# ProgramerSalar/stable-diffusion-from-scratch

Hardware: AMD Instinct MI355X
Metric: images/sec (512×512, 50-step DDIM) at 1/2/4/8 MI355X; UNet step ms (higher is better)
Workload: dtype f16; 1 GPU; sd1-txt2img-512-ddim50; global_batch=16, batch_per_gpu=16, ddim_steps=50, parallelism=dp1

## Files before the change

include/sdk_amd.h:

```cpp
#ifndef SDK_AMD_H
#define SDK_AMD_H

#include <stdint.h>

#ifdef __cplusplus
extern "C" {
#endif

typedef void* sdk_stream_t;

enum sdk_status {
  SDK_OK = 0,
  SDK_EINVAL = -1,
  SDK_EHIP = -2,
  SDK_EWORKSPACE = -3
};

typedef struct {
  const void* src0;
  const void* src1;
  int32_t c_split;
  int32_t cin;
  int32_t ld0, ld1;
  int32_t h, w;
  int32_t ksize;
  int32_t stride, pad;
  int32_t upsample;
  const float* gn_scale;
  const float* gn_shift;
  int32_t silu;
  int32_t pad_end;
} sdk_conv_src;

enum sdk_out_mode {
  SDK_OUT_NHWC_F16 = 0,
  SDK_OUT_NCHW_F32 = 1,
  SDK_OUT_GEGLU_F16 = 2,
  SDK_OUT_ROWS_F32 = 3
};

typedef struct {
  int32_t batch, ho, wo, cout;
  int32_t nseg;
  sdk_conv_src seg[2];
  const void* weight;
  int32_t k_total;
  const float* bias;
  const float* row_bias;
  int32_t row_bias_ld;
  const void* residual;
  int32_t res_ld;
  void* out;
  int32_t out_ld;
  int32_t out_mode;
  int32_t split_k;
  float* workspace;
  int64_t workspace_bytes;
  int32_t variant_hint;
  int32_t act;
  float* gn_partial;
  int64_t weight_batch_stride;
  int32_t split_inlaunch;
  uint32_t* tile_counters;
  int32_t tile_group_m;
  int32_t upsample_phase;
} sdk_conv_args;

#define SDK_TILE_COUNTERS 16384

enum sdk_conv_act {
  SDK_ACT_NONE = 0,
  SDK_ACT_QUICK_GELU = 1,
  SDK_ACT_GELU = 2
};

typedef struct {
  int32_t split_k;
  int32_t grid_tiles;
  int64_t workspace_bytes;
  int32_t variant;
  double flops;
  int32_t gn_chunks;
} sdk_conv_plan_info;

int sdk_conv2d_plan(const sdk_conv_args* a, sdk_conv_plan_info* info);
int sdk_conv2d(const sdk_conv_args* a, sdk_stream_t stream);

typedef struct {
  const void* src0; const void* src1;
  int32_t c_split, ld0, ld1;
  int32_t batch, hw, channels, groups;
  float eps;
  const float* gamma; const float* beta;
  float* scale; float* shift;
  float* workspace; int64_t workspace_bytes;
} sdk_group_norm_args;

int64_t sdk_group_norm_workspace(int32_t batch, int32_t hw, int32_t channels);
int sdk_group_norm_affine(const sdk_group_norm_args* a, sdk_stream_t stream);

int sdk_group_norm_apply(const sdk_group_norm_args* a, int32_t silu, void* y, int32_t ld_y, sdk_stream_t stream);

int sdk_group_norm_apply_padded(const sdk_group_norm_args* a, int32_t silu, void* y, int32_t ld_y, int32_t h,
                                int32_t w, int32_t pad, sdk_stream_t stream);

int sdk_group_norm(const sdk_group_norm_args* a, int32_t silu, void* y, int32_t ld_y, int32_t h, int32_t w,
                   int32_t pad, const float* part0, int32_t nch0, const float* part1, int32_t nch1,
                   sdk_stream_t stream);

int sdk_group_norm_finalize(const sdk_group_norm_args* a, const float* part0, int32_t nch0, const float* part1,
                            int32_t nch1, sdk_stream_t stream);

int sdk_group_norm_apply_ex(const sdk_group_norm_args* a, int32_t silu, const float* post_bias, int32_t pb_ld,
                            const void* residual, int32_t res_ld, void* y, int32_t ld_y, sdk_stream_t stream);

enum { SDK_GN_STATS_GIVEN = 0,
       SDK_GN_STATS_SLICE,
       SDK_GN_STATS_CHUNKED,
       SDK_GN_STATS_PARTS };
enum { SDK_GN_APPLY_NONE = 0,
       SDK_GN_APPLY_IN_STATS,
       SDK_GN_APPLY_FLAT, SDK_GN_APPLY_ROW, SDK_GN_APPLY_STRIDE };
typedef struct { int32_t stats, apply, launches; int64_t workspace_bytes; } sdk_group_norm_plan_info;
int sdk_group_norm_plan(const sdk_group_norm_args* a, int32_t want_stats, int32_t want_apply, int32_t h, int32_t w,
                        int32_t pad, int32_t nch0, int32_t nch1, int32_t allow_single_launch,
                        sdk_group_norm_plan_info* info);

double sdk_probe_mfma_flops(int32_t m16, int32_t blocks, int32_t iters);
int sdk_probe_mfma(int32_t m16, int32_t blocks, int32_t iters, const void* seed, float* sink, sdk_stream_t stream);
int sdk_probe_copy(const void* src, void* dst, int64_t bytes, sdk_stream_t stream);
int sdk_probe_copy_ex(const void* src, void* dst, int64_t bytes, int32_t mode, sdk_stream_t stream);

int sdk_layer_norm(const void* x, void* y, int32_t rows, int32_t cols, int32_t ld_x, int32_t ld_y,
                   const float* gamma, const float* beta, float eps, sdk_stream_t stream);

typedef struct {
  const void* q; const void* k; const void* v; void* o;
  int32_t q_ld, k_ld, v_ld, o_ld;
  int32_t batch, heads, nq, nk, head_dim;
  float scale;
  int32_t causal;
} sdk_attention_args;

int sdk_attention(const sdk_attention_args* a, sdk_stream_t stream);

enum { SDK_ATTN_AUTO = 0, SDK_ATTN_NW4, SDK_ATTN_NW8, SDK_ATTN_NW8_STAG, SDK_ATTN_QB2, SDK_ATTN_WIDE };
#define SDK_ATTN_WIDE_ROWS 64
#define SDK_ATTN_WIDE_KT 32
typedef struct { int32_t form, dqk, dv, waves, qblocks, stagger, seed_col, causal, grid; } sdk_attention_form_info;
int sdk_attention_form(const sdk_attention_args* a, int32_t form, sdk_attention_form_info* ran ,
                       sdk_stream_t stream);

typedef struct {
  const void* q; const void* k; const void* v; void* o;
  int32_t q_ld, k_ld, v_ld, o_ld;
  int32_t batch, heads, n, dim_head;
  void* workspace; int64_t workspace_bytes;
} sdk_linear_attention_args;
int32_t sdk_linear_attention_chunks(int32_t n);
int64_t sdk_linear_attention_workspace_bytes(const sdk_linear_attention_args* a);
int sdk_linear_attention(const sdk_linear_attention_args* a, sdk_stream_t stream);

typedef struct {
  const void* t; const void* kv; const void* wq; const void* wo; const float* bias; const void* res;
  void* out;
  int32_t t_ld, kv_ld, w_ld, res_ld, out_ld;
  int32_t batch, n_img, nk, channels, head_dim;
  float scale;
} sdk_xattn_args;

int sdk_cross_attention_block_supported(int32_t channels, int32_t head_dim, int32_t nk, int32_t n_img);
int sdk_xattn_pack_weight(const void* w, int32_t w_ld, void* packed, int32_t channels, sdk_stream_t stream);
int sdk_cross_attention_block(const sdk_xattn_args* a, sdk_stream_t stream);

typedef struct {
  const float* in_gamma; const float* in_beta; float in_eps;
  const float* out_gamma; const float* out_beta; float out_eps;
  void* out_ln; int32_t out_ln_ld;
} sdk_xattn_ln_args;

int sdk_cross_attention_block_ln(const sdk_xattn_args* a, const sdk_xattn_ln_args* ln, sdk_stream_t stream);

int sdk_segment_softmax(const float* s, int32_t ld_s, void* p, int32_t ld_p, int32_t rows, int32_t nseg,
                        int32_t seglen, float scale, sdk_stream_t stream);

typedef struct {
  const void* t; const void* res; void* out; const void* packed; const float* b2;
  int32_t t_ld, res_ld, out_ld;
  int32_t rows, channels, features;
} sdk_ff_args;

int sdk_ff_supported(int32_t channels, int32_t features);
int64_t sdk_ff_packed_bytes(int32_t channels, int32_t features);
int sdk_ff_pack(const void* w1, const float* b1, const void* w2, void* packed, int32_t channels, int32_t features,
                sdk_stream_t stream);
int sdk_feed_forward(const sdk_ff_args* a, sdk_stream_t stream);

typedef struct {
  const void* x; const void* w; const float* bias; const void* res; void* out;
  int32_t x_ld, res_ld, out_ld;
  int32_t rows, in_features, out_features;
} sdk_token_linear_args;

int sdk_token_linear_supported(int32_t in_features, int32_t out_features);
int sdk_token_linear(const sdk_token_linear_args* a, sdk_stream_t stream);

int sdk_token_linear_ln(const sdk_token_linear_args* a, const float* gamma, const float* beta, float eps,
                        void* out_ln, int32_t out_ln_ld, sdk_stream_t stream);

typedef struct {
  const void* x; const float* gn_scale; const float* gn_shift; const void* w; const float* bias;
  const float* gamma; const float* beta; void* tok; void* qkv;
  int32_t x_ld, tok_ld, qkv_ld, rows, hw;
  int32_t in_features, features, qkv_features;
  float eps;
} sdk_proj_norm_qkv_args;

int sdk_proj_norm_qkv_supported(int32_t in_features, int32_t features, int32_t qkv_features);
int sdk_proj_norm_qkv(const sdk_proj_norm_qkv_args* a, sdk_stream_t stream);

typedef struct {
  const float* x; const float* e; const float* e_uncond; const float* noise;
  float* x_prev; float* pred_x0;
  int64_t n;
  float sqrt_one_minus_at, sqrt_at, dir_coef, sqrt_a_prev, sigma, temperature;
  float guidance;
  int32_t v_param;
  float v_sqrt_a, v_sqrt_1ma;
} sdk_ddim_args;

int sdk_ddim_step(const sdk_ddim_args* a, sdk_stream_t stream);

int sdk_ddim_xprev(const sdk_ddim_args* a, sdk_stream_t stream);

typedef struct {
  const float* x; const float* model_out; const float* noise; const float* x_recon_in;
  float* x_prev; float* x_recon;
  int64_t n;
  int32_t stage, x0_param, clip;
  float c_recip, c_recipm1, coef1, coef2, sigma, nonzero, temperature;
} sdk_posterior_args;

int sdk_posterior_step(const sdk_posterior_args* a, sdk_stream_t stream);

typedef struct {
  const float* x0; const float* noise; const float* mask; const float* img;
  float* out;
  int64_t n, per_sample;
  int32_t hw, mask_mode;
  float sqrt_acp, sqrt_1m_acp;
} sdk_masked_q_args;

int sdk_masked_q_sample(const sdk_masked_q_args* a, sdk_stream_t stream);

int sdk_cfg_combine(const float* e_uncond, const float* e_cond, float* out, int64_t n, float guidance,
                    sdk_stream_t stream);

typedef struct {
  sdk_ddim_args step;
  int32_t pred_x0_in;
  float drop_scale;
  const uint8_t* keep;
  sdk_masked_q_args blend;
} sdk_ddim_ex_args;

int sdk_ddim_step_ex(const sdk_ddim_ex_args* a, sdk_stream_t stream);

typedef struct {
  sdk_posterior_args step;
  const uint8_t* keep;
  float drop_scale;
} sdk_posterior_ex_args;

int sdk_posterior_step_ex(const sdk_posterior_ex_args* a, sdk_stream_t stream);

enum { SDK_MULTISTEP_PLMS = 0, SDK_MULTISTEP_PLMS_WARMUP = 1, SDK_MULTISTEP_DPM = 2 };

typedef struct {
  sdk_ddim_args step;
  const float* hist[3];
  const float* e_next;
  float* hist_out;
  int32_t form, nhist;
  float c_x, c_0, c_1;
  int32_t reserved;
  sdk_masked_q_args blend;
} sdk_multistep_args;

int sdk_multistep_step(const sdk_multistep_args* a, sdk_stream_t stream);

typedef struct {
  const float* src[4];
  int32_t channels[4];
  int32_t nsrc;
  void* y;
  int32_t batch, hw, c_pad;
} sdk_concat_args;

int sdk_concat_nchw_to_nhwc(const sdk_concat_args* a, sdk_stream_t stream);

typedef struct {
  const float* src[4];
  int32_t channels[4];
  int32_t nsrc;
  void* y;
  int32_t batch, h, w, c_pad;
  int32_t kh, kw, sy, sx;
  int32_t p0, np;
} sdk_patch_pack_args;

int sdk_patch_pack(const sdk_patch_pack_args* a, sdk_stream_t stream);

int sdk_vq_code_norms(const float* codebook, float* norms, int32_t n, int32_t d, sdk_stream_t stream);

int32_t sdk_vq_nearest_splits(int64_t m, int32_t n, int32_t d);

int sdk_vq_nearest(const float* z, const float* codebook, const float* norms, int64_t* idx, float* z_q,
                   int32_t batch, int32_t d, int32_t hw, int32_t n, void* keys, int64_t keys_bytes,
                   int32_t force_splits, sdk_stream_t stream);

int sdk_vq_lookup(const int64_t* idx, const float* codebook, float* out, int64_t m, int32_t n, int32_t d,
                  int32_t hw, int32_t nchw, sdk_stream_t stream);

int sdk_vq_remap(const int64_t* inds, const int64_t* used, const int64_t* rnd, int64_t* out, int64_t count,
                 int32_t n_used, int32_t mode, int64_t unknown, int32_t extra, sdk_stream_t stream);

int sdk_ddpm_step(const float* x, const float* eps, const float* noise, float* out, int64_t n,
                  float inv_sqrt_alpha, float coef, float sigma, sdk_stream_t stream);

int sdk_timestep_embedding(const int64_t* t, const float* freqs, void* out, int32_t batch, int32_t dim,
                           sdk_stream_t stream);

int sdk_nchw_to_nhwc(const float* x, void* y, int32_t batch, int32_t channels, int32_t hw, int32_t c_pad,
                     float scale, sdk_stream_t stream);

int sdk_diag_gaussian_sample(const float* moments, const float* noise, float* z, int32_t batch, int32_t channels,
                             int32_t hw, float scale, sdk_stream_t stream);

int sdk_stochastic_encode(const float* x0, const float* noise, float* out, int64_t n, float sqrt_a,
                          float sqrt_1ma, sdk_stream_t stream);

int sdk_token_embedding(const int64_t* ids, const float* tok, const float* pos, void* out, int32_t batch,
                        int32_t seq, int32_t dim, sdk_stream_t stream);

int sdk_extract_patches(const float* z, float* out, int32_t batch, int32_t channels, int32_t h, int32_t w,
                        int32_t kh, int32_t kw, int32_t sy, int32_t sx, sdk_stream_t stream);
int sdk_fold_patches(const float* patches, const float* pix_w, const float* l_w, float* out, int32_t batch,
                     int32_t channels, int32_t h, int32_t w, int32_t ph, int32_t pw, int32_t sy, int32_t sx,
                     int32_t ly, int32_t lx, sdk_stream_t stream);

int sdk_upsample_bilinear2x(const void* x, void* y, int32_t batch, int32_t h, int32_t w, int32_t channels,
                            sdk_stream_t stream);
int sdk_gelu(const void* x, void* y, int64_t n, sdk_stream_t stream);

int sdk_upsample_nearest2x_padded(const void* x, int32_t ld_x, void* y, int32_t batch, int32_t h, int32_t w,
                                  int32_t channels, int32_t pad, sdk_stream_t stream);

int sdk_zero_border(const void* x, int32_t ld_x, void* y, int32_t batch, int32_t h, int32_t w, int32_t channels,
                    int32_t pad, sdk_stream_t stream);

int sdk_group_norm_film(const sdk_group_norm_args* a, const float* film, int32_t film_ld, int32_t film_off,
                        int32_t silu, void* y, int32_t ld_y, int32_t h, int32_t w, int32_t pad, const float* part0,
                        int32_t nch0, const float* part1, int32_t nch1, sdk_stream_t stream);

enum { SDK_RESAMPLE_AVGPOOL2 = 0, SDK_RESAMPLE_NEAREST2 = 1 };
int sdk_group_norm_resample(const sdk_group_norm_args* a, int32_t mode, int32_t silu, int32_t h, int32_t w,
                            int32_t pad, void* y_act, void* y_raw, sdk_stream_t stream);

int sdk_embedding_add(const void* emb, const float* table, const int64_t* ids, void* out, int32_t batch, int32_t dim,
                      int32_t n, sdk_stream_t stream);

int sdk_embedding_rows(const int64_t* ids, const float* table, void* out, int32_t n, int32_t dim,
                       sdk_stream_t stream);

enum { SDK_RESIZE_NEAREST = 0, SDK_RESIZE_BILINEAR = 1, SDK_RESIZE_BICUBIC = 2, SDK_RESIZE_AREA = 3 };
typedef struct {
  const float* x;
  float* y;
  int32_t planes, h, w, out_h, out_w, mode;
  double scale_h, scale_w;
} sdk_resize2d_args;

int sdk_resize2d(const sdk_resize2d_args* a, sdk_stream_t stream);

const char* sdk_last_error(void);
int sdk_version(void);
const char* sdk_kernel_name(int32_t variant);

#ifdef __cplusplus
}
#endif
#endif
```

stable-diffusion-from-scratch_amd/_lib.py:

```python
from __future__ import annotations

import ctypes as C
import os

_HERE = os.path.dirname(os.path.abspath(__file__))
LIB_PATH = os.environ.get("SD_AMD_LIB") or os.path.join(_HERE, "libsdk_amd.so")

vp = C.c_void_p
i32 = C.c_int32
i64 = C.c_int64
f32 = C.c_float
fp = C.POINTER(C.c_float)


class ConvSrc(C.Structure):
    _fields_ = [("src0", vp), ("src1", vp), ("c_split", i32), ("cin", i32), ("ld0", i32), ("ld1", i32),
                ("h", i32), ("w", i32), ("ksize", i32), ("stride", i32), ("pad", i32), ("upsample", i32),
                ("gn_scale", vp), ("gn_shift", vp), ("silu", i32), ("pad_end", i32)]


class ConvArgs(C.Structure):
    _fields_ = [("batch", i32), ("ho", i32), ("wo", i32), ("cout", i32), ("nseg", i32), ("seg", ConvSrc * 2),
                ("weight", vp), ("k_total", i32), ("bias", vp), ("row_bias", vp), ("row_bias_ld", i32),
                ("residual", vp), ("res_ld", i32), ("out", vp), ("out_ld", i32), ("out_mode", i32),
                ("split_k", i32), ("workspace", vp), ("workspace_bytes", i64), ("variant_hint", i32),
                ("act", i32), ("gn_partial", vp), ("weight_batch_stride", i64), ("split_inlaunch", i32),
                ("tile_counters", vp), ("tile_group_m", i32), ("upsample_phase", i32)]


class ConvPlanInfo(C.Structure):
    _fields_ = [("split_k", i32), ("grid_tiles", i32), ("workspace_bytes", i64), ("variant", i32),
                ("flops", C.c_double), ("gn_chunks", i32)]


class GroupNormArgs(C.Structure):
    _fields_ = [("src0", vp), ("src1", vp), ("c_split", i32), ("ld0", i32), ("ld1", i32), ("batch", i32),
                ("hw", i32), ("channels", i32), ("groups", i32), ("eps", f32), ("gamma", vp), ("beta", vp),
                ("scale", vp), ("shift", vp), ("workspace", vp), ("workspace_bytes", i64)]


class GroupNormPlanInfo(C.Structure):
    _fields_ = [("stats", i32), ("apply", i32), ("launches", i32), ("workspace_bytes", i64)]


class AttentionArgs(C.Structure):
    _fields_ = [("q", vp), ("k", vp), ("v", vp), ("o", vp), ("q_ld", i32), ("k_ld", i32), ("v_ld", i32),
                ("o_ld", i32), ("batch", i32), ("heads", i32), ("nq", i32), ("nk", i32), ("head_dim", i32),
                ("scale", f32), ("causal", i32)]


class AttentionFormInfo(C.Structure):
    _fields_ = [("form", i32), ("dqk", i32), ("dv", i32), ("waves", i32), ("qblocks", i32), ("stagger", i32),
                ("seed_col", i32), ("causal", i32), ("grid", i32)]


class LinearAttentionArgs(C.Structure):
    _fields_ = [("q", vp), ("k", vp), ("v", vp), ("o", vp), ("q_ld", i32), ("k_ld", i32), ("v_ld", i32),
                ("o_ld", i32), ("batch", i32), ("heads", i32), ("n", i32), ("dim_head", i32), ("workspace", vp),
                ("workspace_bytes", i64)]


class XAttnArgs(C.Structure):
    _fields_ = [("t", vp), ("kv", vp), ("wq", vp), ("wo", vp), ("bias", vp), ("res", vp), ("out", vp),
                ("t_ld", i32), ("kv_ld", i32), ("w_ld", i32), ("res_ld", i32), ("out_ld", i32), ("batch", i32),
                ("n_img", i32), ("nk", i32), ("channels", i32), ("head_dim", i32), ("scale", f32)]


class XAttnLnArgs(C.Structure):
    _fields_ = [("in_gamma", vp), ("in_beta", vp), ("in_eps", f32), ("out_gamma", vp), ("out_beta", vp),
                ("out_eps", f32), ("out_ln", vp), ("out_ln_ld", i32)]


class FfArgs(C.Structure):
    _fields_ = [("t", vp), ("res", vp), ("out", vp), ("packed", vp), ("b2", vp), ("t_ld", i32), ("res_ld", i32),
                ("out_ld", i32), ("rows", i32), ("channels", i32), ("features", i32)]


class TokenLinearArgs(C.Structure):
    _fields_ = [("x", vp), ("w", vp), ("bias", vp), ("res", vp), ("out", vp), ("x_ld", i32), ("res_ld", i32),
                ("out_ld", i32), ("rows", i32), ("in_features", i32), ("out_features", i32)]


class ProjNormQkvArgs(C.Structure):
    _fields_ = [("x", vp), ("gn_scale", vp), ("gn_shift", vp), ("w", vp), ("bias", vp), ("gamma", vp), ("beta", vp),
                ("tok", vp), ("qkv", vp), ("x_ld", i32), ("tok_ld", i32), ("qkv_ld", i32), ("rows", i32), ("hw", i32),
                ("in_features", i32), ("features", i32), ("qkv_features", i32), ("eps", f32)]


class DdimArgs(C.Structure):
    _fields_ = [("x", vp), ("e", vp), ("e_uncond", vp), ("noise", vp), ("x_prev", vp), ("pred_x0", vp),
                ("n", i64), ("sqrt_one_minus_at", f32), ("sqrt_at", f32), ("dir_coef", f32), ("sqrt_a_prev", f32),
                ("sigma", f32), ("temperature", f32), ("guidance", f32), ("v_param", i32), ("v_sqrt_a", f32),
                ("v_sqrt_1ma", f32)]


class PosteriorArgs(C.Structure):
    _fields_ = [("x", vp), ("model_out", vp), ("noise", vp), ("x_recon_in", vp), ("x_prev", vp), ("x_recon", vp),
                ("n", i64), ("stage", i32), ("x0_param", i32), ("clip", i32), ("c_recip", f32), ("c_recipm1", f32),
                ("coef1", f32), ("coef2", f32), ("sigma", f32), ("nonzero", f32), ("temperature", f32)]


class MaskedQArgs(C.Structure):
    _fields_ = [("x0", vp), ("noise", vp), ("mask", vp), ("img", vp), ("out", vp), ("n", i64), ("per_sample", i64),
                ("hw", i32), ("mask_mode", i32), ("sqrt_acp", f32), ("sqrt_1m_acp", f32)]


class DdimExArgs(C.Structure):
    _fields_ = [("step", DdimArgs), ("pred_x0_in", i32), ("drop_scale", f32), ("keep", vp), ("blend", MaskedQArgs)]


class MultistepArgs(C.Structure):
    _fields_ = [("step", DdimArgs), ("hist", vp * 3), ("e_next", vp), ("hist_out", vp), ("form", i32), ("nhist", i32),
                ("c_x", f32), ("c_0", f32), ("c_1", f32), ("reserved", i32), ("blend", MaskedQArgs)]


class PosteriorExArgs(C.Structure):
    _fields_ = [("step", PosteriorArgs), ("keep", vp), ("drop_scale", f32)]


class ConcatArgs(C.Structure):
    _fields_ = [("src", vp * 4), ("channels", i32 * 4), ("nsrc", i32), ("y", vp), ("batch", i32), ("hw", i32),
                ("c_pad", i32)]


class PatchPackArgs(C.Structure):
    _fields_ = [("src", vp * 4), ("channels", i32 * 4), ("nsrc", i32), ("y", vp), ("batch", i32), ("h", i32),
                ("w", i32), ("c_pad", i32), ("kh", i32), ("kw", i32), ("sy", i32), ("sx", i32), ("p0", i32),
                ("np", i32)]


class Resize2dArgs(C.Structure):
    _fields_ = [("x", vp), ("y", vp), ("planes", i32), ("h", i32), ("w", i32), ("out_h", i32), ("out_w", i32),
                ("mode", i32), ("scale_h", C.c_double), ("scale_w", C.c_double)]


OUT_NHWC_F16, OUT_NCHW_F32, OUT_GEGLU_F16, OUT_ROWS_F32 = 0, 1, 2, 3
RESIZE_NEAREST, RESIZE_BILINEAR, RESIZE_BICUBIC, RESIZE_AREA = range(4)
ACT_NONE, ACT_QUICK_GELU, ACT_GELU = 0, 1, 2
ATTN_AUTO, ATTN_NW4, ATTN_NW8, ATTN_NW8_STAG, ATTN_QB2, ATTN_WIDE = range(6)
MULTISTEP_PLMS, MULTISTEP_PLMS_WARMUP, MULTISTEP_DPM = range(3)
ATTN_WIDE_ROWS, ATTN_WIDE_KT = 64, 32
RESAMPLE_AVGPOOL2, RESAMPLE_NEAREST2 = 0, 1
GN_STATS = ("given", "slice", "chunked", "parts")
GN_APPLY = ("none", "in_stats", "flat", "row", "stride")

EXPORTS = ["sdk_conv2d_plan", "sdk_conv2d", "sdk_group_norm_workspace", "sdk_group_norm_affine", "sdk_group_norm_apply", "sdk_group_norm_apply_padded", "sdk_group_norm_apply_ex", "sdk_group_norm", "sdk_group_norm_finalize", "sdk_group_norm_plan", "sdk_layer_norm",
           "sdk_attention", "sdk_attention_form", "sdk_linear_attention", "sdk_linear_attention_workspace_bytes", "sdk_linear_attention_chunks", "sdk_cross_attention_block_supported", "sdk_xattn_pack_weight", "sdk_cross_attention_block", "sdk_cross_attention_block_ln", "sdk_segment_softmax", "sdk_ff_supported", "sdk_ff_packed_bytes", "sdk_ff_pack", "sdk_feed_forward", "sdk_token_linear_supported", "sdk_token_linear", "sdk_token_linear_ln", "sdk_proj_norm_qkv_supported", "sdk_proj_norm_qkv", "sdk_ddim_step", "sdk_ddim_xprev", "sdk_ddim_step_ex", "sdk_multistep_step", "sdk_cfg_combine", "sdk_posterior_step", "sdk_posterior_step_ex", "sdk_masked_q_sample", "sdk_concat_nchw_to_nhwc", "sdk_patch_pack", "sdk_ddpm_step", "sdk_timestep_embedding", "sdk_nchw_to_nhwc",
           "sdk_diag_gaussian_sample", "sdk_stochastic_encode", "sdk_token_embedding", "sdk_extract_patches",
           "sdk_fold_patches", "sdk_vq_code_norms", "sdk_vq_nearest_splits", "sdk_vq_nearest", "sdk_vq_lookup", "sdk_vq_remap",
           "sdk_upsample_bilinear2x", "sdk_upsample_nearest2x_padded", "sdk_zero_border", "sdk_gelu",
           "sdk_group_norm_film", "sdk_group_norm_resample", "sdk_embedding_add", "sdk_embedding_rows", "sdk_resize2d", "sdk_last_error", "sdk_version", "sdk_kernel_name",
           "sdk_probe_mfma_flops", "sdk_probe_mfma", "sdk_probe_copy", "sdk_probe_copy_ex"]

_lib = None


def lib():
    global _lib
    if _lib is not None:
        return _lib
    if not os.path.exists(LIB_PATH):
        raise RuntimeError(f"sd_amd: HIP library not built ({LIB_PATH} missing); run __graft_entry__.build()")
    import torch
    L = C.CDLL(LIB_PATH)
    L.sdk_conv2d_plan.argtypes = [C.POINTER(ConvArgs), C.POINTER(ConvPlanInfo)]
    L.sdk_conv2d.argtypes = [C.POINTER(ConvArgs), vp]
    L.sdk_group_norm_workspace.argtypes = [i32, i32, i32]
    L.sdk_group_norm_workspace.restype = i64
    L.sdk_group_norm_affine.argtypes = [C.POINTER(GroupNormArgs), vp]
    L.sdk_group_norm_apply.argtypes = [C.POINTER(GroupNormArgs), i32, vp, i32, vp]
    L.sdk_group_norm_apply_padded.argtypes = [C.POINTER(GroupNormArgs), i32, vp, i32, i32, i32, i32, vp]
    L.sdk_group_norm_apply_ex.argtypes = [C.POINTER(GroupNormArgs), i32, vp, i32, vp, i32, vp, i32, vp]
    L.sdk_group_norm.argtypes = [C.POINTER(GroupNormArgs), i32, vp, i32, i32, i32, i32, vp, i32, vp, i32, vp]
    L.sdk_group_norm_finalize.argtypes = [C.POINTER(GroupNormArgs), vp, i32, vp, i32, vp]
    L.sdk_group_norm_film.argtypes = [C.POINTER(GroupNormArgs), vp, i32, i32, i32, vp, i32, i32, i32, i32, vp, i32, vp,
                                      i32, vp]
    L.sdk_group_norm_plan.argtypes = [C.POINTER(GroupNormArgs), i32, i32, i32, i32, i32, i32, i32, i32,
                                      C.POINTER(GroupNormPlanInfo)]
    L.sdk_group_norm_resample.argtypes = [C.POINTER(GroupNormArgs), i32, i32, i32, i32, i32, vp, vp, vp]
    L.sdk_embedding_add.argtypes = [vp, vp, vp, vp, i32, i32, i32, vp]
    L.sdk_embedding_rows.argtypes = [vp, vp, vp, i32, i32, vp]
    L.sdk_resize2d.argtypes = [C.POINTER(Resize2dArgs), vp]
    L.sdk_upsample_bilinear2x.argtypes = [vp, vp, i32, i32, i32, i32, vp]
    L.sdk_upsample_nearest2x_padded.argtypes = [vp, i32, vp, i32, i32, i32, i32, i32, vp]
    L.sdk_zero_border.argtypes = [vp, i32, vp, i32, i32, i32, i32, i32, vp]
    L.sdk_gelu.argtypes = [vp, vp, i64, vp]
    L.sdk_layer_norm.argtypes = [vp, vp, i32, i32, i32, i32, vp, vp, f32, vp]
    L.sdk_attention.argtypes = [C.POINTER(AttentionArgs), vp]
    L.sdk_attention_form.argtypes = [C.POINTER(AttentionArgs), i32, C.POINTER(AttentionFormInfo), vp]
    L.sdk_linear_attention.argtypes = [C.POINTER(LinearAttentionArgs), vp]
    L.sdk_linear_attention_workspace_bytes.argtypes = [C.POINTER(LinearAttentionArgs)]
    L.sdk_linear_attention_workspace_bytes.restype = i64
    L.sdk_linear_attention_chunks.argtypes = [i32]
    L.sdk_linear_attention_chunks.restype = i32
    L.sdk_cross_attention_block_supported.argtypes = [i32, i32, i32, i32]
    L.sdk_xattn_pack_weight.argtypes = [vp, i32, vp, i32, vp]
    L.sdk_cross_attention_block.argtypes = [C.POINTER(XAttnArgs), vp]
    L.sdk_cross_attention_block_ln.argtypes = [C.POINTER(XAttnArgs), C.POINTER(XAttnLnArgs), vp]
    L.sdk_segment_softmax.argtypes = [vp, i32, vp, i32, i32, i32, i32, f32, vp]
    L.sdk_ff_supported.argtypes = [i32, i32]
    L.sdk_ff_packed_bytes.argtypes = [i32, i32]
    L.sdk_ff_packed_bytes.restype = i64
    L.sdk_ff_pack.argtypes = [vp, vp, vp, vp, i32, i32, vp]
    L.sdk_feed_forward.argtypes = [C.POINTER(FfArgs), vp]
    L.sdk_token_linear_supported.argtypes = [i32, i32]
    L.sdk_token_linear.argtypes = [C.POINTER(TokenLinearArgs), vp]
    L.sdk_token_linear_ln.argtypes = [C.POINTER(TokenLinearArgs), vp, vp, f32, vp, i32, vp]
    L.sdk_proj_norm_qkv_supported.argtypes = [i32, i32, i32]
    L.sdk_proj_norm_qkv.argtypes = [C.POINTER(ProjNormQkvArgs), vp]
    L.sdk_ddim_step.argtypes = [C.POINTER(DdimArgs), vp]
    L.sdk_ddim_xprev.argtypes = [C.POINTER(DdimArgs), vp]
    L.sdk_posterior_step.argtypes = [C.POINTER(PosteriorArgs), vp]
    L.sdk_ddim_step_ex.argtypes = [C.POINTER(DdimExArgs), vp]
    L.sdk_multistep_step.argtypes = [C.POINTER(MultistepArgs), vp]
    L.sdk_cfg_combine.argtypes = [vp, vp, vp, i64, f32, vp]
    L.sdk_posterior_step_ex.argtypes = [C.POINTER(PosteriorExArgs), vp]
    L.sdk_masked_q_sample.argtypes = [C.POINTER(MaskedQArgs), vp]
    L.sdk_concat_nchw_to_nhwc.argtypes = [C.POINTER(ConcatArgs), vp]
    L.sdk_patch_pack.argtypes = [C.POINTER(PatchPackArgs), vp]
    L.sdk_vq_code_norms.argtypes = [vp, vp, i32, i32, vp]
    L.sdk_vq_nearest_splits.argtypes = [i64, i32, i32]
    L.sdk_vq_nearest_splits.restype = i32
    L.sdk_vq_nearest.argtypes = [vp, vp, vp, vp, vp, i32, i32, i32, i32, vp, i64, i32, vp]
    L.sdk_vq_lookup.argtypes = [vp, vp, vp, i64, i32, i32, i32, i32, vp]
    L.sdk_vq_remap.argtypes = [vp, vp, vp, vp, i64, i32, i32, i64, i32, vp]
    L.sdk_ddpm_step.argtypes = [vp, vp, vp, vp, i64, f32, f32, f32, vp]
    L.sdk_timestep_embedding.argtypes = [vp, vp, vp, i32, i32, vp]
    L.sdk_nchw_to_nhwc.argtypes = [vp, vp, i32, i32, i32, i32, f32, vp]
    L.sdk_diag_gaussian_sample.argtypes = [vp, vp, vp, i32, i32, i32, f32, vp]
    L.sdk_stochastic_encode.argtypes = [vp, vp, vp, i64, f32, f32, vp]
    L.sdk_token_embedding.argtypes = [vp, vp, vp, vp, i32, i32, i32, vp]
    L.sdk_extract_patches.argtypes = [vp, vp, i32, i32, i32, i32, i32, i32, i32, i32, vp]
    L.sdk_fold_patches.argtypes = [vp, vp, vp, vp, i32, i32, i32, i32, i32, i32, i32, i32, i32, i32, vp]
    L.sdk_probe_mfma_flops.argtypes = [i32, i32, i32]
    L.sdk_probe_mfma_flops.restype = C.c_double
    L.sdk_probe_mfma.argtypes = [i32, i32, i32, vp, vp, vp]
    L.sdk_probe_copy.argtypes = [vp, vp, i64, vp]
    L.sdk_probe_copy_ex.argtypes = [vp, vp, i64, i32, vp]
    L.sdk_last_error.restype = C.c_char_p
    L.sdk_kernel_name.restype = C.c_char_p
    L.sdk_kernel_name.argtypes = [i32]
    for name in EXPORTS:
        if not hasattr(L, name):
            raise RuntimeError(f"sd_amd: {LIB_PATH} does not export {name}")
    _lib = L
    return L


def check(rc: int, what: str):
    if rc != 0:
        msg = lib().sdk_last_error().decode(errors="replace")
        raise RuntimeError(f"sd_amd.{what} failed ({rc}): {msg}")
```

stable-diffusion-from-scratch_amd/build.py:

```python
from __future__ import annotations

import concurrent.futures as cf
import os
import re
import subprocess

HERE = os.path.dirname(os.path.abspath(__file__))
CSRC = os.path.join(HERE, "csrc")
BUILD = os.path.join(HERE, "build")
LIB = os.path.join(HERE, "libsdk_amd.so")
SOURCES = ["norm.hip", "attention.hip", "attention_wide.hip", "linattn.hip", "sampler.hip", "xattn.hip", "ff.hip", "token.hip", "proj_qkv.hip", "vq.hip", "cond.hip", "probe.hip"]
CONV_TILE_PARTS = 5


def _units():
    yield "conv_plan.hip", "conv_plan", []
    yield "conv_small.hip", "conv_small", []
    yield "conv_rowpanel.hip", "conv_rowpanel", []
    for k in range(1, CONV_TILE_PARTS + 1):
        yield "conv_tile.hip", f"conv_tile_p{k}", [f"-DSDK_CONV_PART={k}"]
    for src in SOURCES:
        yield src, src.replace(".hip", ""), []


def _deps(src: str, csrc: str):
    headers = [os.path.join(csrc, "common.h"), os.path.join(HERE, "..", "include", "sdk_amd.h")]
    if src.startswith("conv") or src == "proj_qkv.hip":
        headers += sorted(os.path.join(csrc, f) for f in os.listdir(csrc) if f.startswith("conv") and f.endswith(".h"))
    return [os.path.join(csrc, src)] + headers
HIPCC = os.environ.get("HIPCC", "/opt/rocm/bin/hipcc")
FLAGS = ["--offload-arch=gfx950", "-O3", "-fPIC", "-std=c++17", "-Wno-unused-result"]
EXTRA = {"attention.hip": ["-mno-amdgpu-ieee", "-fno-honor-nans"],
         "attention_wide.hip": ["-mno-amdgpu-ieee", "-fno-honor-nans"]}
REMARK = "-Rpass-analysis=kernel-resource-usage"
NO_SCRATCH = re.compile(r"token_linear320_kernel|attn_wide_kernel|conv_rowpanel_kernel|proj_norm_qkv_kernel")
WARN_SCRATCH = re.compile(r"conv_glds_kernel|conv_ph_kernel|ff_geglu_kernel|xattn_block_kernel|attn_fwd_kernel|vq_nearest_")
_RES = re.compile(r"remark: (?:Function Name: (\S+)|\s+(VGPRs|AGPRs|ScratchSize \[bytes/lane\]|Occupancy \[waves/SIMD\]): (\d+))")


def resource_usage(stderr: str):
    out = []
    for m in _RES.finditer(stderr):
        if m.group(1):
            out.append((m.group(1), {}))
        elif out:
            out[-1][1][m.group(2).split(" ")[0]] = int(m.group(3))
    return out


def _needs(obj: str, deps) -> bool:
    if not os.path.exists(obj):
        return True
    t = os.path.getmtime(obj)
    return any(os.path.getmtime(d) > t for d in deps)


def build(force: bool = False, verbose: bool = False, diag: bool = False, tag: str = "", defines=(),
          extra=None, csrc: str = CSRC) -> str:
    suffix = "_diag" if diag else (f"_{tag}" if tag else "")
    bdir = BUILD + suffix
    lib = LIB.replace(".so", f"{suffix}.so")
    extra_flags = dict(EXTRA)
    for k, v in (extra or {}).items():
        extra_flags[k] = extra_flags.get(k, []) + list(v)
    os.makedirs(bdir, exist_ok=True)
    jobs = []
    objs = []
    for src, stem, udefs in _units():
        s = os.path.join(csrc, src)
        o = os.path.join(bdir, stem + ".o")
        objs.append(o)
        flags_file = o + ".flags"
        dflags = (["-DSDK_CONV_DIAGNOSTICS"] if diag else []) + list(defines) + udefs
        fl = " ".join(FLAGS + extra_flags.get(src, []) + dflags)
        stale_flags = not os.path.exists(flags_file) or open(flags_file).read() != fl
        if force or stale_flags or _needs(o, _deps(src, csrc)) or not os.path.exists(o + ".res"):
            for stale in (o, flags_file):
                if os.path.exists(stale):
                    os.remove(stale)
            jobs.append(([HIPCC, *FLAGS, *dflags, *extra_flags.get(src, []), REMARK, "-c", s, "-o", o],
                         (flags_file, fl)))

    def run(cmd, sidecar=None):
        r = subprocess.run(cmd, capture_output=True, text=True)
        if r.returncode != 0:
            raise RuntimeError(f"hipcc failed: {' '.join(cmd)}\n{r.stdout}\n{r.stderr}")
        if REMARK in cmd:
            usage = resource_usage(r.stderr)
            obj = cmd[cmd.index("-o") + 1]
            with open(obj + ".res", "w") as f:
                for name, u in usage:
                    f.write(f"{name} vgpr={u.get('VGPRs')} agpr={u.get('AGPRs')} scratch={u.get('ScratchSize')} "
                            f"occ={u.get('Occupancy')}\n")
            if os.path.basename(obj).startswith("token") and not any(
                    NO_SCRATCH.search(n) and "ScratchSize" in u for n, u in usage):
                os.remove(obj)
                raise RuntimeError("no kernel-resource-usage remark for token_linear320_kernel: cannot verify "
                                   "that it uses no scratch")
            bad = [n for n, u in usage if NO_SCRATCH.search(n) and u.get("ScratchSize", 0) > 0]
            for n, u in usage:
                if WARN_SCRATCH.search(n) and u.get("ScratchSize", 0) > 0:
                    print(f"warning: {n} uses {u['ScratchSize']} B/lane of scratch", flush=True)
            if bad:
                os.remove(obj)
                raise RuntimeError("counted-vmcnt kernels use scratch (spills break the hand-counted waits): " +
                                   ", ".join(bad))
        if sidecar:
            with open(sidecar[0], "w") as f:
                f.write(sidecar[1])
        if verbose:
            print(" ".join(cmd))
        return r

    workers = int(os.environ.get("SD_AMD_BUILD_JOBS", "8"))
    with cf.ThreadPoolExecutor(max_workers=min(workers, max(1, len(jobs)))) as ex:
        list(ex.map(lambda j: run(*j), jobs))
    if force or jobs or _needs(lib, objs):
        run([HIPCC, "--offload-arch=gfx950", "-shared", "-fPIC", *objs, "-o", lib])
        with open(os.path.join(bdir, "resource_usage.txt"), "w") as f:
            for o in objs:
                if os.path.exists(o + ".res"):
                    f.write(open(o + ".res").read())
    return lib


if __name__ == "__main__":
    import sys
    print(build(verbose=True, diag="--diag" in sys.argv))
```

stable-diffusion-from-scratch_amd/csrc/ff.hip:

```cpp
#include <cstdlib>
#include <type_traits>

#include "common.h"

namespace sdk {
namespace {

constexpr int FFC = 320;
constexpr int FF_KS = FFC / 16;
constexpr int FF_OB = FFC / 32;
constexpr int FF_OBH = FF_OB / 2;
constexpr int FF_W1 = 32 * FFC * 2;
constexpr int FF_W2 = 2 * FFC * 16;
constexpr int FF_B1 = 32 * 4;
constexpr int FF_BLK = FF_W1 + FF_W2 + FF_B1;
constexpr int FF_BSL = FF_W1 + FF_W2 + 1024;
constexpr int FF_BPC = (FF_W1 + FF_W2) / 1024 + 1;
constexpr int FF_SLOT = 2 * FF_BSL;
constexpr int FF_PIECES = 2 * FF_BPC;
constexpr int FF_NW = 8, FF_NT = FF_NW * 64, FF_ROWS = 128;
constexpr int FF_GPW = (FF_PIECES + FF_NW - 1) / FF_NW;
constexpr int FF_NS = 2;
constexpr int FF_XB = FF_NS * FF_SLOT;
constexpr int FF_LDS = FF_XB + FF_NW * 1024 + 1024;
constexpr int FF_ORS = FFC + 8;
constexpr unsigned FF_OOB = 0x80000000u;
static_assert(FF_ROWS * FF_ORS * 2 <= FF_NS * FF_SLOT, "epilogue staging fits the ring");
static_assert(FF_LDS <= 160 * 1024, "LDS");

struct FfParams {
  const half_t* t;
  const half_t* res;
  half_t* out;
  const char* w;
  const float* b2;
  int t_ld, res_ld, out_ld;
  int M, nfb;
};

__device__ __forceinline__ __amdgpu_buffer_rsrc_t ff_rsrc(const void* base, long long bytes) {
  const int n = (int)(bytes < 0x7fffffffLL ? bytes : 0x7fffffffLL);
  return __builtin_amdgcn_make_buffer_rsrc(const_cast<void*>(base), 0, n, 0x00020000);
}

__device__ __forceinline__ void ff_dma(__amdgpu_buffer_rsrc_t r, char* dst, unsigned voff) {
  __builtin_amdgcn_raw_ptr_buffer_load_lds(r, (__attribute__((address_space(3))) void*)dst, 16, voff, 0, 0, 0);
}

template <int DBG>
__global__ void __launch_bounds__(FF_NT, 1) ff_geglu_kernel(FfParams p) {
  extern __shared__ __attribute__((aligned(16))) char ffl[];
  const int tid = threadIdx.x, lane = tid & 63;
  const int wave = __builtin_amdgcn_readfirstlane(tid >> 6);
  const int pr = wave & 3, half = wave >> 2;
  const int fr = lane & 31, hh = lane >> 5;
  const int m0 = blockIdx.x * FF_ROWS;
  const __amdgpu_buffer_rsrc_t rw = ff_rsrc(p.w, (long long)p.nfb * FF_BLK);

  const unsigned lane16 = (unsigned)lane * 16u;
  const unsigned lane16_b1 = lane < 8 ? lane16 : FF_OOB;
  unsigned soff[FF_GPW];
  int doff[FF_GPW];
  unsigned b1mask = 0;
#pragma unroll
  for (int j = 0; j < FF_GPW; ++j) {
    const int piece = j * FF_NW + wave;
    const int blk = piece / FF_BPC, q = piece - blk * FF_BPC;
    const bool dummy = piece >= FF_PIECES, b1p = !dummy && q == FF_BPC - 1;
    soff[j] = dummy ? FF_OOB : (unsigned)(blk * FF_BLK + (b1p ? FF_W1 + FF_W2 : q * 1024));
    doff[j] = dummy ? FF_LDS - 1024 : blk * FF_BSL + (b1p ? FF_W1 + FF_W2 : q * 1024);
    b1mask |= (b1p ? 1u : 0u) << j;
  }
  auto issue = [&](int it, int slot) __attribute__((always_inline)) {
    if constexpr ((DBG & 1) != 0) return;
    const unsigned base = 2 * it < p.nfb ? (unsigned)(2 * it) * FF_BLK : FF_OOB;
#pragma unroll
    for (int j = 0; j < FF_GPW; ++j) {
      const bool dummy = doff[j] == FF_LDS - 1024;
      char* d = ffl + (dummy ? 0 : slot * FF_SLOT) + doff[j];
      ff_dma(rw, d, base + soff[j] + (((b1mask >> j) & 1u) ? lane16_b1 : lane16));
    }
  };

  h8 tq[FF_KS];
  {
    const int tok = min(m0 + pr * 32 + fr, p.M - 1);
    const half_t* tp = p.t + (size_t)tok * p.t_ld + 8 * hh;
#pragma unroll
    for (int ks = 0; ks < FF_KS; ++ks) tq[ks] = *reinterpret_cast<const h8*>(tp + 16 * ks);
  }
  issue(0, 0);

  const int sw = (fr >> 1) & 7;
  f16v o[FF_OBH];
#pragma unroll
  for (int ob = 0; ob < FF_OBH; ++ob) o[ob] = f16v{};
  const int niter = p.nfb / 2;
  h8* xb_own = reinterpret_cast<h8*>(ffl + FF_XB + wave * 1024) + lane;
  const h8* xb_par = reinterpret_cast<const h8*>(ffl + FF_XB + (wave ^ 4) * 1024) + lane;
  for (int it = 0; it < niter; ++it) {
    const int slot = it & 1;
    asm volatile("s_waitcnt vmcnt(0)" ::: "memory");
    __builtin_amdgcn_s_barrier();
    issue(it + 1, slot ^ 1);
    const char* st = ffl + slot * FF_SLOT + half * FF_BSL;
    const float* b1 = reinterpret_cast<const float*>(st + FF_W1 + FF_W2);
    f16v s;
    {
      const f4 q0 = *reinterpret_cast<const f4*>(b1 + 4 * hh), q1 = *reinterpret_cast<const f4*>(b1 + 8 + 4 * hh);
      const f4 q2 = *reinterpret_cast<const f4*>(b1 + 16 + 4 * hh), q3 = *reinterpret_cast<const f4*>(b1 + 24 + 4 * hh);
#pragma unroll
      for (int q = 0; q < 4; ++q) {
        s[q] = q0[q];
        s[4 + q] = q1[q];
        s[8 + q] = q2[q];
        s[12 + q] = q3[q];
      }
    }
    auto w1frag = [&](int ks) __attribute__((always_inline)) {
      const int c = 2 * (ks & 3) + hh;
      return *reinterpret_cast<const h8*>(st + (ks >> 2) * 4096 + fr * 128 + ((c ^ sw) << 4));
    };
    constexpr int LA = 4;
    h8 wa[FF_KS];
#pragma unroll
    for (int j = 0; j < LA; ++j) wa[j] = w1frag(j);
#pragma unroll
    for (int ks = 0; ks < FF_KS; ++ks) {
      if (ks + LA < FF_KS) wa[ks + LA] = w1frag(ks + LA);
      if constexpr ((DBG & 2) == 0) s = __builtin_amdgcn_mfma_f32_32x32x16_f16(wa[ks], tq[ks], s, 0, 0, 0);
      else s[ks & 15] += (float)wa[ks][0];
    }
    __builtin_amdgcn_sched_group_barrier(0x100, LA + 4, 0);
#pragma unroll
    for (int i = 0; i < FF_KS; ++i) {
      __builtin_amdgcn_sched_group_barrier(0x008, 1, 0);
      __builtin_amdgcn_sched_group_barrier(0x100, 1, 0);
    }
    h8 h;
#pragma unroll
    for (int j = 0; j < 8; ++j) {
      if constexpr ((DBG & 4) != 0) h[j] = (half_t)s[j];
      else h[j] = (half_t)(s[j] * gelu_erf(s[j + 8]));
    }
    *xb_own = h;
    __syncthreads();
    const h8 hp = *xb_par;
    const h8 he = half ? hp : h, ho = half ? h : hp;
    const char* w2e = ffl + slot * FF_SLOT + FF_W1 + (hh * FFC + half * 160 + fr) * 16;
    const char* w2o = w2e + FF_BSL;
#pragma unroll
    for (int ob = 0; ob < FF_OBH; ++ob) {
      const h8 ae = *reinterpret_cast<const h8*>(w2e + ob * 32 * 16);
      const h8 ao = *reinterpret_cast<const h8*>(w2o + ob * 32 * 16);
      if constexpr ((DBG & 2) == 0) {
        o[ob] = __builtin_amdgcn_mfma_f32_32x32x16_f16(ae, he, o[ob], 0, 0, 0);
        o[ob] = __builtin_amdgcn_mfma_f32_32x32x16_f16(ao, ho, o[ob], 0, 0, 0);
      } else {
        o[ob][ob] += (float)ae[0] + (float)ao[0] + (float)he[ob & 7] + (float)ho[ob & 7];
      }
    }
  }

  asm volatile("s_waitcnt vmcnt(0)" ::: "memory");
  __syncthreads();
  half_t* os = reinterpret_cast<half_t*>(ffl);
  const int trow = pr * 32 + fr;
#pragma unroll
  for (int ob = 0; ob < FF_OBH; ++ob)
#pragma unroll
    for (int g = 0; g < 4; ++g) {
      const int ch = half * 160 + ob * 32 + 8 * g + 4 * hh;
      const f4 bb = p.b2 ? *reinterpret_cast<const f4*>(p.b2 + ch) : f4{0.f, 0.f, 0.f, 0.f};
      h4 v;
#pragma unroll
      for (int q = 0; q < 4; ++q) v[q] = (half_t)(o[ob][4 * g + q] + bb[q]);
      *reinterpret_cast<h4*>(os + trow * FF_ORS + ch) = v;
    }
  __syncthreads();
  constexpr int CPR = FFC / 8;
  for (int e = tid; e < FF_ROWS * CPR; e += FF_NT) {
    const int r = e / CPR, c8 = e - r * CPR;
    const int m = m0 + r;
    if (m >= p.M) break;
    h8 v = *reinterpret_cast<const h8*>(os + r * FF_ORS + c8 * 8);
    if (p.res) {
      const h8 rr = *reinterpret_cast<const h8*>(p.res + (size_t)m * p.res_ld + c8 * 8);
#pragma unroll
      for (int q = 0; q < 8; ++q) v[q] = (half_t)((float)v[q] + (float)rr[q]);
    }
    *reinterpret_cast<h8*>(p.out + (size_t)m * p.out_ld + c8 * 8) = v;
  }
}

__global__ void __launch_bounds__(256) ff_pack_kernel(const half_t* __restrict__ w1, const float* __restrict__ b1,
                                                      const half_t* __restrict__ w2, char* __restrict__ out, int F,
                                                      int nfb) {
  constexpr int CPB = FF_BLK / 16;
  const long long q = (long long)blockIdx.x * 256 + threadIdx.x;
  if (q >= (long long)nfb * CPB) return;
  const int fb = (int)(q / CPB), e = (int)(q - (long long)fb * CPB);
  char* dst = out + (size_t)fb * FF_BLK + (size_t)e * 16;
  auto w1row = [&](int r) { return r < 16 ? 16 * fb + r : F + 16 * fb + (r - 16); };
  if (e < FF_W1 / 16) {
    const int u = e / 256, rem = e - u * 256, r = rem / 8, cpos = rem - r * 8;
    const int c = cpos ^ ((r >> 1) & 7);
    *reinterpret_cast<h8*>(dst) = *reinterpret_cast<const h8*>(w1 + (size_t)w1row(r) * FFC + 64 * u + 8 * c);
  } else if (e < (FF_W1 + FF_W2) / 16) {
    const int x = e - FF_W1 / 16, hv = x / FFC, o = x - hv * FFC;
    h8 v;
#pragma unroll
    for (int j = 0; j < 8; ++j) v[j] = w2[(size_t)o * F + 16 * fb + 8 * (j >> 2) + 4 * hv + (j & 3)];
    *reinterpret_cast<h8*>(dst) = v;
  } else {
    const int r0 = (e - (FF_W1 + FF_W2) / 16) * 4;
    f4 v;
#pragma unroll
    for (int i = 0; i < 4; ++i) v[i] = b1 ? b1[w1row(r0 + i)] : 0.f;
    *reinterpret_cast<f4*>(dst) = v;
  }
}

template <int DBG>
int ff_launch(const FfParams& p, unsigned blocks, hipStream_t s) {
  static std::atomic<unsigned long long> lds_done{0};
  const int rc = ensure_dyn_lds((const void*)ff_geglu_kernel<DBG>, FF_LDS, lds_done, "feed_forward");
  if (rc != SDK_OK) return rc;
  hipLaunchKernelGGL(ff_geglu_kernel<DBG>, dim3(blocks), dim3(FF_NT), FF_LDS, s, p);
  return check_launch("feed_forward");
}

int ff_launch_dbg(const FfParams& p, unsigned blocks, int dbg, hipStream_t s) {
#if defined(SDK_CONV_DIAGNOSTICS)
  switch (dbg) {
    case 1: return ff_launch<1>(p, blocks, s);
    case 2: return ff_launch<2>(p, blocks, s);
    case 3: return ff_launch<3>(p, blocks, s);
    case 4: return ff_launch<4>(p, blocks, s);
    case 5: return ff_launch<5>(p, blocks, s);
    default: break;
  }
#endif
  (void)dbg;
  return ff_launch<0>(p, blocks, s);
}

bool ff_shape_ok(int channels, int features) { return channels == FFC && features > 0 && features % 32 == 0; }

}
}

using namespace sdk;

extern "C" int sdk_ff_supported(int32_t channels, int32_t features) { return ff_shape_ok(channels, features) ? 1 : 0; }

extern "C" int64_t sdk_ff_packed_bytes(int32_t channels, int32_t features) {
  return ff_shape_ok(channels, features) ? (int64_t)(features / 16) * FF_BLK : -1;
}

extern "C" int sdk_ff_pack(const void* w1, const float* b1, const void* w2, void* packed, int32_t channels,
                           int32_t features, sdk_stream_t stream) {
  if (!w1 || !w2 || !packed) return fail(SDK_EINVAL, "ff_pack: null pointer");
  if (!ff_shape_ok(channels, features)) return fail(SDK_EINVAL, "ff_pack: channels must be 320, features a multiple of 32");
  if (((uintptr_t)w1 | (uintptr_t)packed) & 15) return fail(SDK_EINVAL, "ff_pack: w1 / packed must be 16-B aligned");
  const int nfb = features / 16;
  const long long chunks = (long long)nfb * (FF_BLK / 16);
  hipLaunchKernelGGL(ff_pack_kernel, dim3((unsigned)((chunks + 255) / 256)), dim3(256), 0, (hipStream_t)stream,
                     (const half_t*)w1, b1, (const half_t*)w2, (char*)packed, (int)features, nfb);
  return check_launch("ff_pack");
}

extern "C" int sdk_feed_forward(const sdk_ff_args* a, sdk_stream_t stream) {
  if (!a || !a->t || !a->out || !a->packed) return fail(SDK_EINVAL, "feed_forward: null pointer");
  if (!ff_shape_ok(a->channels, a->features))
    return fail(SDK_EINVAL, "feed_forward: channels must be 320, features a multiple of 32");
  if (a->rows <= 0) return fail(SDK_EINVAL, "feed_forward: empty");
  if (a->t_ld % 8 || a->out_ld % 8 || (a->res && a->res_ld % 8) || a->t_ld < a->channels || a->out_ld < a->channels ||
      (a->res && a->res_ld < a->channels))
    return fail(SDK_EINVAL, "feed_forward: row strides must be multiples of 8 and >= channels");
  if (((uintptr_t)a->t | (uintptr_t)a->out | (uintptr_t)a->res | (uintptr_t)a->packed | (uintptr_t)a->b2) & 15)
    return fail(SDK_EINVAL, "feed_forward: pointers must be 16-B aligned");
  if ((long long)(a->features / 16) * FF_BLK >= 0x7fffffffLL) return fail(SDK_EINVAL, "feed_forward: too many features");
  FfParams p{(const half_t*)a->t, (const half_t*)a->res, (half_t*)a->out, (const char*)a->packed, a->b2,
             a->t_ld, a->res_ld, a->out_ld, a->rows, a->features / 16};
  const unsigned blocks = (unsigned)((a->rows + FF_ROWS - 1) / FF_ROWS);
#if defined(SDK_CONV_DIAGNOSTICS)
  static const int dbg = getenv("SDK_FF_DBG") ? atoi(getenv("SDK_FF_DBG")) & 7 : 0;
#else
  constexpr int dbg = 0;
#endif
  return ff_launch_dbg(p, blocks, dbg, (hipStream_t)stream);
}
```

stable-diffusion-from-scratch_amd/openai_model/attention.py:

```python
from __future__ import annotations

import os
import math

import torch
from torch import nn

from .. import ops
from ..packing import f32, gn_norm, gn_scale_shift, prep_norm
from .utils import conv_nd, normalization, zero_module


def Normalize(in_channels):
    return torch.nn.GroupNorm(num_groups=32, num_channels=in_channels, eps=1e-6, affine=True)


_FUSED_ENV = os.environ.get("SD_AMD_FUSED_XATTN")
FUSED_CROSS_ATTENTION = _FUSED_ENV != "0"
FUSED_XATTN_MIN_ROWS = 0 if _FUSED_ENV == "1" else 65536
FUSED_XATTN_640_MAX_ROWS = 16384
FUSED_XATTN_NORMS = os.environ.get("SD_AMD_XATTN_NORMS") != "0"


def _use_fused_xattn(channels, head_dim, nk, n_img, batch):
    if not FUSED_CROSS_ATTENTION or n_img % 64:
        return False
    rows = batch * n_img
    if _FUSED_ENV != "1":
        if channels == 320:
            if rows < FUSED_XATTN_MIN_ROWS:
                return False
        elif channels != 640 or rows > FUSED_XATTN_640_MAX_ROWS:
            return False
    return ops.cross_attention_block_supported(channels, head_dim, nk, n_img)


XATTN_REASSOC = os.environ.get("SD_AMD_XATTN_REASSOC") != "0"

FUSED_FF = os.environ.get("SD_AMD_FUSED_FF") != "0"
TOKEN_LINEAR = os.environ.get("SD_AMD_TOKEN_LINEAR", "1") != "0"
_CHAIN_ENV = os.environ.get("SD_AMD_PROJ_QKV_CHAIN", "1")
PROJ_QKV_CHAIN = _CHAIN_ENV != "0"
PROJ_QKV_CHAIN_GN = _CHAIN_ENV != "xn"


class ReassocContext:
    __slots__ = ("kv", "w1", "w2", "heads", "nk", "batch", "_build")

    def __init__(self, kv, heads, nk, batch, build):
        self.kv, self.heads, self.nk, self.batch, self._build = kv, heads, nk, batch, build
        self.w1 = self.w2 = None

    def weights(self):
        if self.w1 is None:
            if torch.cuda.is_available() and torch.cuda.is_current_stream_capturing():
                raise RuntimeError("ReassocContext: per-prompt weights are built eagerly — run one eager "
                                   "step with this context before capturing a graph")
            self.w1, self.w2 = self._build()
            self._build = None
        return self.w1, self.w2


def reassoc_weights(k, v, wq, wo):
    B, L, H, d = k.shape
    w1 = torch.einsum("bjhe,hec->bhjc", k, wq.view(H, d, -1)).reshape(B, H * L, -1)
    w2 = torch.einsum("che,bjhe->bchj", wo.view(wo.shape[0], H, d), v).reshape(B, wo.shape[0], H * L)
    return w1, w2


def _reassoc_applies(inner, heads, nk):
    kr = (heads * nk + ops.BK - 1) // ops.BK * ops.BK
    return XATTN_REASSOC and 2 * kr <= inner


class CrossAttention(nn.Module):

    def __init__(self, query_dim, context_dim=None, heads=8, dim_head=64, dropout=0.):
        super().__init__()
        inner_dim = dim_head * heads
        self.self_attn = context_dim is None
        context_dim = query_dim if context_dim is None else context_dim
        self.scale = dim_head ** -0.5
        self.heads = heads
        self.dim_head = dim_head
        self.to_q = nn.Linear(query_dim, inner_dim, bias=False)
        self.to_k = nn.Linear(context_dim, inner_dim, bias=False)
        self.to_v = nn.Linear(context_dim, inner_dim, bias=False)
        self.to_out = nn.Sequential(nn.Linear(inner_dim, query_dim), nn.Dropout(dropout))

    def _prepare(self, dev):
        qd = self.to_q.in_features
        cd = self.to_k.in_features
        if self.self_attn:
            w = torch.cat([self.to_q.weight, self.to_k.weight, self.to_v.weight], 0)
            self._pc_qkv = ops.PackedConv([(w, qd)], None, device=dev)
        self._pc_q = ops.PackedConv([(self.to_q.weight, qd)], None, device=dev)
        self._pc_kv = ops.PackedConv([(torch.cat([self.to_k.weight, self.to_v.weight], 0), cd)], None, device=dev)
        self._pc_o = ops.PackedConv([(self.to_out[0].weight, self.heads * self.dim_head)], self.to_out[0].bias,
                                    device=dev)
        inner = self.heads * self.dim_head
        self._ptl_o = (ops.PackedTokenLinear(self.to_out[0].weight, self.to_out[0].bias, dev)
                       if self.self_attn and ops.token_linear_supported(inner, self.to_out[0].out_features) else None)
        if not self.self_attn:
            self._bo32 = f32(self.to_out[0].bias, dev)
            self._pc_reassoc = None

    def context_kv(self, ctx2d, L=None):
        kv = ops.linear(self._pc_kv, ctx2d)
        inner = self.heads * self.dim_head
        if L is None or self.self_attn or not _reassoc_applies(inner, self.heads, L):
            return kv
        B, H, d = ctx2d.shape[0] // L, self.heads, self.dim_head
        C = self.to_q.in_features
        Co = self.to_out[0].out_features

        def build():
            dev = kv.device
            if self._pc_reassoc is None:
                wq, wo = self.to_q.weight.detach(), self.to_out[0].weight.detach()
                self._pc_reassoc = (
                    [ops.PackedConv([(wq[h * d:(h + 1) * d].t().contiguous(), d)], None, device=dev) for h in range(H)],
                    [ops.PackedConv([(wo[:, h * d:(h + 1) * d].contiguous(), d)], None, device=dev) for h in range(H)])
            pq, po = self._pc_reassoc
            kr = (H * L + ops.BK - 1) // ops.BK * ops.BK
            w1 = torch.zeros(B, (kr + ops.BN - 1) // ops.BN * ops.BN, C, dtype=torch.float16, device=dev)
            w2 = torch.zeros(B, (Co + ops.BN - 1) // ops.BN * ops.BN, kr, dtype=torch.float16, device=dev)
            w1h = w1[:, :H * L].view(B, H, L, C)
            for h in range(H):
                w1h[:, h] = ops.linear(pq[h], kv[:, h * d:(h + 1) * d]).view(B, L, C)
                w2[:, :Co, h * L:(h + 1) * L] = ops.linear(po[h], kv[:, inner + h * d:inner + (h + 1) * d]).view(
                    B, L, Co).transpose(1, 2)
            return ops.PerImageWeights(w1, H * L), ops.PerImageWeights(w2, Co, self._bo32)
        return ReassocContext(kv, H, L, B, build)

    def _run(self, t, residual, B, N, kv=None, Lc=None, qkv=None):
        inner = self.heads * self.dim_head
        if kv is None:
            if self.self_attn:
                if qkv is None:
                    qkv = ops.linear(self._pc_qkv, t)
                q, k, v, nk = qkv[:, :inner], qkv[:, inner:2 * inner], qkv[:, 2 * inner:], N
            else:
                q = ops.linear(self._pc_q, t)
                kvx = ops.linear(self._pc_kv, t)
                k, v, nk = kvx[:, :inner], kvx[:, inner:], N
        else:
            ops.PROFILER.region = "cross_attention"
            if isinstance(kv, ReassocContext):
                if t.stride(-1) == 1 and N % 128 == 0 and kv.batch == B:
                    w1, w2 = kv.weights()
                    s = ops.linear(w1, t, out_mode=ops.OUT_ROWS_F32, n_img=N)
                    p = ops.segment_softmax(s, kv.heads, kv.nk, self.scale, ld_p=w2.k_total)
                    out = ops.linear(w2, p, residual=residual, n_img=N)
                    ops.PROFILER.region = None
                    return out
                kv = kv.kv
            if t.stride(-1) == 1 and _use_fused_xattn(inner, self.dim_head, Lc, N, B):
                out = ops.cross_attention_block(t, kv, self._pc_q, self._pc_o, batch=B, n_img=N, nk=Lc,
                                                heads=self.heads, head_dim=self.dim_head, scale=self.scale,
                                                residual=residual)
                ops.PROFILER.region = None
                return out
            q = ops.linear(self._pc_q, t)
            k, v, nk = kv[:, :inner], kv[:, inner:], Lc
        o = ops.attention(q, k, v, batch=B, heads=self.heads, nq=N, nk=nk, head_dim=self.dim_head, scale=self.scale)
        if TOKEN_LINEAR and self._ptl_o is not None and o.stride(-1) == 1 and \
                (residual is None or residual.is_contiguous()):
            out = ops.token_linear(self._ptl_o, o, residual=residual)
        else:
            out = ops.linear(self._pc_o, o, residual=residual)
        ops.PROFILER.region = None
        return out


class GELU(nn.Module):

    def __init__(self, dim_in, dim_out):
        super().__init__()
        self.proj = nn.Linear(dim_in, dim_out * 2)


class FeedForward(nn.Module):

    def __init__(self, dim, dim_out=None, mult=4, glu=False, dropout=0.):
        super().__init__()
        inner_dim = int(dim * mult)
        dim_out = dim if dim_out is None else dim_out
        if not glu:
            raise NotImplementedError("sd_amd: only the gated (GEGLU) feed-forward is on the SD path")
        self.net = nn.Sequential(GELU(dim, inner_dim), nn.Dropout(dropout), nn.Linear(inner_dim, dim_out))

    def _prepare(self, dev):
        p = self.net[0].proj
        self._pc1 = ops.PackedConv([(p.weight, p.in_features)], p.bias, geglu=True, device=dev)
        self._pc2 = ops.PackedConv([(self.net[2].weight, self.net[2].in_features)], self.net[2].bias, device=dev)
        self._pff = None
        if FUSED_FF and ops.ff_supported(p.in_features, p.out_features // 2):
            self._pff = ops.PackedFF(p.weight, p.bias, self.net[2].weight, self.net[2].bias, dev)

    def _run(self, t, residual):
        if self._pff is not None and t.stride(-1) == 1:
            return ops.feed_forward(self._pff, t, residual=residual)
        g = ops.linear(self._pc1, t, out_mode=ops.OUT_GEGLU_F16)
        return ops.linear(self._pc2, g, residual=residual)


class BasicTransformerBlock(nn.Module):

    def __init__(self, dim, n_heads, d_head, dropout=0., context_dim=None, gated_ff=True, checkpoint=True):
        super().__init__()
        self.attn1 = CrossAttention(query_dim=dim, heads=n_heads, dim_head=d_head, dropout=dropout)
        self.ff = FeedForward(dim=dim, dropout=dropout, glu=gated_ff)
        self.attn2 = CrossAttention(query_dim=dim, context_dim=context_dim, heads=n_heads, dim_head=d_head,
                                    dropout=dropout)
        self.norm1 = nn.LayerNorm(dim)
        self.norm2 = nn.LayerNorm(dim)
        self.norm3 = nn.LayerNorm(dim)
        self.checkpoint = checkpoint

    def _prepare(self, dev):
        for m in (self.attn1, self.attn2, self.ff):
            m._prepare(dev)
        for n in (self.norm1, self.norm2, self.norm3):
            prep_norm(n, dev)

    def _run(self, tok, B, N, kv=None, Lc=None, t=None, qkv=None):
        if t is None and qkv is None:
            t = ops.layer_norm(tok, self.norm1._g, self.norm1._b, self.norm1.eps)
        tok = self.attn1._run(t, tok, B, N, qkv=qkv)
        a2 = self.attn2
        if (kv is not None and FUSED_XATTN_NORMS and tok.stride(-1) == 1
                and _use_fused_xattn(a2.heads * a2.dim_head, a2.dim_head, Lc, N, B)):
            ops.PROFILER.region = "cross_attention"
            tok, t = ops.cross_attention_block(
                tok, kv, a2._pc_q, a2._pc_o, batch=B, n_img=N, nk=Lc, heads=a2.heads, head_dim=a2.dim_head,
                scale=a2.scale, residual=tok, norm_in=(self.norm2._g, self.norm2._b, self.norm2.eps),
                norm_out=(self.norm3._g, self.norm3._b, self.norm3.eps))
            ops.PROFILER.region = None
            return self.ff._run(t, tok)
        t = ops.layer_norm(tok, self.norm2._g, self.norm2._b, self.norm2.eps)
        tok = self.attn2._run(t, tok, B, N, kv, Lc)
        t = ops.layer_norm(tok, self.norm3._g, self.norm3._b, self.norm3.eps)
        return self.ff._run(t, tok)


class SpatialTransformer(nn.Module):

    def __init__(self, in_channels, n_heads, d_head, depth=1, dropout=0., context_dim=None, use_linear=False):
        super().__init__()
        self.in_channels = in_channels
        inner_dim = n_heads * d_head
        self.inner_dim = inner_dim
        self.use_linear = use_linear
        self.norm = Normalize(in_channels)
        if use_linear:
            self.proj_in = nn.Linear(in_channels, inner_dim)
        else:
            self.proj_in = nn.Conv2d(in_channels, inner_dim, kernel_size=1, stride=1, padding=0)
        self.transformer_blocks = nn.ModuleList(
            [BasicTransformerBlock(inner_dim, n_heads, d_head, dropout=dropout, context_dim=context_dim)
             for _ in range(depth)])
        if use_linear:
            self.proj_out = zero_module(nn.Linear(in_channels, inner_dim))
        else:
            self.proj_out = zero_module(nn.Conv2d(inner_dim, in_channels, kernel_size=1, stride=1, padding=0))

    def _prepare(self, dev):
        prep_norm(self.norm, dev)
        self._pc_in = ops.PackedConv([(self.proj_in.weight, self.in_channels)], self.proj_in.bias, device=dev)
        self._ptl_in = (ops.PackedTokenLinear(self.proj_in.weight, self.proj_in.bias, dev)
                        if ops.token_linear_supported(self.in_channels, self.inner_dim) else None)
        self._pc_out = ops.PackedConv([(self.proj_out.weight, self.inner_dim)], self.proj_out.bias, device=dev)
        for blk in self.transformer_blocks:
            blk._prepare(dev)
        self._ppq = None
        if len(self.transformer_blocks) and self._ptl_in is not None:
            a1 = self.transformer_blocks[0].attn1
            if ops.proj_norm_qkv_supported(self.in_channels, self.inner_dim, 3 * a1.heads * a1.dim_head):
                wqkv = torch.cat([a1.to_q.weight, a1.to_k.weight, a1.to_v.weight], 0)
                self._ppq = ops.PackedProjQkv(self.proj_in.weight, self.proj_in.bias, wqkv, dev)

    def context_kv(self, ctx2d, L=None):
        return [blk.attn2.context_kv(ctx2d, L) for blk in self.transformer_blocks]

    def _run(self, x, kvs=None, Lc=None):
        B, H, W, Cc = x.shape
        if (PROJ_QKV_CHAIN and TOKEN_LINEAR and self._ppq is not None and x.is_contiguous()
                and ops.proj_qkv_chain_fills(B * H * W, ops.cu_count(x.device))):
            n1 = self.transformer_blocks[0].norm1
            if PROJ_QKV_CHAIN_GN:
                tok, qkv = ops.proj_norm_qkv(self._ppq, x.view(B * H * W, Cc), (n1._g, n1._b, n1.eps),
                                             gn=gn_scale_shift(self.norm, x), hw=H * W)
            else:
                xn = gn_norm(self.norm, x, silu=False)
                tok, qkv = ops.proj_norm_qkv(self._ppq, xn.view(B * H * W, Cc), (n1._g, n1._b, n1.eps))
            for i, blk in enumerate(self.transformer_blocks):
                tok = blk._run(tok, B, H * W, None if kvs is None else kvs[i], Lc, qkv=qkv if i == 0 else None)
            return ops.conv2d(self._pc_out, tok.view(B, H, W, self.inner_dim), residual=x, gn_stats=True)
        xn = gn_norm(self.norm, x, silu=False)
        t1 = None
        if TOKEN_LINEAR and self._ptl_in is not None and xn.is_contiguous():
            n1 = self.transformer_blocks[0].norm1 if len(self.transformer_blocks) else None
            if n1 is not None:
                tok, t1 = ops.token_linear(self._ptl_in, xn.view(B * H * W, Cc), norm=(n1._g, n1._b, n1.eps))
            else:
                tok = ops.token_linear(self._ptl_in, xn.view(B * H * W, Cc))
        else:
            tok = ops.conv2d(self._pc_in, xn).view(B * H * W, self.inner_dim)
        for i, blk in enumerate(self.transformer_blocks):
            tok = blk._run(tok, B, H * W, None if kvs is None else kvs[i], Lc, t=t1 if i == 0 else None)
        return ops.conv2d(self._pc_out, tok.view(B, H, W, self.inner_dim), residual=x, gn_stats=True)


class QKVAttentionLegacy(nn.Module):

    def __init__(self, n_heads):
        super().__init__()
        self.n_heads = n_heads

    def scale(self, ch):
        return 1.0 / math.sqrt(math.sqrt(ch))


class FlashAttention(nn.Module):

    def __init__(self, n_heads):
        super().__init__()
        self.n_heads = n_heads

    def scale(self, ch):
        return 1.0 / math.sqrt(ch)


class AttentionBlock(nn.Module):

    def __init__(self, channels, num_heads=1, num_head_channels=-1, use_checkpoint=False,
                 use_new_attention_order=False):
        super().__init__()
        self.channels = channels
        if num_head_channels == -1:
            self.num_heads = num_heads
        else:
            assert channels % num_head_channels == 0
            self.num_heads = channels // num_head_channels
        self.use_checkpoint = use_checkpoint
        self.norm = normalization(channels)
        self.qkv = conv_nd(1, channels, channels * 3, 1)
        self.attention = FlashAttention(self.num_heads) if use_new_attention_order else \
            QKVAttentionLegacy(self.num_heads)
        self.proj_out = zero_module(conv_nd(1, channels, channels, 1))

    def _prepare(self, dev):
        self.norm._prepare(dev)
        self._pc_qkv = ops.PackedConv([(self.qkv.weight, self.channels)], self.qkv.bias, device=dev)
        self._pc_proj = ops.PackedConv([(self.proj_out.weight, self.channels)], self.proj_out.bias, device=dev)

    def _run(self, x):
        B, H, W, Cc = x.shape
        xn = self.norm.norm(x, silu=False)
        qkv = ops.conv2d(self._pc_qkv, xn).view(B * H * W, 3 * Cc)
        ch = Cc // self.num_heads
        o = ops.attention(qkv[:, :Cc], qkv[:, Cc:2 * Cc], qkv[:, 2 * Cc:], batch=B, heads=self.num_heads,
                          nq=H * W, nk=H * W, head_dim=ch, scale=self.attention.scale(ch))
        return ops.conv2d(self._pc_proj, o.view(B, H, W, Cc), residual=x, gn_stats=True)
```

stable-diffusion-from-scratch_amd/ops.py:

```python
from __future__ import annotations

import ctypes as C
import math

import numpy as np
import torch

from . import _lib
from ._lib import (ACT_NONE, ACT_QUICK_GELU, ACT_GELU, AttentionArgs, XAttnArgs, XAttnLnArgs, FfArgs, TokenLinearArgs, ProjNormQkvArgs, ConvArgs, ConvPlanInfo, GroupNormArgs,
                   OUT_GEGLU_F16, OUT_NCHW_F32, OUT_NHWC_F16, OUT_ROWS_F32, check, lib)

BK = 64
BN = 128


def _stream():
    return C.c_void_p(torch.cuda.current_stream().cuda_stream)


def _ptr(t):
    return C.c_void_p(t.data_ptr()) if t is not None else None


def _need_cuda(t: torch.Tensor, what: str, dtype=torch.float16):
    if not isinstance(t, torch.Tensor) or not t.is_cuda:
        raise TypeError(f"sd_amd.{what}: expected a CUDA tensor (HIP path only, no CPU fallback)")
    if dtype is not None and t.dtype != dtype:
        raise TypeError(f"sd_amd.{what}: expected {dtype}, got {t.dtype}")


def need_gpu_sampler(option: str, device):
    if torch.device(device).type != "cuda":
        raise NotImplementedError(f"sd_amd: {option} is implemented on the GPU only (HIP kernels, no CPU "
                                  f"fallback); got device '{device}'")



class _Workspace:

    def __init__(self):
        self.buf = {}
        self.retired = []
        self.lane = 0

    def release_retired(self):
        self.retired.clear()

    def use_lane(self, lane: int):
        import contextlib

        @contextlib.contextmanager
        def cm():
            prev, self.lane = self.lane, lane
            try:
                yield
            finally:
                self.lane = prev
        return cm()

    def counters(self, device) -> torch.Tensor:
        key = (torch.device(device).index, self.lane, "cnt")
        c = self.buf.get(key)
        if c is None:
            if torch.cuda.is_current_stream_capturing():
                raise RuntimeError("sd_amd: tile counters must exist before graph capture (run one warm-up step)")
            c = torch.zeros(TILE_COUNTERS, dtype=torch.int32, device=device)
            self.buf[key] = c
        return c

    def get(self, nbytes: int, device) -> torch.Tensor:
        key = (torch.device(device).index, self.lane)
        b = self.buf.get(key)
        if b is None or b.numel() < nbytes:
            if torch.cuda.is_current_stream_capturing():
                raise RuntimeError("sd_amd: workspace must be sized before graph capture (run one warm-up step)")
            if b is not None:
                self.retired.append(b)
                nbytes = max(nbytes, 2 * b.numel())
            b = torch.empty(max(nbytes, 1 << 20), dtype=torch.uint8, device=device)
            self.buf[key] = b
        return b


WORKSPACE = _Workspace()
TILE_COUNTERS = 16384



def _as_pair(x):
    if isinstance(x, tuple):
        a, b = x
        return a, b
    return x, None


def src_shape(x):
    a, b = _as_pair(x)
    B, H, W, C0 = a.shape
    return B, H, W, C0 + (b.shape[-1] if b is not None else 0)


def _fill_src(s: "_lib.ConvSrc", x, ksize, stride, pad, upsample, gn, silu):
    a, b = _as_pair(x)
    _need_cuda(a, "conv2d")
    B, H, W, C0 = a.shape
    if a.stride(3) != 1 or (H > 1 and a.stride(1) != W * a.stride(2)) or (B > 1 and a.stride(0) != H * a.stride(1)):
        raise ValueError("sd_amd.conv2d: source must be NHWC with contiguous channels and a uniform pixel stride")
    s.src0 = a.data_ptr()
    s.ld0 = a.stride(2) if a.dim() == 4 else a.stride(1)
    if b is not None:
        _need_cuda(b, "conv2d")
        s.src1 = b.data_ptr()
        s.ld1 = b.stride(2)
        s.c_split = C0
        s.cin = C0 + b.shape[-1]
    else:
        s.src1 = None
        s.ld1 = 0
        s.c_split = C0
        s.cin = C0
    s.h, s.w = H, W
    s.ksize, s.stride, s.pad, s.upsample = ksize, stride, pad, 1 if upsample else 0
    if gn is not None:
        s.gn_scale, s.gn_shift = gn[0].data_ptr(), gn[1].data_ptr()
    else:
        s.gn_scale = s.gn_shift = None
    s.silu = 1 if silu else 0
    return B, H, W



class PackedConv:

    def __init__(self, segments, bias=None, geglu=False, device="cuda"):
        cols, self.seg_geom = [], []
        n_out = None
        for w, cin_src in segments:
            w = w.detach().float()
            if w.dim() == 2:
                w = w[:, :, None, None]
            if w.dim() == 3:
                w = w[:, :, :, None]
            N, Cin, kh, kw = w.shape
            assert kh == kw, "square kernels only"
            if n_out is None:
                n_out = N
            assert N == n_out
            cin_pad = (cin_src + BK - 1) // BK * BK
            wp = torch.zeros(N, kh, kw, cin_pad, dtype=torch.float32, device=w.device)
            wp[:, :, :, :Cin] = w.permute(0, 2, 3, 1)
            wp = wp.reshape(N, kh * kw, cin_pad // BK, BK).permute(0, 2, 1, 3)
            cols.append(wp.reshape(N, -1))
            self.seg_geom.append((kh, cin_src))
        Wt = torch.cat(cols, dim=1)
        b = bias.detach().float().clone() if bias is not None else None
        if geglu:
            inner = n_out // 2
            assert inner % 32 == 0
            idx = []
            for q in range(inner // 32):
                idx += list(range(32 * q, 32 * q + 32)) + list(range(inner + 32 * q, inner + 32 * q + 32))
            idx = torch.tensor(idx, device=Wt.device)
            Wt = Wt[idx]
            if b is not None:
                b = b[idx.to(b.device)]
        self.N = n_out
        self.geglu = geglu
        npad = (n_out + BN - 1) // BN * BN
        Wfull = torch.zeros(npad, Wt.shape[1], dtype=torch.float32, device=Wt.device)
        Wfull[:n_out] = Wt
        self.weight = Wfull.to(device=device, dtype=torch.float16).contiguous()
        self.k_total = self.weight.shape[1]
        self.bias = b.to(device=device, dtype=torch.float32).contiguous() if b is not None else None


class PerImageWeights:

    def __init__(self, weight, n, bias=None):
        assert weight.dim() == 3 and weight.dtype == torch.float16 and weight.is_contiguous()
        assert weight.shape[1] % BN == 0 and weight.shape[2] % BK == 0 and n <= weight.shape[1]
        self.weight = weight
        self.N = n
        self.k_total = weight.shape[2]
        self.bias = bias
        self.geglu = False
        self.seg_geom = [(1, weight.shape[2])]
        self.w_batch_stride = weight.shape[1] * weight.shape[2]


def fold_upsample_weight(w):
    assert w.dim() == 4 and w.shape[2:] == (3, 3)
    rows = ((w[:, :, 0], w[:, :, 1] + w[:, :, 2]), (w[:, :, 0] + w[:, :, 1], w[:, :, 2]))
    out = w.new_empty(4, w.shape[0], w.shape[1], 2, 2)
    for a in range(2):
        for dy in range(2):
            r = rows[a][dy]
            cols = ((r[:, :, 0], r[:, :, 1] + r[:, :, 2]), (r[:, :, 0] + r[:, :, 1], r[:, :, 2]))
            for b in range(2):
                for dx in range(2):
                    out[2 * a + b, :, :, dy, dx] = cols[b][dx]
    return out


class PhaseConv:

    def __init__(self, weight, cin_src, bias=None, device="cuda"):
        ph = fold_upsample_weight(weight.detach().float())
        packs = [PackedConv([(ph[q], cin_src)], bias if q == 0 else None, device=device) for q in range(4)]
        self.weight = torch.stack([pk.weight for pk in packs]).contiguous()
        self.N, self.k_total, self.bias = packs[0].N, packs[0].k_total, packs[0].bias
        self.geglu = False
        self.seg_geom = [(2, cin_src)]
        self.w_batch_stride = self.weight.shape[1] * self.weight.shape[2]


def _conv_source_files():
    import os
    src = os.environ.get("SD_AMD_CONV_SOURCE") or os.path.join(os.path.dirname(os.path.abspath(__file__)), "csrc")
    if not os.path.isdir(src):
        src = os.path.dirname(src)
    return [os.path.join(src, f) for f in sorted(os.listdir(src)) if f.startswith("conv")]


def _conv_source_hash():
    import hashlib
    import os
    h = hashlib.sha1()
    for path in _conv_source_files():
        h.update(os.path.basename(path).encode() + b"\0")
        with open(path, "rb") as f:
            h.update(f.read())
    return h.hexdigest()[:16]


class _Autotune:
    VARIANTS = (2, 7, 6, 4, 3, 8, 9, 16, 17, 18, 19, 20, 21, 22, 23, 24, 25, 26, 31, 32, 33, 34, 35, 38, 40, 49)
    SPLITS = (0, 1, 2, 3, 4, 6, 8, 12, 16, -2)
    GROUPS = (1, 8, 16)

    def __init__(self):
        import os
        self.enabled = False
        self.table = {}
        self.timed = 0
        ev = os.environ.get("SD_AMD_TUNE_VARIANTS")
        if ev:
            self.VARIANTS = tuple(int(v) for v in ev.split(","))
        self.reps = int(os.environ.get("SD_AMD_TUNE_REPS", "3"))

    def enable(self, on=True):
        self.enabled = on

    def save(self, path):
        import json
        with open(path, "w") as f:
            json.dump({"device": torch.cuda.get_device_name(0) if torch.cuda.is_available() else None,
                       "conv_source": _conv_source_hash(),
                       "entries": [[list(k), list(v)] for k, v in sorted(self.table.items(), key=str)]}, f, indent=0)

    def load(self, path):
        import json
        with open(path) as f:
            d = json.load(f)
        if d.get("conv_source") != _conv_source_hash():
            return 0
        n = 0
        for k, v in d["entries"]:
            self.table[tuple(k)] = tuple(v)
            n += 1
        return n

    def key(self, a, pc, gn=False):
        s0, s1 = a.seg[0], a.seg[1]
        return (a.batch, a.ho, a.wo, a.cout, a.nseg, pc.k_total, a.out_mode, s0.cin, s0.h, s0.w, s0.ksize,
                s0.stride, s0.upsample, s0.c_split, int(bool(s0.gn_scale) or bool(s0.silu)),
                s1.cin if a.nseg > 1 else 0, int(gn), int(bool(a.weight_batch_stride)))

    def choose(self, a, pc, dev, gn=False):
        key = self.key(a, pc, gn)
        hit = self.table.get(key)
        if hit is not None or not self.enabled or torch.cuda.is_current_stream_capturing():
            return hit
        cands = self.VARIANTS
        if a.nseg > 1 and (a.seg[1].gn_scale or a.seg[1].silu):
            self.table[key] = (0, 0)
            return self.table[key]
        if a.seg[0].gn_scale or a.seg[0].silu:
            cands = (0, 35)
        best, best_t = (0, 0), float("inf")
        info = ConvPlanInfo()
        stream = _stream()
        emit_any = False
        if gn:
            for v in cands:
                for sp in self.SPLITS:
                    a.variant_hint = v + 1
                    set_split(a, sp, dev)
                    if lib().sdk_conv2d_plan(C.byref(a), C.byref(info)) == 0 and info.gn_chunks > 0:
                        emit_any = True
        for v in cands:
            for sp in self.SPLITS:
                a.variant_hint = v + 1
                set_split(a, sp, dev)
                if lib().sdk_conv2d_plan(C.byref(a), C.byref(info)) != 0:
                    continue
                if info.variant != v:
                    continue
                if sp == 0 and info.split_k in self.SPLITS[1:]:
                    continue
                part = None
                if emit_any:
                    if info.gn_chunks == 0:
                        continue
                    part = torch.empty(a.batch, info.gn_chunks, a.cout, 2, dtype=torch.float32, device=dev)
                    a.gn_partial = part.data_ptr()
                else:
                    a.gn_partial = None
                if info.workspace_bytes > 0:
                    ws = WORKSPACE.get(info.workspace_bytes, dev)
                    a.workspace, a.workspace_bytes = ws.data_ptr(), ws.numel()
                for gm in (self.GROUPS if info.split_k == 1 else (0,)):
                    a.tile_group_m = gm
                    check(lib().sdk_conv2d(C.byref(a), stream), "conv2d(autotune)")
                    e0, e1 = torch.cuda.Event(enable_timing=True), torch.cuda.Event(enable_timing=True)
                    e0.record()
                    for _ in range(self.reps):
                        lib().sdk_conv2d(C.byref(a), stream)
                    e1.record()
                    e1.synchronize()
                    t = e0.elapsed_time(e1)
                    if t < best_t:
                        best_t, best = t, (v + 1, -2 if sp == -2 else info.split_k, gm)
        a.variant_hint, a.gn_partial, a.tile_group_m = 0, None, 0
        set_split(a, 0, dev)
        self.table[key] = best
        self.timed += 1
        if self.timed % 10 == 0:
            import sys
            print(f"sd_amd autotune: {self.timed} conv problems timed", file=sys.stderr, flush=True)
        return best


AUTOTUNE = _Autotune()


def set_split(a, sp, dev):
    if sp == -2:
        a.split_k, a.split_inlaunch = 2, 1
        a.tile_counters = WORKSPACE.counters(dev).data_ptr()
    else:
        a.split_k, a.split_inlaunch, a.tile_counters = sp, 0, None


FORCE_VARIANT = None
TILE_GROUP_M = None


GN_ATTR = "_sd_gn_partial"
EMIT_GN_STATS = True


def _claim(out):
    if out is not None and hasattr(out, GN_ATTR):
        delattr(out, GN_ATTR)
    return out


BUF_LIMIT = int(__import__("os").environ.get("SD_AMD_CONV_CHUNK_LIMIT", "2147483647"))


def _src_bytes(x):
    a, b = _as_pair(x)
    B, H, W, _ = a.shape
    ld = max(a.stride(2), b.stride(2) if b is not None else 0)
    return B * H * W * ld * 2


def _bslice(t, b0, b1):
    if t is None:
        return None
    if isinstance(t, tuple):
        return tuple(_bslice(u, b0, b1) for u in t)
    return t[b0:b1]


def _conv2d_batch_chunks(pc, x, seg2, gn, row_bias, residual, out, B, kw):
    big = max(_src_bytes(x), _src_bytes(seg2[0]) if seg2 is not None else 0)
    n = -(-big // BUF_LIMIT)
    while big * 1.0 / n >= BUF_LIMIT or B % n:
        n += 1
        if n >= B:
            n = B
            break
    cb = B // n
    outs = []
    for b0 in range(0, B, cb):
        b1 = min(B, b0 + cb)
        s2 = None if seg2 is None else (_bslice(seg2[0], b0, b1), _bslice(seg2[1], b0, b1), seg2[2])
        rb = None if row_bias is None else (row_bias[0][b0:b1], row_bias[1])
        outs.append(conv2d(pc, _bslice(x, b0, b1), seg2=s2, gn=_bslice(gn, b0, b1), row_bias=rb,
                           residual=_bslice(residual, b0, b1), out=None if out is None else out[b0:b1], **kw))
    full = out if out is not None else torch.cat(outs, 0)
    parts = [getattr(o, GN_ATTR, None) for o in outs]
    if all(pp is not None for pp in parts) and len({pp[1] for pp in parts}) == 1:
        setattr(full, GN_ATTR, (torch.cat([pp[0] for pp in parts], 0), parts[0][1], full._version))
    return full


def _conv_out(pc, x, ksize, stride, pad, pad_end, upsample, phase, out_mode):
    B, H, W = _as_pair(x)[0].shape[:3]
    lh, lw = (2 * H, 2 * W) if upsample else (H, W)
    Ho = (lh + 2 * pad + pad_end - ksize) // stride + 1
    Wo = (lw + 2 * pad + pad_end - ksize) // stride + 1
    if phase:
        Ho, Wo = 2 * (H - 2), 2 * (W - 2)
    shape = {OUT_GEGLU_F16: (B, Ho, Wo, pc.N // 2), OUT_NCHW_F32: (B, pc.N, Ho, Wo)}.get(out_mode, (B, Ho, Wo, pc.N))
    dt = torch.float16 if out_mode in (OUT_NHWC_F16, OUT_GEGLU_F16) else torch.float32
    return Ho, Wo, shape, dt


def conv2d(pc: PackedConv, x, *, ksize=None, stride=1, pad=None, pad_end=0, upsample=False, gn=None, silu=False,
           seg2=None, bias=True, row_bias=None, residual=None, out_mode=OUT_NHWC_F16, out=None,
           variant=None, split_k=None, act=ACT_NONE, gn_stats=False, plan_out=None, phase=False):
    _claim(out)
    if phase:
        assert isinstance(pc, PhaseConv) and not isinstance(x, tuple) and not upsample and stride == 1
        ksize, pad, pad_end = 2, 0, 0
    B0 = _as_pair(x)[0].shape[0]
    dev = _as_pair(x)[0].device
    k0 = pc.seg_geom[0][0] if ksize is None else ksize
    Ho, Wo, shape, dt = _conv_out(pc, x, k0, stride, k0 // 2 if pad is None else pad, pad_end, upsample, phase, out_mode)
    if B0 > 1 and (_src_bytes(x) >= BUF_LIMIT or (seg2 is not None and _src_bytes(seg2[0]) >= BUF_LIMIT)):
        if out is None:
            out = torch.empty(shape, dtype=dt, device=dev)
        kw = dict(ksize=ksize, stride=stride, pad=pad, pad_end=pad_end, upsample=upsample, silu=silu, bias=bias,
                  out_mode=out_mode, variant=variant, split_k=split_k, act=act, gn_stats=gn_stats,
                  plan_out=plan_out, phase=phase)
        return _conv2d_batch_chunks(pc, x, seg2, gn, row_bias, residual, out, B0, kw)
    a = ConvArgs()
    if pad is None:
        pad = k0 // 2
    B, H, W = _fill_src(a.seg[0], x, k0, stride, pad, upsample, gn, silu)
    a.seg[0].pad_end = pad_end
    a.upsample_phase = 1 if phase else 0
    a.nseg = 1
    if seg2 is not None:
        x2, gn2, silu2 = seg2
        _fill_src(a.seg[1], x2, 1, 1, 0, False, gn2, silu2)
        a.nseg = 2
    a.batch, a.ho, a.wo, a.cout = B, Ho, Wo, pc.N
    a.act = act
    a.weight = pc.weight.data_ptr()
    a.k_total = pc.k_total
    a.weight_batch_stride = getattr(pc, "w_batch_stride", 0)
    a.bias = pc.bias.data_ptr() if (bias and pc.bias is not None) else None
    if row_bias is not None:
        rb, off = row_bias
        a.row_bias = rb.data_ptr() + 4 * off
        a.row_bias_ld = rb.stride(0)
    if out is None:
        out = torch.empty(shape, dtype=dt, device=dev)
    a.out = out.data_ptr()
    a.out_ld = out.shape[-1] if out_mode != OUT_NCHW_F32 else 0
    a.out_mode = out_mode
    if residual is not None:
        _need_cuda(residual, "conv2d residual")
        a.residual = residual.data_ptr()
        a.res_ld = residual.shape[-1]
    want_gn = gn_stats and EMIT_GN_STATS and out_mode == OUT_NHWC_F16
    tuned = AUTOTUNE.choose(a, pc, dev, want_gn) if (AUTOTUNE.enabled or AUTOTUNE.table) else None
    if tuned is not None:
        a.variant_hint = tuned[0]
        set_split(a, tuned[1], dev)
        a.tile_group_m = tuned[2] if len(tuned) > 2 else 0
    if variant is None:
        variant = FORCE_VARIANT
    if variant is not None:
        if variant + 1 != a.variant_hint:
            set_split(a, 0, dev)
            a.tile_group_m = 0
        a.variant_hint = variant + 1
    if split_k is not None:
        set_split(a, split_k, dev)
    if TILE_GROUP_M is not None:
        a.tile_group_m = TILE_GROUP_M
    info = ConvPlanInfo()
    check(lib().sdk_conv2d_plan(C.byref(a), C.byref(info)), "conv2d_plan")
    if plan_out is not None:
        plan_out.update(variant=info.variant, split_k=info.split_k, grid_tiles=info.grid_tiles,
                        gn_chunks=info.gn_chunks)
    if info.workspace_bytes > 0:
        ws = WORKSPACE.get(info.workspace_bytes, dev)
        a.workspace = ws.data_ptr()
        a.workspace_bytes = ws.numel()
    part = None
    if want_gn and info.gn_chunks > 0 and out.shape[-1] == pc.N:
        part = torch.empty(B, info.gn_chunks, pc.N, 2, dtype=torch.float32, device=dev)
        a.gn_partial = part.data_ptr()
    if PROFILER.active:
        nb = sum(t.numel() * 2 for t in _as_pair(x) if t is not None) + pc.N * pc.k_total * 2
        if seg2 is not None:
            nb += sum(t.numel() * 2 for t in _as_pair(seg2[0]) if t is not None)
        nb += out.numel() * out.element_size() + (residual.numel() * 2 if residual is not None else 0)
        PROFILER.begin("conv", info, shape=(B * Ho * Wo, pc.N, pc.k_total, info.variant, info.split_k), nbytes=nb)
    check(lib().sdk_conv2d(C.byref(a), _stream()), "conv2d")
    if PROFILER.active:
        PROFILER.end()
    if part is not None:
        setattr(out, GN_ATTR, (part, info.gn_chunks, out._version))
    return out


def linear(pc: PackedConv, x2d, *, silu=False, residual=None, out_mode=OUT_NHWC_F16, out=None, bias=True,
           act=ACT_NONE, n_img=None, plan_out=None, split_k=None):
    _claim(out)
    M = x2d.shape[0]
    nb, rows = (1, M) if n_img is None else (M // n_img, n_img)
    assert nb * rows == M
    if isinstance(pc, PerImageWeights):
        assert n_img is not None and nb == pc.weight.shape[0], "per-image weights: n_img must split M by image"
    x4 = x2d.view(nb, rows, 1, x2d.shape[-1]) if x2d.stride(-1) == 1 and x2d.is_contiguous() else None
    if x4 is None:
        x4 = x2d.as_strided((nb, rows, 1, x2d.shape[1]), (rows * x2d.stride(0), x2d.stride(0), x2d.stride(0), 1))
    res4 = residual.view(nb, rows, 1, residual.shape[-1]) if residual is not None else None
    y = conv2d(pc, x4, ksize=1, pad=0, silu=silu, residual=res4, out_mode=out_mode, bias=bias,
               out=None if out is None else out.view(nb, rows, 1, out.shape[-1]), act=act, plan_out=plan_out,
               split_k=split_k)
    return y.view(M, y.shape[-1])


def segment_softmax(s, nseg, seglen, scale, ld_p=None, out=None):
    _need_cuda(s, "segment_softmax", torch.float32)
    assert s.dtype == torch.float32 and s.stride(-1) == 1
    M = s.shape[0]
    ld_p = ld_p or (nseg * seglen + BK - 1) // BK * BK
    if out is None:
        out = torch.empty(M, ld_p, dtype=torch.float16, device=s.device)
    check(lib().sdk_segment_softmax(s.data_ptr(), s.stride(0), out.data_ptr(), out.stride(0), M, nseg, seglen,
                                    float(scale), _stream()), "segment_softmax")
    return out



def _gn_args(x, gamma=None, beta=None, eps=0.0, groups=32, gn=None):
    a0, a1 = _as_pair(x)
    _need_cuda(a0, "group_norm")
    B, H, W, Ch = src_shape(x)
    args = GroupNormArgs()
    args.src0 = a0.data_ptr()
    args.ld0 = a0.stride(2)
    if a1 is not None:
        args.src1 = a1.data_ptr()
        args.ld1 = a1.stride(2)
    args.c_split = a0.shape[-1]
    args.batch, args.hw, args.channels = B, H * W, Ch
    if gamma is not None:
        args.groups, args.eps = groups, eps
        args.gamma, args.beta = gamma.data_ptr(), beta.data_ptr()
        gn = (torch.empty(B, Ch, dtype=torch.float32, device=a0.device),
              torch.empty(B, Ch, dtype=torch.float32, device=a0.device))
        ws = WORKSPACE.get(lib().sdk_group_norm_workspace(B, H * W, Ch), a0.device)
        args.workspace, args.workspace_bytes = ws.data_ptr(), ws.numel()
    if gn is not None:
        args.scale, args.shift = gn[0].data_ptr(), gn[1].data_ptr()
    return args, (B, H, W, Ch), a0.device, gn


def _producer_parts(x):
    srcs = [t for t in _as_pair(x) if t is not None]
    parts = [getattr(t, GN_ATTR, None) for t in srcs]
    parts = [pp if pp is not None and pp[2] == t._version else None for pp, t in zip(parts, srcs)]
    if not all(pp is not None for pp in parts):
        return None, 0, None, 0
    p1, n1 = (parts[1][0], parts[1][1]) if len(parts) > 1 else (None, 0)
    return parts[0][0], parts[0][1], p1, n1


def group_norm_plan(x, *, groups=32, pad=0, stats=True, apply=True, parts=None, single_launch=True):
    args, (B, H, W, Ch), _, _ = _gn_args(x)
    args.groups = groups
    args.scale = args.shift = args.src0
    if parts is None:
        _, n0, _, n1 = _producer_parts(x)
    else:
        n0, n1 = (parts, parts) if isinstance(parts, int) else parts
    info = _lib.GroupNormPlanInfo()
    check(lib().sdk_group_norm_plan(C.byref(args), int(stats), int(apply), H, W, pad, int(n0), int(n1),
                                    int(single_launch), C.byref(info)), "group_norm_plan")
    return {"stats": _lib.GN_STATS[info.stats], "apply": _lib.GN_APPLY[info.apply], "launches": info.launches,
            "workspace_bytes": info.workspace_bytes}


PREPAD = 1


def gn_conv_pad():
    return (1, 0) if PREPAD else (0, 1)


def group_norm_apply(x, gn, silu=True, out=None, pad=0):
    args, (B, H, W, Ch), dev, _ = _gn_args(x, gn=gn)
    y = _claim(out) if out is not None else torch.empty(B, H + 2 * pad, W + 2 * pad, Ch, dtype=torch.float16,
                                                          device=dev)
    if PROFILER.active:
        PROFILER.begin("gn_apply", None)
    if pad:
        check(lib().sdk_group_norm_apply_padded(C.byref(args), 1 if silu else 0, _ptr(y), Ch, H, W, pad, _stream()),
              "group_norm_apply_padded")
    else:
        check(lib().sdk_group_norm_apply(C.byref(args), 1 if silu else 0, _ptr(y), Ch, _stream()),
              "group_norm_apply")
    if PROFILER.active:
        PROFILER.end()
    return y


def group_norm_apply_ex(x, gn, silu=True, post_bias=None, residual=None):
    args, (B, H, W, Ch), dev, _ = _gn_args(x, gn=gn)
    y = torch.empty(B, H, W, Ch, dtype=torch.float16, device=dev)
    pb_ld = 0
    if post_bias is not None:
        _need_cuda(post_bias, "group_norm_apply_ex post_bias", torch.float32)
        pb_ld = post_bias.stride(0)
    res_ld = 0
    if residual is not None:
        _need_cuda(residual, "group_norm_apply_ex residual")
        res_ld = residual.shape[-1]
    if PROFILER.active:
        PROFILER.begin("gn_apply", None)
    check(lib().sdk_group_norm_apply_ex(C.byref(args), 1 if silu else 0, _ptr(post_bias), pb_ld, _ptr(residual),
                                        res_ld, _ptr(y), Ch, _stream()), "group_norm_apply_ex")
    if PROFILER.active:
        PROFILER.end()
    return y


def upsample_bilinear2x(x):
    _need_cuda(x, "upsample_bilinear2x")
    x = x.contiguous()
    B, H, W, Cc = x.shape
    y = torch.empty(B, 2 * H, 2 * W, Cc, dtype=torch.float16, device=x.device)
    check(lib().sdk_upsample_bilinear2x(_ptr(x), _ptr(y), B, H, W, Cc, _stream()), "upsample_bilinear2x")
    return y


def zero_border(x, pad=1):
    _need_cuda(x, "zero_border")
    B, H, W, Cc = x.shape
    if x.stride(-1) != 1 or x.stride(1) != W * x.stride(2) or x.stride(0) != H * x.stride(1):
        x = x.contiguous()
    y = torch.empty(B, H + 2 * pad, W + 2 * pad, Cc, dtype=torch.float16, device=x.device)
    check(lib().sdk_zero_border(_ptr(x), x.stride(2), _ptr(y), B, H, W, Cc, pad, _stream()), "zero_border")
    return y


def upsample_nearest2x_padded(x, pad=1):
    _need_cuda(x, "upsample_nearest2x_padded")
    B, H, W, Cc = x.shape
    if x.stride(-1) != 1 or x.stride(1) != W * x.stride(2) or x.stride(0) != H * x.stride(1):
        x = x.contiguous()
    y = torch.empty(B, 2 * H + 2 * pad, 2 * W + 2 * pad, Cc, dtype=torch.float16, device=x.device)
    check(lib().sdk_upsample_nearest2x_padded(_ptr(x), x.stride(2), _ptr(y), B, H, W, Cc, pad, _stream()),
          "upsample_nearest2x_padded")
    return y


def gelu(x):
    _need_cuda(x, "gelu")
    x = x.contiguous()
    y = torch.empty_like(x)
    check(lib().sdk_gelu(_ptr(x), _ptr(y), x.numel(), _stream()), "gelu")
    return y


def group_norm_scale_shift(x, gamma, beta, eps, groups=32):
    args, _, _, gn = _gn_args(x, gamma, beta, eps, groups)
    p0, n0, p1, n1 = _producer_parts(x)
    if PROFILER.active:
        PROFILER.begin("group_norm", None)
    check(lib().sdk_group_norm_finalize(C.byref(args), _ptr(p0), n0, _ptr(p1), n1, _stream()), "group_norm_finalize")
    if PROFILER.active:
        PROFILER.end()
    return gn


def group_norm_affine(x, gamma, beta, eps, groups=32):
    args, _, _, gn = _gn_args(x, gamma, beta, eps, groups)
    if PROFILER.active:
        PROFILER.begin("group_norm", None)
    check(lib().sdk_group_norm_affine(C.byref(args), _stream()), "group_norm_affine")
    if PROFILER.active:
        PROFILER.end()
    return gn


def group_norm(x, gamma, beta, eps, groups=32, silu=True, pad=0, out=None):
    args, (B, H, W, Ch), dev, gn = _gn_args(x, gamma, beta, eps, groups)
    y = _claim(out) if out is not None else torch.empty(B, H + 2 * pad, W + 2 * pad, Ch, dtype=torch.float16,
                                                          device=dev)
    p0, n0, p1, n1 = _producer_parts(x)
    if PROFILER.active:
        PROFILER.begin("group_norm", None)
    check(lib().sdk_group_norm(C.byref(args), 1 if silu else 0, _ptr(y), y.shape[-1], H, W, pad, _ptr(p0), n0,
                               _ptr(p1), n1, _stream()), "group_norm")
    if PROFILER.active:
        PROFILER.end()
    return y


def group_norm_film(x, gamma, beta, eps, film, film_off, groups=32, silu=True, pad=0, out=None):
    args, (B, H, W, Ch), dev, gn = _gn_args(x, gamma, beta, eps, groups)
    _need_cuda(film, "group_norm_film film", torch.float32)
    if film.dim() != 2 or film.shape[0] != B or film.stride(1) != 1 or film_off < 0 or \
            film_off + 2 * Ch > film.shape[1]:
        raise ValueError(f"sd_amd.group_norm_film: film {tuple(film.shape)} has no [{B}, {film_off}:{film_off}+2*{Ch}]")
    y = _claim(out) if out is not None else torch.empty(B, H + 2 * pad, W + 2 * pad, Ch, dtype=torch.float16,
                                                          device=dev)
    p0, n0, p1, n1 = _producer_parts(x)
    if PROFILER.active:
        PROFILER.begin("group_norm_film", None)
    check(lib().sdk_group_norm_film(C.byref(args), _ptr(film), film.stride(0), film_off, 1 if silu else 0, _ptr(y),
                                    y.shape[-1], H, W, pad, _ptr(p0), n0, _ptr(p1), n1, _stream()),
          "group_norm_film")
    if PROFILER.active:
        PROFILER.end()
    return y


RESAMPLE_MODES = {"down": _lib.RESAMPLE_AVGPOOL2, "up": _lib.RESAMPLE_NEAREST2}


def group_norm_resample(x, gn, mode, silu=True, pad=0, act=True, raw=True):
    args, (B, H, W, Ch), dev, _ = _gn_args(x, gn=gn)
    if gn is None:
        act = False
    if not act and not raw:
        raise ValueError("sd_amd.group_norm_resample: no output asked for")
    Ho, Wo = (H // 2, W // 2) if mode == "down" else (2 * H, 2 * W)
    ya = torch.empty(B, Ho + 2 * pad, Wo + 2 * pad, Ch, dtype=torch.float16, device=dev) if act else None
    yr = torch.empty(B, Ho, Wo, Ch, dtype=torch.float16, device=dev) if raw else None
    if PROFILER.active:
        PROFILER.begin("group_norm_resample", None)
    check(lib().sdk_group_norm_resample(C.byref(args), RESAMPLE_MODES[mode], 1 if silu else 0, H, W, pad, _ptr(ya),
                                        _ptr(yr), _stream()), "group_norm_resample")
    if PROFILER.active:
        PROFILER.end()
    return ya, yr


def embedding_add(emb, table, ids):
    _need_cuda(emb, "embedding_add emb")
    _need_cuda(table, "embedding_add table", torch.float32)
    _need_cuda(ids, "embedding_add ids", torch.int64)
    B, D = emb.shape
    if table.dim() != 2 or table.shape[1] != D or ids.shape != (B,):
        raise ValueError(f"sd_amd.embedding_add: emb {tuple(emb.shape)}, table {tuple(table.shape)}, "
                         f"ids {tuple(ids.shape)}")
    emb, table, ids = emb.contiguous(), table.contiguous(), ids.contiguous()
    out = torch.empty(B, D, dtype=torch.float16, device=emb.device)
    if PROFILER.active:
        PROFILER.begin("embedding_add", None)
    check(lib().sdk_embedding_add(_ptr(emb), _ptr(table), _ptr(ids), _ptr(out), B, D, table.shape[0], _stream()),
          "embedding_add")
    if PROFILER.active:
        PROFILER.end()
    return out


def embedding_rows(ids, table):
    _need_cuda(ids, "embedding_rows ids", torch.int64)
    _need_cuda(table, "embedding_rows table", torch.float32)
    if ids.dim() != 1 or ids.numel() < 1 or table.dim() != 2 or table.shape[1] < 1:
        raise ValueError(f"sd_amd.embedding_rows: ids {tuple(ids.shape)} (want [n >= 1]), table {tuple(table.shape)} "
                         "(want [rows, dim >= 1])")
    if ids.device != table.device:
        raise ValueError("sd_amd.embedding_rows: ids and table on different devices")
    lo, hi = int(ids.min()), int(ids.max())
    if lo < 0 or hi >= table.shape[0]:
        raise ValueError(f"sd_amd.embedding_rows: id outside [0, {table.shape[0]}) (min {lo}, max {hi})")
    ids, table = ids.contiguous(), table.contiguous()
    n, dim = ids.shape[0], table.shape[1]
    out = torch.empty(n, dim, dtype=torch.float16, device=table.device)
    check(lib().sdk_embedding_rows(_ptr(ids), _ptr(table), _ptr(out), n, dim, _stream()), "embedding_rows")
    return out


RESIZE_MODES = {"nearest": _lib.RESIZE_NEAREST, "bilinear": _lib.RESIZE_BILINEAR, "bicubic": _lib.RESIZE_BICUBIC,
                "area": _lib.RESIZE_AREA}


def resize2d(x, scale_factor, mode="bilinear", out=None):
    _need_cuda(x, "resize2d", torch.float32)
    if x.dim() != 4:
        raise ValueError(f"sd_amd.resize2d: expected NCHW, got {tuple(x.shape)}")
    if mode not in RESIZE_MODES:
        raise ValueError(f"sd_amd.resize2d: mode {mode!r} not in {sorted(RESIZE_MODES)}")
    sh, sw = (scale_factor if isinstance(scale_factor, (tuple, list)) else (scale_factor, scale_factor))
    sh, sw = float(sh), float(sw)
    if not (sh > 0 and sw > 0 and math.isfinite(sh) and math.isfinite(sw)):
        raise ValueError(f"sd_amd.resize2d: scale_factor {scale_factor!r} must be positive and finite")
    B, Cc, H, W = x.shape
    Ho, Wo = math.floor(H * sh), math.floor(W * sw)
    if min(B, Cc, H, W, Ho, Wo) < 1:
        raise ValueError(f"sd_amd.resize2d: empty input or output ({tuple(x.shape)} -> {Ho} x {Wo})")
    if B * Cc >= 2 ** 31 or max(H, W, Ho, Wo) >= 2 ** 31:
        raise ValueError("sd_amd.resize2d: sizes exceed int32")
    x = x.contiguous()
    if out is None:
        out = torch.empty(B, Cc, Ho, Wo, dtype=torch.float32, device=x.device)
    else:
        _need_cuda(out, "resize2d out", torch.float32)
        if tuple(out.shape) != (B, Cc, Ho, Wo) or not out.is_contiguous() or out.device != x.device:
            raise ValueError(f"sd_amd.resize2d: out must be contiguous {(B, Cc, Ho, Wo)} on the input's device")
    a = _lib.Resize2dArgs()
    a.x, a.y = x.data_ptr(), out.data_ptr()
    a.planes, a.h, a.w, a.out_h, a.out_w = B * Cc, H, W, Ho, Wo
    a.mode, a.scale_h, a.scale_w = RESIZE_MODES[mode], sh, sw
    if PROFILER.active:
        PROFILER.begin("resize2d", None, nbytes=4 * (x.numel() + out.numel()))
    check(lib().sdk_resize2d(C.byref(a), _stream()), "resize2d")
    if PROFILER.active:
        PROFILER.end()
    return out


def layer_norm(x2d, gamma, beta, eps=1e-5, out=None):
    _need_cuda(x2d, "layer_norm")
    M, Cc = x2d.shape
    y = _claim(out) if out is not None else torch.empty(M, Cc, dtype=torch.float16, device=x2d.device)
    if PROFILER.active:
        PROFILER.begin("layer_norm", None)
    check(lib().sdk_layer_norm(_ptr(x2d), _ptr(y), M, Cc, x2d.stride(0), y.stride(0), _ptr(gamma), _ptr(beta),
                               C.c_float(eps), _stream()), "layer_norm")
    if PROFILER.active:
        PROFILER.end()
    return y



def probe_peaks(reps=3):
    dev = torch.device("cuda", torch.cuda.current_device())
    seed = torch.randn(32768, device=dev).half()
    nsm = torch.cuda.get_device_properties(dev).multi_processor_count
    sink = torch.empty(4 * nsm * 4, dtype=torch.float32, device=dev)
    out = {}
    for m16, iters, name in ((1, 40000, "mfma_16x16x32_f16_tflops"), (0, 20000, "mfma_32x32x16_f16_tflops")):
        top = 0.0
        for blocks in (2 * nsm, 4 * nsm):
            check(lib().sdk_probe_mfma(m16, blocks, 200, _ptr(seed), _ptr(sink), _stream()), "probe_mfma")
            best = float("inf")
            for _ in range(reps):
                e0, e1 = torch.cuda.Event(enable_timing=True), torch.cuda.Event(enable_timing=True)
                e0.record()
                check(lib().sdk_probe_mfma(m16, blocks, iters, _ptr(seed), _ptr(sink), _stream()), "probe_mfma")
                e1.record()
                e1.synchronize()
                best = min(best, e0.elapsed_time(e1))
            top = max(top, lib().sdk_probe_mfma_flops(m16, blocks, iters) / (best * 1e-3) / 1e12)
        out[name] = round(top, 1)
    nbytes = 1 << 30
    src = torch.empty(nbytes // 2, dtype=torch.float16, device=dev).normal_()
    dst = torch.empty_like(src)
    best_gbs, best_mode = 0.0, 0
    for mode in (0, 1, 2, 3, 1 | (8 << 2), 3 | (8 << 2), 1 | (32 << 2), 3 | (32 << 2), 256, 257, 258, 259):
        check(lib().sdk_probe_copy_ex(_ptr(src), _ptr(dst), nbytes, mode, _stream()), "probe_copy")
        best = float("inf")
        for _ in range(reps):
            e0, e1 = torch.cuda.Event(enable_timing=True), torch.cuda.Event(enable_timing=True)
            e0.record()
            check(lib().sdk_probe_copy_ex(_ptr(src), _ptr(dst), nbytes, mode, _stream()), "probe_copy")
            e1.record()
            e1.synchronize()
            best = min(best, e0.elapsed_time(e1))
        gbs = 2 * nbytes / (best * 1e-3) / 1e9
        if gbs > best_gbs:
            best_gbs, best_mode = gbs, mode
    out["hbm_copy_gbs"] = round(best_gbs, 1)
    out["hbm_copy_mode"] = {"loads_in_flight": 8 if best_mode & 1 else 4, "nontemporal": bool(best_mode & 2),
                            "form": "flat one pass" if best_mode & 256 else "grid-stride",
                            "workgroups_per_cu": None if best_mode & 256 else ((best_mode >> 2) & 63) or 16}
    del src, dst
    return out



ATTN_FORMS = {"auto": _lib.ATTN_AUTO, "nw4": _lib.ATTN_NW4, "nw8": _lib.ATTN_NW8, "nw8_stag": _lib.ATTN_NW8_STAG,
              "qb2": _lib.ATTN_QB2, "wide": _lib.ATTN_WIDE}
_ATTN_FORM_NAMES = {v: k for k, v in ATTN_FORMS.items()}
ATTN_WIDE_ROWS = _lib.ATTN_WIDE_ROWS
ATTN_WIDE_KT = _lib.ATTN_WIDE_KT


def attention(q, k, v, *, batch, heads, nq, nk, head_dim, scale, out=None, causal=False, form=None, form_out=None):
    for t, n in ((q, "q"), (k, "k"), (v, "v")):
        _need_cuda(t, "attention " + n)
    if out is None:
        out = torch.empty(batch * nq, heads * head_dim, dtype=torch.float16, device=q.device)
    _claim(out)
    a = AttentionArgs()
    a.q, a.k, a.v, a.o = q.data_ptr(), k.data_ptr(), v.data_ptr(), out.data_ptr()
    a.q_ld, a.k_ld, a.v_ld, a.o_ld = q.stride(0), k.stride(0), v.stride(0), out.stride(0)
    a.batch, a.heads, a.nq, a.nk, a.head_dim, a.scale = batch, heads, nq, nk, head_dim, scale
    a.causal = 1 if causal else 0
    if PROFILER.active:
        PROFILER.begin("attention", (batch, heads, nq, nk, head_dim))
    if form is None and form_out is None:
        check(lib().sdk_attention(C.byref(a), _stream()), "attention")
    else:
        info = _lib.AttentionFormInfo()
        check(lib().sdk_attention_form(C.byref(a), ATTN_FORMS[form or "auto"], C.byref(info), _stream()), "attention")
        if form_out is not None:
            form_out.update(form=_ATTN_FORM_NAMES[info.form], dqk=info.dqk, dv=info.dv, waves=info.waves,
                            qblocks=info.qblocks, stagger=info.stagger, seed_col=info.seed_col,
                            causal=info.causal, grid=info.grid)
    if PROFILER.active:
        PROFILER.end()
    return out


def linear_attention(q, k, v, *, batch, heads, n, dim_head, out=None):
    for t, nm in ((q, "q"), (k, "k"), (v, "v")):
        _need_cuda(t, "linear_attention " + nm)
    if out is None:
        out = torch.empty(batch * n, heads * dim_head, dtype=torch.float16, device=q.device)
    _claim(out)
    a = _lib.LinearAttentionArgs()
    a.q, a.k, a.v, a.o = q.data_ptr(), k.data_ptr(), v.data_ptr(), out.data_ptr()
    a.q_ld, a.k_ld, a.v_ld, a.o_ld = q.stride(0), k.stride(0), v.stride(0), out.stride(0)
    a.batch, a.heads, a.n, a.dim_head = batch, heads, n, dim_head
    nbytes = lib().sdk_linear_attention_workspace_bytes(C.byref(a))
    if nbytes < 0:
        check(-1, "linear_attention")
    ws = torch.empty(nbytes, dtype=torch.uint8, device=q.device)
    a.workspace, a.workspace_bytes = ws.data_ptr(), nbytes
    if PROFILER.active:
        PROFILER.begin("linear_attention", None)
    check(lib().sdk_linear_attention(C.byref(a), _stream()), "linear_attention")
    if PROFILER.active:
        PROFILER.end()
    return out


def cross_attention_block_supported(channels, head_dim, nk, n_img):
    return bool(lib().sdk_cross_attention_block_supported(channels, head_dim, nk, n_img))


XATTN_PACKED_W = True


def xattn_packed_weight(pc: PackedConv):
    pk = getattr(pc, "_xattn_pk", None)
    if pk is None:
        Cc = pc.N
        pk = torch.empty(Cc * Cc, dtype=torch.float16, device=pc.weight.device)
        check(lib().sdk_xattn_pack_weight(pc.weight.data_ptr(), pc.k_total, pk.data_ptr(), Cc, _stream()),
              "xattn_pack_weight")
        pc._xattn_pk = pk
    return pk


def cross_attention_block(t, kv, pc_q: PackedConv, pc_o: PackedConv, *, batch, n_img, nk, heads, head_dim, scale,
                          residual=None, out=None, norm_in=None, norm_out=None, out_ln=None):
    Cc = heads * head_dim
    for x, n in ((t, "t"), (kv, "kv")):
        _need_cuda(x, "cross_attention_block " + n)
    if pc_q.k_total != Cc or pc_o.k_total != Cc or pc_q.N != Cc or pc_o.N != Cc:
        raise ValueError("sd_amd.cross_attention_block: to_q / to_out must be channels x channels")
    if out is None:
        out = torch.empty(batch * n_img, Cc, dtype=torch.float16, device=t.device)
    _claim(out)
    _claim(out_ln)
    a = XAttnArgs()
    a.t, a.kv, a.wq, a.wo = t.data_ptr(), kv.data_ptr(), pc_q.weight.data_ptr(), pc_o.weight.data_ptr()
    packed = XATTN_PACKED_W and (not torch.cuda.is_current_stream_capturing() or
                                 (hasattr(pc_q, "_xattn_pk") and hasattr(pc_o, "_xattn_pk")))
    if packed:
        a.wq, a.wo = xattn_packed_weight(pc_q).data_ptr(), xattn_packed_weight(pc_o).data_ptr()
    a.bias = pc_o.bias.data_ptr() if pc_o.bias is not None else None
    a.res = residual.data_ptr() if residual is not None else None
    a.out = out.data_ptr()
    a.t_ld, a.kv_ld, a.w_ld = t.stride(0), kv.stride(0), 0 if packed else Cc
    a.res_ld = residual.stride(0) if residual is not None else 0
    a.out_ld = out.stride(0)
    a.batch, a.n_img, a.nk, a.channels, a.head_dim, a.scale = batch, n_img, nk, Cc, head_dim, scale
    if PROFILER.active:
        PROFILER.begin("cross_attention_block", None)
        PROFILER._cur = PROFILER._cur[:2] + (4.0 * batch * n_img * Cc * Cc + 4.0 * batch * n_img * nk * Cc,) + \
            PROFILER._cur[3:]
    if norm_in is None and norm_out is None:
        check(lib().sdk_cross_attention_block(C.byref(a), _stream()), "cross_attention_block")
    else:
        ln = XAttnLnArgs()
        if norm_in is not None:
            ln.in_gamma, ln.in_beta, ln.in_eps = norm_in[0].data_ptr(), norm_in[1].data_ptr(), norm_in[2]
        if norm_out is not None:
            if out_ln is None:
                out_ln = torch.empty_like(out)
            ln.out_gamma, ln.out_beta, ln.out_eps = norm_out[0].data_ptr(), norm_out[1].data_ptr(), norm_out[2]
            ln.out_ln, ln.out_ln_ld = out_ln.data_ptr(), out_ln.stride(0)
        check(lib().sdk_cross_attention_block_ln(C.byref(a), C.byref(ln), _stream()), "cross_attention_block")
    if PROFILER.active:
        PROFILER.end()
    return (out, out_ln) if norm_out is not None else out


def ff_supported(channels, features):
    return bool(lib().sdk_ff_supported(channels, features))


class PackedFF:

    def __init__(self, w1, b1, w2, b2, device):
        F2, Cc = w1.shape
        self.channels, self.features = Cc, F2 // 2
        if not ff_supported(Cc, self.features):
            raise ValueError(f"sd_amd.PackedFF: unsupported shape channels={Cc} features={self.features}")
        w1h = w1.detach().to(device=device, dtype=torch.float16).contiguous()
        w2h = w2.detach().to(device=device, dtype=torch.float16).contiguous()
        b1f = b1.detach().to(device=device, dtype=torch.float32).contiguous() if b1 is not None else None
        self.b2 = b2.detach().to(device=device, dtype=torch.float32).contiguous() if b2 is not None else None
        nbytes = lib().sdk_ff_packed_bytes(Cc, self.features)
        self.packed = torch.empty(nbytes, dtype=torch.uint8, device=device)
        check(lib().sdk_ff_pack(_ptr(w1h), _ptr(b1f), _ptr(w2h), _ptr(self.packed), Cc, self.features, _stream()),
              "ff_pack")


def feed_forward(pf: PackedFF, t, residual=None, out=None):
    _need_cuda(t, "feed_forward t")
    M, Cc = t.shape
    if Cc != pf.channels or t.stride(-1) != 1:
        raise ValueError("sd_amd.feed_forward: t must be [M, channels] with unit column stride")
    if out is None:
        out = torch.empty(M, Cc, dtype=torch.float16, device=t.device)
    _claim(out)
    a = FfArgs()
    a.t, a.out, a.packed = t.data_ptr(), out.data_ptr(), pf.packed.data_ptr()
    a.b2 = pf.b2.data_ptr() if pf.b2 is not None else None
    if residual is not None:
        _need_cuda(residual, "feed_forward residual")
        a.res, a.res_ld = residual.data_ptr(), residual.stride(0)
    a.t_ld, a.out_ld = t.stride(0), out.stride(0)
    a.rows, a.channels, a.features = M, Cc, pf.features
    if PROFILER.active:
        PROFILER.begin("feed_forward", None, shape=(M, Cc, pf.features))
        PROFILER._cur = PROFILER._cur[:2] + (2.0 * M * Cc * 3 * pf.features,) + PROFILER._cur[3:]
    check(lib().sdk_feed_forward(C.byref(a), _stream()), "feed_forward")
    if PROFILER.active:
        PROFILER.end()
    return out


def token_linear_supported(in_features, out_features):
    return bool(lib().sdk_token_linear_supported(in_features, out_features))


class PackedTokenLinear:

    def __init__(self, w, b, device):
        w = w.detach().reshape(w.shape[0], -1)
        if not token_linear_supported(w.shape[1], w.shape[0]):
            raise ValueError(f"sd_amd.PackedTokenLinear: unsupported shape {tuple(w.shape)}")
        self.features = w.shape[0]
        self.w = w.to(device=device, dtype=torch.float16).contiguous()
        self.b = b.detach().to(device=device, dtype=torch.float32).contiguous() if b is not None else None


def token_linear(pk: PackedTokenLinear, x, residual=None, out=None, norm=None):
    _need_cuda(x, "token_linear x")
    M, K = x.shape
    if K != pk.features or x.stride(-1) != 1:
        raise ValueError("sd_amd.token_linear: x must be [M, 320] with unit column stride")
    if out is None:
        out = torch.empty(M, pk.features, dtype=torch.float16, device=x.device)
    _claim(out)
    a = TokenLinearArgs()
    a.x, a.w, a.out = x.data_ptr(), pk.w.data_ptr(), out.data_ptr()
    a.bias = pk.b.data_ptr() if pk.b is not None else None
    if residual is not None:
        _need_cuda(residual, "token_linear residual")
        if residual.shape != (M, pk.features) or residual.stride(-1) != 1:
            raise ValueError("sd_amd.token_linear: residual must be [M, 320] with unit column stride")
        a.res, a.res_ld = residual.data_ptr(), residual.stride(0)
    a.x_ld, a.out_ld = x.stride(0), out.stride(0)
    a.rows, a.in_features, a.out_features = M, K, pk.features
    if PROFILER.active:
        PROFILER.begin("token_linear", None, shape=(M, pk.features, K))
        PROFILER._cur = PROFILER._cur[:2] + (2.0 * M * K * pk.features,) + PROFILER._cur[3:]
    if norm is None:
        check(lib().sdk_token_linear(C.byref(a), _stream()), "token_linear")
    else:
        g, bt, eps = norm
        _need_cuda(g, "token_linear_ln gamma", torch.float32)
        _need_cuda(bt, "token_linear_ln beta", torch.float32)
        if g.numel() != pk.features or bt.numel() != pk.features:
            raise ValueError("sd_amd.token_linear: norm gamma / beta must have 320 elements")
        out_ln = torch.empty(M, pk.features, dtype=torch.float16, device=x.device)
        check(lib().sdk_token_linear_ln(C.byref(a), g.data_ptr(), bt.data_ptr(), float(eps), out_ln.data_ptr(),
                                        out_ln.stride(0), _stream()), "token_linear_ln")
    if PROFILER.active:
        PROFILER.end()
    return out if norm is None else (out, out_ln)


PROJ_QKV_C, PROJ_QKV_N = 320, 960
PROJ_QKV_PANEL = 256


def proj_qkv_perm():
    p = torch.arange(PROJ_QKV_C)
    c, r = p // 160, p % 160
    nb, cg, q = r // 16, (r % 16) // 4, r % 4
    g = 10 * c + nb
    return 32 * (g // 2) + 8 * cg + 4 * (g % 2) + q


def proj_qkv_pack(w_in, b_in, w_qkv, b_qkv=None):
    w_in = w_in.detach().float().reshape(w_in.shape[0], -1)
    w_qkv = w_qkv.detach().float().reshape(w_qkv.shape[0], -1)
    if tuple(w_in.shape) != (PROJ_QKV_C, PROJ_QKV_C) or tuple(w_qkv.shape) != (PROJ_QKV_N, PROJ_QKV_C):
        raise ValueError(f"sd_amd.proj_qkv_pack: unsupported shapes {tuple(w_in.shape)} / {tuple(w_qkv.shape)}")
    perm = proj_qkv_perm().to(w_in.device)
    b_in = torch.zeros(PROJ_QKV_C, device=w_in.device) if b_in is None else b_in.detach().float()
    b_qkv = torch.zeros(PROJ_QKV_N, device=w_in.device) if b_qkv is None else b_qkv.detach().float().to(w_in.device)
    return torch.cat([w_in[perm], w_qkv.to(w_in.device)], 0), torch.cat([b_in[perm], b_qkv], 0)


def proj_qkv_unpack(w, b):
    perm = proj_qkv_perm().to(w.device)
    w_in, b_in = torch.empty_like(w[:PROJ_QKV_C]), torch.empty_like(b[:PROJ_QKV_C])
    w_in[perm], b_in[perm] = w[:PROJ_QKV_C], b[:PROJ_QKV_C]
    return w_in, b_in, w[PROJ_QKV_C:], b[PROJ_QKV_C:]


def proj_norm_qkv_supported(in_features, features, qkv_features):
    return bool(lib().sdk_proj_norm_qkv_supported(in_features, features, qkv_features))


_CU_COUNT = {}


def cu_count(dev):
    key = torch.device(dev)
    if key not in _CU_COUNT:
        _CU_COUNT[key] = torch.cuda.get_device_properties(key).multi_processor_count
    return _CU_COUNT[key]


def proj_qkv_chain_fills(rows, cus):
    panels = (rows + PROJ_QKV_PANEL - 1) // PROJ_QKV_PANEL
    last = panels % cus
    return panels <= cus or last == 0 or 2 * last >= cus


class PackedProjQkv:

    def __init__(self, w_in, b_in, w_qkv, device, b_qkv=None):
        w, b = proj_qkv_pack(w_in, b_in, w_qkv, b_qkv)
        self.w = w.to(device=device, dtype=torch.float16).contiguous()
        self.b = b.to(device=device, dtype=torch.float32).contiguous()


def proj_norm_qkv(pk: PackedProjQkv, x, norm, gn=None, hw=None, tok=None, qkv=None):
    _need_cuda(x, "proj_norm_qkv x")
    M, K = x.shape
    if K != PROJ_QKV_C or x.stride(-1) != 1:
        raise ValueError("sd_amd.proj_norm_qkv: x must be [M, 320] with unit column stride")
    g, bt, eps = norm
    _need_cuda(g, "proj_norm_qkv gamma", torch.float32)
    _need_cuda(bt, "proj_norm_qkv beta", torch.float32)
    if g.numel() != PROJ_QKV_C or bt.numel() != PROJ_QKV_C:
        raise ValueError("sd_amd.proj_norm_qkv: norm gamma / beta must have 320 elements")
    if tok is None:
        tok = torch.empty(M, PROJ_QKV_C, dtype=torch.float16, device=x.device)
    if qkv is None:
        qkv = torch.empty(M, PROJ_QKV_N, dtype=torch.float16, device=x.device)
    _claim(tok)
    _claim(qkv)
    a = ProjNormQkvArgs()
    a.x, a.w, a.bias, a.gamma, a.beta = x.data_ptr(), pk.w.data_ptr(), pk.b.data_ptr(), g.data_ptr(), bt.data_ptr()
    a.tok, a.qkv = tok.data_ptr(), qkv.data_ptr()
    a.x_ld, a.tok_ld, a.qkv_ld = x.stride(0), tok.stride(0), qkv.stride(0)
    a.rows, a.in_features, a.features, a.qkv_features = M, K, tok.shape[1], qkv.shape[1]
    a.eps = float(eps)
    if gn is not None:
        sc, sh = gn
        _need_cuda(sc, "proj_norm_qkv gn scale", torch.float32)
        _need_cuda(sh, "proj_norm_qkv gn shift", torch.float32)
        if hw and (not sc.is_contiguous() or not sh.is_contiguous() or sc.numel() != M // hw * PROJ_QKV_C
                   or sh.numel() != sc.numel()):
            raise ValueError("sd_amd.proj_norm_qkv: gn scale / shift must be contiguous fp32 [M / hw, 320]")
        a.gn_scale, a.gn_shift = sc.data_ptr(), sh.data_ptr()
    a.hw = int(hw or 0)
    if PROFILER.active:
        PROFILER.begin("proj_norm_qkv", None, shape=(M, PROJ_QKV_C + PROJ_QKV_N, K),
                       nbytes=2 * M * (K + PROJ_QKV_C + PROJ_QKV_N))
        PROFILER._cur = PROFILER._cur[:2] + (2.0 * M * K * (PROJ_QKV_C + PROJ_QKV_N),) + PROFILER._cur[3:]
    check(lib().sdk_proj_norm_qkv(C.byref(a), _stream()), "proj_norm_qkv")
    if PROFILER.active:
        PROFILER.end()
    return tok, qkv



def token_embedding(ids: torch.Tensor, tok: torch.Tensor, pos: torch.Tensor):
    _need_cuda(ids, "token_embedding", torch.int64)
    _need_cuda(tok, "token_embedding table", torch.float32)
    _need_cuda(pos, "token_embedding positions", torch.float32)
    B, T = ids.shape
    if T > pos.shape[0]:
        raise ValueError(f"sd_amd.token_embedding: {T} tokens > {pos.shape[0]} positions")
    out = torch.empty(B, T, tok.shape[1], dtype=torch.float16, device=ids.device)
    check(lib().sdk_token_embedding(_ptr(ids.contiguous()), _ptr(tok), _ptr(pos), _ptr(out), B, T, tok.shape[1],
                                    _stream()), "token_embedding")
    return out


def extract_patches(z: torch.Tensor, kh: int, kw: int, sy: int, sx: int):
    _need_cuda(z, "extract_patches", torch.float32)
    z = z.contiguous()
    B, Cc, H, W = z.shape
    Ly, Lx = (H - kh) // sy + 1, (W - kw) // sx + 1
    out = torch.empty(Ly * Lx, B, Cc, kh, kw, dtype=torch.float32, device=z.device)
    check(lib().sdk_extract_patches(_ptr(z), _ptr(out), B, Cc, H, W, kh, kw, sy, sx, _stream()), "extract_patches")
    return out


def fold_patches(patches: torch.Tensor, pix_w: torch.Tensor, l_w, H: int, W: int, sy: int, sx: int, Ly: int,
                 Lx: int):
    _need_cuda(patches, "fold_patches", torch.float32)
    _need_cuda(pix_w, "fold_patches weights", torch.float32)
    patches = patches.contiguous()
    L, B, Cc, ph, pw = patches.shape
    assert L == Ly * Lx
    out = torch.empty(B, Cc, H, W, dtype=torch.float32, device=patches.device)
    check(lib().sdk_fold_patches(_ptr(patches), _ptr(pix_w.contiguous()), _ptr(l_w), _ptr(out), B, Cc, H, W, ph, pw,
                                 sy, sx, Ly, Lx, _stream()), "fold_patches")
    return out


def timestep_embedding(t: torch.Tensor, freqs: torch.Tensor, dim: int):
    _need_cuda(t, "timestep_embedding", torch.int64)
    out = torch.empty(t.shape[0], dim, dtype=torch.float16, device=t.device)
    check(lib().sdk_timestep_embedding(_ptr(t), _ptr(freqs), _ptr(out), t.shape[0], dim, _stream()),
          "timestep_embedding")
    return out


def nchw_to_nhwc(x: torch.Tensor, c_pad: int, scale: float = 1.0):
    _need_cuda(x, "nchw_to_nhwc", torch.float32)
    x = x.contiguous()
    B, Cc, H, W = x.shape
    y = torch.empty(B, H, W, c_pad, dtype=torch.float16, device=x.device)
    check(lib().sdk_nchw_to_nhwc(_ptr(x), _ptr(y), B, Cc, H * W, c_pad, C.c_float(scale), _stream()),
          "nchw_to_nhwc")
    return y


def _drop_scale(what, keep, drop_p, ref, noise):
    p = float(drop_p)
    if not 0.0 <= p <= 1.0:
        raise ValueError(f"sd_amd.{what}: drop_p must be in [0, 1], got {drop_p}")
    if keep is None:
        if p > 0.0:
            raise ValueError(f"sd_amd.{what}: drop_p > 0 needs keep (one byte per element)")
        return None, 0.0
    if not torch.is_tensor(keep) or not keep.is_cuda or keep.device != ref.device or \
            keep.dtype not in (torch.uint8, torch.bool):
        raise ValueError(f"sd_amd.{what}: keep must be a CUDA uint8 / bool tensor on {ref.device}")
    if keep.shape != ref.shape:
        raise ValueError(f"sd_amd.{what}: keep {tuple(keep.shape)} vs {tuple(ref.shape)}")
    if noise is None:
        raise ValueError(f"sd_amd.{what}: keep needs noise")
    keep = keep.contiguous()
    if keep.dtype == torch.bool:
        keep = keep.view(torch.uint8)
    return keep, (0.0 if p == 1.0 else float(np.float32(1.0 / (1.0 - p))))


def _same_f32(what, ref, **tensors):
    out = {}
    for k, v in tensors.items():
        if v is None:
            out[k] = None
            continue
        if not torch.is_tensor(v) or not v.is_cuda or v.dtype != torch.float32 or v.device != ref.device:
            raise ValueError(f"sd_amd.{what}: {k} must be a CUDA fp32 tensor on {ref.device}")
        if v.shape != ref.shape:
            raise ValueError(f"sd_amd.{what}: {k} {tuple(v.shape)} vs {tuple(ref.shape)}")
        out[k] = v.contiguous()
    return out


def _mask_mode(what, mask, shape):
    if len(shape) != 4:
        raise ValueError(f"sd_amd.{what}: the mask blend needs NCHW tensors, got {tuple(shape)}")
    B, Cc, H, W = shape
    modes = {(B, 1, H, W): 0, (1, 1, H, W): 1, (B, Cc, H, W): 2}
    if tuple(mask.shape) not in modes:
        raise ValueError(f"sd_amd.{what}: mask {tuple(mask.shape)} does not broadcast over {tuple(shape)}")
    return modes[tuple(mask.shape)]


def _ddim_ex(what, ref, x, e, sc, pred_x0_in, noise, e_uncond, guidance, v_param, x_prev, pred_x0, temperature,
             keep, drop_p, blend_x0, blend_noise, blend_mask, blend_sqrt_acp, blend_sqrt_1m_acp, x_next):
    t = _same_f32(what, ref, noise=noise, e_uncond=e_uncond)
    noise, e_uncond = t["noise"], t["e_uncond"]
    keep, scale = _drop_scale(what, keep, drop_p, ref, noise)
    ex = _lib.DdimExArgs()
    a = ex.step
    a.x = x.data_ptr() if x is not None else None
    a.e, a.x_prev, a.pred_x0 = e.data_ptr(), x_prev.data_ptr(), pred_x0.data_ptr()
    a.e_uncond = e_uncond.data_ptr() if e_uncond is not None else None
    a.noise = noise.data_ptr() if noise is not None else None
    a.n = ref.numel()
    if not pred_x0_in:
        a.sqrt_one_minus_at = float(sc["sqrt_one_minus_at"])
        a.sqrt_at = float(sc["sqrt_at"])
    a.dir_coef = float(sc["dir_coef"])
    a.sqrt_a_prev = float(sc["sqrt_a_prev"])
    a.sigma = float(sc["sigma"])
    a.temperature = float(temperature)
    a.guidance = float(guidance)
    if v_param is not None:
        a.v_param = 1
        a.v_sqrt_a, a.v_sqrt_1ma = float(v_param[0]), float(v_param[1])
    ex.pred_x0_in = int(pred_x0_in)
    if keep is not None:
        ex.keep, ex.drop_scale = keep.data_ptr(), scale
    if blend_mask is None:
        if blend_x0 is not None or blend_noise is not None or x_next is not None:
            raise ValueError(f"sd_amd.{what}: blend_x0 / blend_noise / x_next need blend_mask")
        check(lib().sdk_ddim_step_ex(C.byref(ex), _stream()), what)
        return None
    if blend_x0 is None or blend_noise is None or blend_sqrt_acp is None or blend_sqrt_1m_acp is None:
        raise ValueError(f"sd_amd.{what}: the blend needs blend_x0, blend_noise, blend_sqrt_acp and blend_sqrt_1m_acp")
    t = _same_f32(what, ref, blend_x0=blend_x0, blend_noise=blend_noise)
    if not torch.is_tensor(blend_mask) or not blend_mask.is_cuda or blend_mask.dtype != torch.float32 or \
            blend_mask.device != ref.device:
        raise ValueError(f"sd_amd.{what}: blend_mask must be a CUDA fp32 tensor on {ref.device}")
    m = ex.blend
    m.mask_mode = _mask_mode(what, blend_mask, ref.shape)
    blend_mask = blend_mask.contiguous()
    if x_next is None:
        x_next = torch.empty_like(ref)
    elif x_next.shape != ref.shape or not x_next.is_contiguous() or x_next.dtype != torch.float32 or \
            x_next.device != ref.device:
        raise ValueError(f"sd_amd.{what}: x_next must be a contiguous CUDA fp32 tensor of x's shape")
    m.x0, m.noise, m.mask, m.out = t["blend_x0"].data_ptr(), t["blend_noise"].data_ptr(), blend_mask.data_ptr(), \
        x_next.data_ptr()
    m.n, m.per_sample, m.hw = ref.numel(), ref.numel() // ref.shape[0], ref.shape[2] * ref.shape[3]
    m.sqrt_acp, m.sqrt_1m_acp = float(blend_sqrt_acp), float(blend_sqrt_1m_acp)
    check(lib().sdk_ddim_step_ex(C.byref(ex), _stream()), what)
    return x_next


def ddim_step(x, e, sc: dict, noise=None, e_uncond=None, guidance=1.0, v_param=None, x_prev=None, pred_x0=None,
              temperature=1.0, *, keep=None, drop_p=0.0, blend_x0=None, blend_noise=None, blend_mask=None,
              blend_sqrt_acp=None, blend_sqrt_1m_acp=None, x_next=None):
    _need_cuda(x, "ddim_step", torch.float32)
    _need_cuda(e, "ddim_step", torch.float32)
    if e.shape != x.shape:
        raise ValueError(f"sd_amd.ddim_step: x {tuple(x.shape)} vs e {tuple(e.shape)}")
    x, e = x.contiguous(), e.contiguous()
    xp = x_prev if x_prev is not None else torch.empty_like(x)
    p0 = pred_x0 if pred_x0 is not None else torch.empty_like(x)
    xn = _ddim_ex("ddim_step", x, x, e, sc, False, noise, e_uncond, guidance, v_param, xp, p0, temperature, keep,
                  drop_p, blend_x0, blend_noise, blend_mask, blend_sqrt_acp, blend_sqrt_1m_acp, x_next)
    return (xp, p0) if xn is None else (xp, p0, xn)


def ddim_xprev(pred_x0, e, sc: dict, x=None, noise=None, e_uncond=None, guidance=1.0, v_param=None, x_prev=None,
               temperature=1.0, *, keep=None, drop_p=0.0, blend_x0=None, blend_noise=None, blend_mask=None,
               blend_sqrt_acp=None, blend_sqrt_1m_acp=None, x_next=None):
    _need_cuda(pred_x0, "ddim_xprev", torch.float32)
    _need_cuda(e, "ddim_xprev", torch.float32)
    if e.shape != pred_x0.shape:
        raise ValueError(f"sd_amd.ddim_xprev: pred_x0 {tuple(pred_x0.shape)} vs e {tuple(e.shape)}")
    pred_x0, e = pred_x0.contiguous(), e.contiguous()
    xp = x_prev if x_prev is not None else torch.empty_like(pred_x0)
    if v_param is not None:
        if x is None:
            raise ValueError("sd_amd.ddim_xprev: v_param needs x")
        _need_cuda(x, "ddim_xprev", torch.float32)
        x = x.contiguous()
    else:
        x = None
    xn = _ddim_ex("ddim_xprev", pred_x0, x, e, sc, True, noise, e_uncond, guidance, v_param, xp, pred_x0, temperature,
                  keep, drop_p, blend_x0, blend_noise, blend_mask, blend_sqrt_acp, blend_sqrt_1m_acp, x_next)
    return xp if xn is None else (xp, xn)


MULTISTEP_FORMS = {"plms": _lib.MULTISTEP_PLMS, "plms_warmup": _lib.MULTISTEP_PLMS_WARMUP, "dpm": _lib.MULTISTEP_DPM}


def multistep_step(x, e, sc: dict, form="plms", history=(), e_next=None, coefs=None, e_uncond=None, guidance=1.0,
                   v_param=None, x_prev=None, pred_x0=None, hist_out=None, *, blend_x0=None, blend_noise=None,
                   blend_mask=None, blend_sqrt_acp=None, blend_sqrt_1m_acp=None, x_next=None):
    what = "multistep_step"
    _need_cuda(x, what, torch.float32)
    _need_cuda(e, what, torch.float32)
    if e.shape != x.shape:
        raise ValueError(f"sd_amd.{what}: x {tuple(x.shape)} vs e {tuple(e.shape)}")
    if form not in MULTISTEP_FORMS:
        raise ValueError(f"sd_amd.{what}: form must be one of {sorted(MULTISTEP_FORMS)}, got {form!r}")
    history = list(history)
    most = {"plms": 3, "plms_warmup": 0, "dpm": 1}[form]
    if len(history) > most:
        raise ValueError(f"sd_amd.{what}: form '{form}' takes at most {most} history tensors, got {len(history)}")
    if (form == "plms_warmup") != (e_next is not None):
        raise ValueError(f"sd_amd.{what}: e_next goes with form 'plms_warmup' (and only with it)")
    if (form == "dpm") != (coefs is not None):
        raise ValueError(f"sd_amd.{what}: coefs = (c_x, c_0, c_1) goes with form 'dpm' (and only with it)")
    x, e = x.contiguous(), e.contiguous()
    t = _same_f32(what, x, e_uncond=e_uncond, e_next=e_next, **{f"history[{k}]": h for k, h in enumerate(history)})
    for k, h in enumerate(history):
        if h is None:
            raise ValueError(f"sd_amd.{what}: history[{k}] is None")
    outs = {"x_prev": x_prev, "pred_x0": pred_x0, "hist_out": hist_out, "x_next": x_next}
    for k, v in outs.items():
        if v is not None and (not torch.is_tensor(v) or v.shape != x.shape or not v.is_contiguous() or
                              v.dtype != torch.float32 or v.device != x.device):
            raise ValueError(f"sd_amd.{what}: {k} must be a contiguous CUDA fp32 tensor of x's shape")
    xp = x_prev if x_prev is not None else torch.empty_like(x)
    p0 = pred_x0 if pred_x0 is not None else torch.empty_like(x)
    m = _lib.MultistepArgs()
    a = m.step
    a.x, a.e, a.x_prev, a.pred_x0 = x.data_ptr(), e.data_ptr(), xp.data_ptr(), p0.data_ptr()
    a.e_uncond = t["e_uncond"].data_ptr() if t["e_uncond"] is not None else None
    a.n = x.numel()
    a.sqrt_one_minus_at, a.sqrt_at = float(sc["sqrt_one_minus_at"]), float(sc["sqrt_at"])
    if form != "dpm":
        if float(sc.get("sigma", 0.0)) != 0.0:
            raise ValueError(f"sd_amd.{what}: PLMS is deterministic: the scalars must be those of eta = 0")
        a.dir_coef, a.sqrt_a_prev = float(sc["dir_coef"]), float(sc["sqrt_a_prev"])
    else:
        m.c_x, m.c_0, m.c_1 = (float(c) for c in coefs)
    a.temperature, a.guidance = 1.0, float(guidance)
    if v_param is not None:
        a.v_param = 1
        a.v_sqrt_a, a.v_sqrt_1ma = float(v_param[0]), float(v_param[1])
    m.form, m.nhist = MULTISTEP_FORMS[form], len(history)
    for k in range(len(history)):
        m.hist[k] = t[f"history[{k}]"].data_ptr()
    if e_next is not None:
        m.e_next = t["e_next"].data_ptr()
    if hist_out is not None:
        m.hist_out = hist_out.data_ptr()
    if blend_mask is None:
        if blend_x0 is not None or blend_noise is not None or x_next is not None:
            raise ValueError(f"sd_amd.{what}: blend_x0 / blend_noise / x_next need blend_mask")
        check(lib().sdk_multistep_step(C.byref(m), _stream()), what)
        return xp, p0
    if blend_x0 is None or blend_noise is None or blend_sqrt_acp is None or blend_sqrt_1m_acp is None:
        raise ValueError(f"sd_amd.{what}: the blend needs blend_x0, blend_noise, blend_sqrt_acp and blend_sqrt_1m_acp")
    tb = _same_f32(what, x, blend_x0=blend_x0, blend_noise=blend_noise)
    if not torch.is_tensor(blend_mask) or not blend_mask.is_cuda or blend_mask.dtype != torch.float32 or \
            blend_mask.device != x.device:
        raise ValueError(f"sd_amd.{what}: blend_mask must be a CUDA fp32 tensor on {x.device}")
    b = m.blend
    b.mask_mode = _mask_mode(what, blend_mask, x.shape)
    blend_mask = blend_mask.contiguous()
    xn = x_next if x_next is not None else torch.empty_like(x)
    b.x0, b.noise, b.mask, b.out = tb["blend_x0"].data_ptr(), tb["blend_noise"].data_ptr(), blend_mask.data_ptr(), \
        xn.data_ptr()
    b.n, b.per_sample, b.hw = x.numel(), x.numel() // x.shape[0], x.shape[2] * x.shape[3]
    b.sqrt_acp, b.sqrt_1m_acp = float(blend_sqrt_acp), float(blend_sqrt_1m_acp)
    check(lib().sdk_multistep_step(C.byref(m), _stream()), what)
    return xp, p0, xn


def cfg_combine(e_uncond, e_cond, guidance, out=None):
    _need_cuda(e_cond, "cfg_combine", torch.float32)
    t = _same_f32("cfg_combine", e_cond, e_uncond=e_uncond)
    if t["e_uncond"] is None:
        raise ValueError("sd_amd.cfg_combine: e_uncond must be a CUDA fp32 tensor")
    e_cond = e_cond.contiguous()
    y = out if out is not None else torch.empty_like(e_cond)
    if y.shape != e_cond.shape or not y.is_contiguous() or y.dtype != torch.float32 or y.device != e_cond.device:
        raise ValueError("sd_amd.cfg_combine: out must be a contiguous CUDA fp32 tensor of e_cond's shape")
    check(lib().sdk_cfg_combine(t["e_uncond"].data_ptr(), e_cond.data_ptr(), y.data_ptr(), e_cond.numel(),
                                C.c_float(float(guidance)), _stream()), "cfg_combine")
    return y



def concat_nchw_to_nhwc(srcs, c_pad: int):
    srcs = list(srcs)
    if not 1 <= len(srcs) <= 4:
        raise ValueError(f"sd_amd.concat_nchw_to_nhwc: 1..4 sources, got {len(srcs)}")
    for s in srcs:
        _need_cuda(s, "concat_nchw_to_nhwc", torch.float32)
        if s.dim() != 4 or s.shape[0] != srcs[0].shape[0] or s.shape[2:] != srcs[0].shape[2:]:
            raise ValueError("sd_amd.concat_nchw_to_nhwc: sources must be NCHW with the same batch and spatial "
                             f"size, got {[tuple(t.shape) for t in srcs]}")
    srcs = [s.contiguous() for s in srcs]
    B, _, H, W = srcs[0].shape
    csum = sum(s.shape[1] for s in srcs)
    if c_pad < csum:
        raise ValueError(f"sd_amd.concat_nchw_to_nhwc: c_pad {c_pad} below the channel sum {csum}")
    y = torch.empty(B, H, W, c_pad, dtype=torch.float16, device=srcs[0].device)
    a = _lib.ConcatArgs()
    for i, s in enumerate(srcs):
        a.src[i], a.channels[i] = s.data_ptr(), s.shape[1]
    a.nsrc, a.y, a.batch, a.hw, a.c_pad = len(srcs), y.data_ptr(), B, H * W, c_pad
    check(lib().sdk_concat_nchw_to_nhwc(C.byref(a), _stream()), "concat_nchw_to_nhwc")
    return y


def patch_grid(h: int, w: int, ks, stride):
    h, w = int(h), int(w)
    ks, stride = (int(ks[0]), int(ks[1])), (int(stride[0]), int(stride[1]))
    if h <= 0 or w <= 0 or min(ks) <= 0 or min(stride) <= 0:
        raise ValueError(f"sd_amd.patch_grid: sizes must be positive, got {h}x{w}, ks {ks}, stride {stride}")
    ks = (min(ks[0], h), min(ks[1], w))
    stride = (min(stride[0], h), min(stride[1], w))
    return ks, stride, (h - ks[0]) // stride[0] + 1, (w - ks[1]) // stride[1] + 1


def patch_pack(srcs, c_pad: int, kh: int, kw: int, sy: int, sx: int, p0: int = 0, np: int = None):
    srcs = list(srcs)
    if not 1 <= len(srcs) <= 4:
        raise ValueError(f"sd_amd.patch_pack: 1..4 sources, got {len(srcs)}")
    for s in srcs:
        _need_cuda(s, "patch_pack", torch.float32)
        if s.dim() != 4 or s.shape[0] != srcs[0].shape[0] or s.shape[2:] != srcs[0].shape[2:]:
            raise ValueError("sd_amd.patch_pack: sources must be NCHW with the same batch and spatial size, got "
                             f"{[tuple(t.shape) for t in srcs]}")
    srcs = [s.contiguous() for s in srcs]
    B, _, H, W = srcs[0].shape
    csum = sum(s.shape[1] for s in srcs)
    if c_pad < csum:
        raise ValueError(f"sd_amd.patch_pack: c_pad {c_pad} below the channel sum {csum}")
    if not (0 < kh <= H and 0 < kw <= W and sy > 0 and sx > 0):
        raise ValueError(f"sd_amd.patch_pack: patches {kh}x{kw} every ({sy}, {sx}) do not fit {H}x{W}")
    total = ((H - kh) // sy + 1) * ((W - kw) // sx + 1) * B
    if np is None:
        np = total - p0
    if p0 < 0 or np < 1 or p0 + np > total:
        raise ValueError(f"sd_amd.patch_pack: window [{p0}, {p0 + np}) outside the {total} patches")
    y = torch.empty(np, kh, kw, c_pad, dtype=torch.float16, device=srcs[0].device)
    a = _lib.PatchPackArgs()
    for i, s in enumerate(srcs):
        a.src[i], a.channels[i] = s.data_ptr(), s.shape[1]
    a.nsrc, a.y, a.batch, a.h, a.w, a.c_pad = len(srcs), y.data_ptr(), B, H, W, c_pad
    a.kh, a.kw, a.sy, a.sx, a.p0, a.np = kh, kw, sy, sx, p0, np
    check(lib().sdk_patch_pack(C.byref(a), _stream()), "patch_pack")
    return y


def _t_runs(t, batch):
    ts = [int(t)] * batch if not isinstance(t, (list, tuple)) else [int(v) for v in t]
    if len(ts) != batch:
        raise ValueError(f"sd_amd: {len(ts)} timesteps for a batch of {batch}")
    runs, b0 = [], 0
    for b in range(1, batch + 1):
        if b == batch or ts[b] != ts[b0]:
            runs.append((b0, b, ts[b0]))
            b0 = b
    return runs


def posterior_step(x, model_out, t, tables: dict, noise=None, *, x0_param=False, clip=False, temperature=1.0,
                   stage=0, x_recon_in=None, x_prev=None, x_recon=None, want_x_recon=False, keep=None, drop_p=0.0):
    ref = x if x is not None else model_out
    B = ref.shape[0]
    ins = {"x": x, "model_out": model_out, "noise": noise, "x_recon_in": x_recon_in}
    for k, v in ins.items():
        if v is not None:
            _need_cuda(v, "posterior_step " + k, torch.float32)
            if v.shape != ref.shape:
                raise ValueError(f"sd_amd.posterior_step: {k} {tuple(v.shape)} vs {tuple(ref.shape)}")
            ins[k] = v.contiguous()
    if stage != 1 and x_prev is None:
        x_prev = torch.empty_like(ref, memory_format=torch.contiguous_format)
    if (stage == 1 or want_x_recon) and x_recon is None:
        x_recon = torch.empty_like(ref, memory_format=torch.contiguous_format)
    keep, scale = _drop_scale("posterior_step", keep, drop_p, ref, ins["noise"])
    if keep is not None and stage == 1:
        raise ValueError("sd_amd.posterior_step: keep needs a stage that writes x_prev")
    per = ref.numel() // B
    ex = _lib.PosteriorExArgs()
    ex.drop_scale = scale
    a = ex.step
    a.stage, a.x0_param, a.clip, a.temperature = int(stage), int(bool(x0_param)), int(bool(clip)), float(temperature)
    for b0, b1, ti in _t_runs(t, B):
        off = b0 * per * 4
        for k, v in ins.items():
            setattr(a, k, v.data_ptr() + off if v is not None else None)
        a.x_prev = x_prev.data_ptr() + off if x_prev is not None and stage != 1 else None
        a.x_recon = x_recon.data_ptr() + off if x_recon is not None else None
        ex.keep = keep.data_ptr() + b0 * per if keep is not None else None
        a.n = (b1 - b0) * per
        a.c_recip, a.c_recipm1 = float(tables["c_recip"][ti]), float(tables["c_recipm1"][ti])
        a.coef1, a.coef2, a.sigma = float(tables["coef1"][ti]), float(tables["coef2"][ti]), float(tables["sigma"][ti])
        a.nonzero = 0.0 if ti == 0 or noise is None else 1.0
        check(lib().sdk_posterior_step_ex(C.byref(ex), _stream()), "posterior_step")
    return x_prev, x_recon


def masked_q_sample(x0, noise, mask, img, t, sqrt_acp, sqrt_1m_acp, out=None):
    for k, v in (("x0", x0), ("noise", noise), ("mask", mask), ("img", img)):
        _need_cuda(v, "masked_q_sample " + k, torch.float32)
    if x0.dim() != 4 or noise.shape != x0.shape or img.shape != x0.shape:
        raise ValueError("sd_amd.masked_q_sample: x0, noise and img must be one NCHW shape")
    B, Cc, H, W = x0.shape
    mode = _mask_mode("masked_q_sample", mask, x0.shape)
    x0, noise, mask = x0.contiguous(), noise.contiguous(), mask.contiguous()
    if not img.is_contiguous():
        if out is img:
            raise ValueError("sd_amd.masked_q_sample: in-place update needs a contiguous img")
        img = img.contiguous()
    y = out if out is not None else torch.empty_like(img)
    if y.shape != img.shape or not y.is_contiguous() or y.dtype != torch.float32:
        raise ValueError("sd_amd.masked_q_sample: out must be a contiguous fp32 tensor of img's shape")
    per, hw = Cc * H * W, H * W
    a = _lib.MaskedQArgs()
    a.per_sample, a.hw, a.mask_mode = per, hw, mode
    for b0, b1, ti in _t_runs(t, B):
        off = b0 * per * 4
        a.x0, a.noise, a.img, a.out = x0.data_ptr() + off, noise.data_ptr() + off, img.data_ptr() + off, y.data_ptr() + off
        a.mask = mask.data_ptr() + (0 if mode == 1 else b0 * (hw if mode == 0 else per) * 4)
        a.n = (b1 - b0) * per
        a.sqrt_acp, a.sqrt_1m_acp = float(sqrt_acp[ti]), float(sqrt_1m_acp[ti])
        check(lib().sdk_masked_q_sample(C.byref(a), _stream()), "masked_q_sample")
    return y



def _vq_codebook(codebook, what):
    _need_cuda(codebook, what + " codebook", torch.float32)
    if codebook.dim() != 2 or not codebook.is_contiguous():
        raise ValueError(f"sd_amd.{what}: codebook must be a contiguous [n_e, e_dim] tensor")
    return codebook.shape


def vq_code_norms(codebook: torch.Tensor):
    N, D = _vq_codebook(codebook, "vq_code_norms")
    norms = torch.empty(N, dtype=torch.float32, device=codebook.device)
    check(lib().sdk_vq_code_norms(_ptr(codebook), _ptr(norms), N, D, _stream()), "vq_code_norms")
    return norms


def vq_nearest(z: torch.Tensor, codebook: torch.Tensor, norms: torch.Tensor = None, splits: int = 0):
    _need_cuda(z, "vq_nearest", torch.float32)
    N, D = _vq_codebook(codebook, "vq_nearest")
    if z.dim() != 4 or z.shape[1] != D:
        raise ValueError(f"sd_amd.vq_nearest: z {tuple(z.shape)} does not match e_dim {D} (expected [B, {D}, H, W])")
    if not 1 <= D <= 256:
        raise ValueError(f"sd_amd.vq_nearest: e_dim {D} outside [1, 256]")
    if z.numel() == 0:
        raise ValueError("sd_amd.vq_nearest: empty input")
    if norms is None:
        norms = vq_code_norms(codebook)
    _need_cuda(norms, "vq_nearest norms", torch.float32)
    if norms.shape != (N,):
        raise ValueError(f"sd_amd.vq_nearest: norms {tuple(norms.shape)} vs n_e {N}")
    z = z.contiguous()
    B, _, H, W = z.shape
    M = B * H * W
    zq = torch.empty_like(z)
    idx = torch.empty(M, dtype=torch.int64, device=z.device)
    keys = None
    if splits > 1 or (splits <= 0 and lib().sdk_vq_nearest_splits(M, N, D) > 1):
        keys = torch.empty(M, dtype=torch.int64, device=z.device)
    check(lib().sdk_vq_nearest(_ptr(z), _ptr(codebook), _ptr(norms.contiguous()), _ptr(idx), _ptr(zq), B, D, H * W, N,
                               _ptr(keys), M * 8 if keys is not None else 0, int(splits), _stream()), "vq_nearest")
    return zq, idx


def vq_lookup(idx: torch.Tensor, codebook: torch.Tensor, nchw_shape=None):
    _need_cuda(idx, "vq_lookup", torch.int64)
    N, D = _vq_codebook(codebook, "vq_lookup")
    idx = idx.contiguous().view(-1)
    M = idx.numel()
    if M == 0:
        raise ValueError("sd_amd.vq_lookup: no indices")
    if nchw_shape is not None:
        B, H, W = (int(v) for v in nchw_shape)
        if B * H * W != M:
            raise ValueError(f"sd_amd.vq_lookup: {M} indices do not fill {(B, H, W)}")
        out = torch.empty(B, D, H, W, dtype=torch.float32, device=idx.device)
        hw, nchw = H * W, 1
    else:
        out = torch.empty(M, D, dtype=torch.float32, device=idx.device)
        hw, nchw = 1, 0
    check(lib().sdk_vq_lookup(_ptr(idx), _ptr(codebook), _ptr(out), M, N, D, hw, nchw, _stream()), "vq_lookup")
    return out


def vq_remap(inds: torch.Tensor, used: torch.Tensor, *, to_used: bool, unknown: int = 0, random=None,
             extra: bool = False):
    _need_cuda(inds, "vq_remap", torch.int64)
    _need_cuda(used, "vq_remap used", torch.int64)
    if inds.numel() == 0 or used.dim() != 1 or used.numel() == 0:
        raise ValueError("sd_amd.vq_remap: empty indices or used table")
    src = inds.contiguous()
    if random is not None:
        _need_cuda(random, "vq_remap random", torch.int64)
        if random.numel() != src.numel():
            raise ValueError("sd_amd.vq_remap: random must have one entry per index")
        random = random.contiguous()
    out = torch.empty_like(src)
    check(lib().sdk_vq_remap(_ptr(src), _ptr(used.contiguous()), _ptr(random), _ptr(out), src.numel(), used.numel(),
                             0 if to_used else 1, int(unknown), 1 if extra else 0, _stream()), "vq_remap")
    return out


def diag_gaussian_sample(moments: torch.Tensor, noise=None, scale: float = 1.0, out=None):
    _need_cuda(moments, "diag_gaussian_sample", torch.float32)
    B, C2, H, W = moments.shape
    moments = moments.contiguous()
    if noise is not None:
        _need_cuda(noise, "diag_gaussian_sample noise", torch.float32)
        noise = noise.contiguous()
    z = out if out is not None else torch.empty(B, C2 // 2, H, W, dtype=torch.float32, device=moments.device)
    check(lib().sdk_diag_gaussian_sample(_ptr(moments), _ptr(noise), _ptr(z), B, C2 // 2, H * W, float(scale),
                                         _stream()), "diag_gaussian_sample")
    return z


def stochastic_encode(x0: torch.Tensor, noise: torch.Tensor, sqrt_a: float, sqrt_1ma: float, out=None):
    _need_cuda(x0, "stochastic_encode", torch.float32)
    _need_cuda(noise, "stochastic_encode noise", torch.float32)
    x0, noise = x0.contiguous(), noise.contiguous()
    y = out if out is not None else torch.empty_like(x0)
    check(lib().sdk_stochastic_encode(_ptr(x0), _ptr(noise), _ptr(y), x0.numel(), float(sqrt_a), float(sqrt_1ma),
                                      _stream()), "stochastic_encode")
    return y


def ddpm_step(x, eps, noise, inv_sqrt_alpha, coef, sigma, out=None):
    _need_cuda(x, "ddpm_step", torch.float32)
    y = out if out is not None else torch.empty_like(x)
    check(lib().sdk_ddpm_step(_ptr(x), _ptr(eps), _ptr(noise), _ptr(y), x.numel(), C.c_float(inv_sqrt_alpha),
                              C.c_float(coef), C.c_float(sigma), _stream()), "ddpm_step")
    return y



class _Profiler:

    def __init__(self):
        self.active = False
        self.records = []
        self.regions = []
        self.region = None
        self._cur = None

    def start(self):
        self.records = []
        self.regions = []
        self.active = True

    def stop(self):
        self.active = False

    def begin(self, kind, info, shape=None, nbytes=0):
        s = torch.cuda.current_stream()
        e0 = torch.cuda.Event(enable_timing=True)
        e0.record(s)
        flops = info.flops if isinstance(info, ConvPlanInfo) else None
        if kind == "attention" and info is not None:
            b, h, nq, nk, d = info
            flops = 4.0 * b * h * nq * nk * d
            shape = info
        variant = info.variant if isinstance(info, ConvPlanInfo) else None
        self._cur = (kind, variant, flops, e0, shape, nbytes)

    def end(self):
        s = torch.cuda.current_stream()
        e1 = torch.cuda.Event(enable_timing=True)
        e1.record(s)
        kind, variant, flops, e0, shape, nbytes = self._cur
        self.records.append((kind, variant, flops, e0, e1, shape, nbytes))
        self.regions.append(self.region)

    def region_summary(self, region):
        torch.cuda.synchronize()
        tot = {"launches": 0, "ms": 0.0, "flops": 0.0, "by_kind": {}}
        for rec, reg in zip(self.records, self.regions):
            if reg != region:
                continue
            kind, _, flops, e0, e1, _, _ = rec
            ms = e0.elapsed_time(e1)
            k = tot["by_kind"].setdefault(kind, {"launches": 0, "ms": 0.0, "flops": 0.0})
            for d in (tot, k):
                d["launches"] += 1
                d["ms"] += ms
                d["flops"] += flops or 0.0
        return tot

    def shape_table(self):
        torch.cuda.synchronize()
        out = {}
        for kind, variant, flops, e0, e1, shape, _ in self.records:
            d = out.setdefault((kind, shape), [0, 0.0, 0.0])
            d[0] += 1
            d[1] += e0.elapsed_time(e1)
            d[2] += flops or 0.0
        rows = [(k, v[0], v[1], (v[2] / (v[1] * 1e-3) / 1e12) if v[1] > 0 and v[2] else 0.0) for k, v in out.items()]
        return sorted(rows, key=lambda r: -r[2])

    def summary(self):
        torch.cuda.synchronize()
        out = {}
        for kind, variant, flops, e0, e1, shape, nbytes in self.records:
            key = kind if variant is None else f"{kind}:{variant}"
            d = out.setdefault(key, {"launches": 0, "ms": 0.0, "flops": 0.0, "bytes": 0.0})
            d["launches"] += 1
            d["bytes"] += nbytes
            d["ms"] += e0.elapsed_time(e1)
            d["flops"] += flops or 0.0
        return out


PROFILER = _Profiler()
```

Measured before the change: 18.55 images/sec.

## Fuse SpatialTransformer proj_out and residual into last feed-forward kernel with GN partial stats

Extends the GEGLU feed-forward kernel with a PROJ variant that, for the last transformer block, applies the 1x1 proj_out linear, its bias and the outer residual in the same kernel. Packed proj weights are streamed through a three-stage LDS ring and the output tile is reused from LDS. Per-128-row GroupNorm partial statistics are also emitted so the following group norm can skip its stats pass. This removes a separate conv launch and a round-trip of the token tensor through HBM, at the cost of a larger LDS footprint and a longer, more complex kernel.

After: 18.66 images/sec (median of 6 runs). About the same (+0.6%).

```diff
diff --git a/include/sdk_amd.h b/include/sdk_amd.h
--- a/include/sdk_amd.h
+++ b/include/sdk_amd.h
@@ -188,12 +188,17 @@
   const void* t; const void* res; void* out; const void* packed; const float* b2;
   int32_t t_ld, res_ld, out_ld;
   int32_t rows, channels, features;
+  const void* proj_packed; const float* proj_bias; const void* x;
+  int32_t x_ld, hw;
+  void* gn_partial;
 } sdk_ff_args;
 
 int sdk_ff_supported(int32_t channels, int32_t features);
 int64_t sdk_ff_packed_bytes(int32_t channels, int32_t features);
 int sdk_ff_pack(const void* w1, const float* b1, const void* w2, void* packed, int32_t channels, int32_t features,
                 sdk_stream_t stream);
+int64_t sdk_ff_proj_packed_bytes(int32_t channels);
+int sdk_ff_proj_pack(const void* w, int32_t w_ld, void* packed, int32_t channels, sdk_stream_t stream);
 int sdk_feed_forward(const sdk_ff_args* a, sdk_stream_t stream);
 
 typedef struct {
diff --git a/stable-diffusion-from-scratch_amd/_lib.py b/stable-diffusion-from-scratch_amd/_lib.py
--- a/stable-diffusion-from-scratch_amd/_lib.py
+++ b/stable-diffusion-from-scratch_amd/_lib.py
@@ -73,7 +73,8 @@
 
 class FfArgs(C.Structure):
     _fields_ = [("t", vp), ("res", vp), ("out", vp), ("packed", vp), ("b2", vp), ("t_ld", i32), ("res_ld", i32),
-                ("out_ld", i32), ("rows", i32), ("channels", i32), ("features", i32)]
+                ("out_ld", i32), ("rows", i32), ("channels", i32), ("features", i32),
+                ("proj_packed", vp), ("proj_bias", vp), ("x", vp), ("x_ld", i32), ("hw", i32), ("gn_partial", vp)]
 
 
 class TokenLinearArgs(C.Structure):
@@ -145,7 +146,7 @@
 GN_APPLY = ("none", "in_stats", "flat", "row", "stride")
 
 EXPORTS = ["sdk_conv2d_plan", "sdk_conv2d", "sdk_group_norm_workspace", "sdk_group_norm_affine", "sdk_group_norm_apply", "sdk_group_norm_apply_padded", "sdk_group_norm_apply_ex", "sdk_group_norm", "sdk_group_norm_finalize", "sdk_group_norm_plan", "sdk_layer_norm",
-           "sdk_attention", "sdk_attention_form", "sdk_linear_attention", "sdk_linear_attention_workspace_bytes", "sdk_linear_attention_chunks", "sdk_cross_attention_block_supported", "sdk_xattn_pack_weight", "sdk_cross_attention_block", "sdk_cross_attention_block_ln", "sdk_segment_softmax", "sdk_ff_supported", "sdk_ff_packed_bytes", "sdk_ff_pack", "sdk_feed_forward", "sdk_token_linear_supported", "sdk_token_linear", "sdk_token_linear_ln", "sdk_proj_norm_qkv_supported", "sdk_proj_norm_qkv", "sdk_ddim_step", "sdk_ddim_xprev", "sdk_ddim_step_ex", "sdk_multistep_step", "sdk_cfg_combine", "sdk_posterior_step", "sdk_posterior_step_ex", "sdk_masked_q_sample", "sdk_concat_nchw_to_nhwc", "sdk_patch_pack", "sdk_ddpm_step", "sdk_timestep_embedding", "sdk_nchw_to_nhwc",
+           "sdk_attention", "sdk_attention_form", "sdk_linear_attention", "sdk_linear_attention_workspace_bytes", "sdk_linear_attention_chunks", "sdk_cross_attention_block_supported", "sdk_xattn_pack_weight", "sdk_cross_attention_block", "sdk_cross_attention_block_ln", "sdk_segment_softmax", "sdk_ff_supported", "sdk_ff_packed_bytes", "sdk_ff_pack", "sdk_ff_proj_packed_bytes", "sdk_ff_proj_pack", "sdk_feed_forward", "sdk_token_linear_supported", "sdk_token_linear", "sdk_token_linear_ln", "sdk_proj_norm_qkv_supported", "sdk_proj_norm_qkv", "sdk_ddim_step", "sdk_ddim_xprev", "sdk_ddim_step_ex", "sdk_multistep_step", "sdk_cfg_combine", "sdk_posterior_step", "sdk_posterior_step_ex", "sdk_masked_q_sample", "sdk_concat_nchw_to_nhwc", "sdk_patch_pack", "sdk_ddpm_step", "sdk_timestep_embedding", "sdk_nchw_to_nhwc",
            "sdk_diag_gaussian_sample", "sdk_stochastic_encode", "sdk_token_embedding", "sdk_extract_patches",
            "sdk_fold_patches", "sdk_vq_code_norms", "sdk_vq_nearest_splits", "sdk_vq_nearest", "sdk_vq_lookup", "sdk_vq_remap",
            "sdk_upsample_bilinear2x", "sdk_upsample_nearest2x_padded", "sdk_zero_border", "sdk_gelu",
@@ -202,6 +203,9 @@
     L.sdk_ff_packed_bytes.argtypes = [i32, i32]
     L.sdk_ff_packed_bytes.restype = i64
     L.sdk_ff_pack.argtypes = [vp, vp, vp, vp, i32, i32, vp]
+    L.sdk_ff_proj_packed_bytes.argtypes = [i32]
+    L.sdk_ff_proj_packed_bytes.restype = i64
+    L.sdk_ff_proj_pack.argtypes = [vp, i32, vp, i32, vp]
     L.sdk_feed_forward.argtypes = [C.POINTER(FfArgs), vp]
     L.sdk_token_linear_supported.argtypes = [i32, i32]
     L.sdk_token_linear.argtypes = [C.POINTER(TokenLinearArgs), vp]
diff --git a/stable-diffusion-from-scratch_amd/build.py b/stable-diffusion-from-scratch_amd/build.py
--- a/stable-diffusion-from-scratch_amd/build.py
+++ b/stable-diffusion-from-scratch_amd/build.py
@@ -25,7 +25,7 @@
 
 def _deps(src: str, csrc: str):
     headers = [os.path.join(csrc, "common.h"), os.path.join(HERE, "..", "include", "sdk_amd.h")]
-    if src.startswith("conv") or src == "proj_qkv.hip":
+    if src.startswith("conv") or src in ("proj_qkv.hip", "ff.hip"):
         headers += sorted(os.path.join(csrc, f) for f in os.listdir(csrc) if f.startswith("conv") and f.endswith(".h"))
     return [os.path.join(csrc, src)] + headers
 HIPCC = os.environ.get("HIPCC", "/opt/rocm/bin/hipcc")
diff --git a/stable-diffusion-from-scratch_amd/csrc/ff.hip b/stable-diffusion-from-scratch_amd/csrc/ff.hip
--- a/stable-diffusion-from-scratch_amd/csrc/ff.hip
+++ b/stable-diffusion-from-scratch_amd/csrc/ff.hip
@@ -2,6 +2,7 @@
 #include <type_traits>
 
 #include "common.h"
+#include "conv_tile.h"
 
 namespace sdk {
 namespace {
@@ -27,6 +28,23 @@
 constexpr unsigned FF_OOB = 0x80000000u;
 static_assert(FF_ROWS * FF_ORS * 2 <= FF_NS * FF_SLOT, "epilogue staging fits the ring");
 static_assert(FF_LDS <= 160 * 1024, "LDS");
+constexpr int FFP_NB = FFC / 16;
+constexpr int FFP_NBH = FFP_NB / 2;
+constexpr int FFP_KS = FFC / 32;
+constexpr int FFP_SLAB = FFP_NB * 1024;
+constexpr int FFP_BYTES = FFP_KS * FFP_SLAB;
+constexpr int FFP_GPW = (FFP_NB + FF_NW - 1) / FF_NW;
+constexpr int FFP_RING = FF_ROWS * FF_ORS * 2;
+constexpr int FFP_RB = 32;
+constexpr int FFP_S0 = FF_LDS;
+constexpr int FFP_BIAS = FFP_S0 + FFP_SLAB;
+constexpr int FFP_LDS = FFP_BIAS + 2 * FFC * 4;
+static_assert(FFP_LDS <= 160 * 1024, "LDS");
+static_assert(FFP_RING % 1024 == 0 && FFP_RING + 2 * FFP_SLAB <= FF_XB, "two slab stages end below the exchange slots");
+__device__ __forceinline__ constexpr int ffp_stage(int ks) {
+  return ks % 3 == 0 ? FFP_S0 : FFP_RING + (ks % 3 - 1) * FFP_SLAB;
+}
+static_assert((FF_ROWS / FFP_RB) * FFC * 8 <= 2 * FFP_SLAB, "parked statistics fit the idle slab ring");
 
 struct FfParams {
   const half_t* t;
@@ -36,6 +54,11 @@
   const float* b2;
   int t_ld, res_ld, out_ld;
   int M, nfb;
+  const char* wp;
+  const float* bp;
+  const half_t* x;
+  float2* gnp;
+  int x_ld, hw;
 };
 
 __device__ __forceinline__ __amdgpu_buffer_rsrc_t ff_rsrc(const void* base, long long bytes) {
@@ -47,7 +70,17 @@
   __builtin_amdgcn_raw_ptr_buffer_load_lds(r, (__attribute__((address_space(3))) void*)dst, 16, voff, 0, 0, 0);
 }
 
-template <int DBG>
+__device__ __forceinline__ void ff_issue_proj(__amdgpu_buffer_rsrc_t rwp, char* ffl, int wave, unsigned lane16, int ks) {
+#pragma unroll
+  for (int j = 0; j < FFP_GPW; ++j) {
+    const int piece = j * FF_NW + wave;
+    const bool dummy = piece >= FFP_NB;
+    char* d = ffl + (dummy ? FF_LDS - 1024 : ffp_stage(ks) + piece * 1024);
+    ff_dma(rwp, d, (dummy ? FF_OOB : (unsigned)(ks * FFP_SLAB + piece * 1024)) + lane16);
+  }
+}
+
+template <int DBG, bool PROJ>
 __global__ void __launch_bounds__(FF_NT, 1) ff_geglu_kernel(FfParams p) {
   extern __shared__ __attribute__((aligned(16))) char ffl[];
   const int tid = threadIdx.x, lane = tid & 63;
@@ -88,6 +121,12 @@
     const half_t* tp = p.t + (size_t)tok * p.t_ld + 8 * hh;
 #pragma unroll
     for (int ks = 0; ks < FF_KS; ++ks) tq[ks] = *reinterpret_cast<const h8*>(tp + 16 * ks);
+  }
+  f4 bpv = {0.f, 0.f, 0.f, 0.f}, b2v = {0.f, 0.f, 0.f, 0.f};
+  if constexpr (PROJ) {
+    if (p.bp) bpv = *reinterpret_cast<const f4*>(p.bp + 4 * (tid % (FFC / 4)));
+    if (p.b2) b2v = *reinterpret_cast<const f4*>(p.b2 + 4 * (tid % (FFC / 4)));
+    ff_issue_proj(ff_rsrc(p.wp, FFP_BYTES), ffl, wave, lane16, 0);
   }
   issue(0, 0);
 
@@ -162,8 +201,32 @@
     }
   }
 
+  if constexpr (PROJ) {
+    if (tid < FFC / 4) {
+      reinterpret_cast<f4*>(ffl + FFP_BIAS)[tid] = bpv;
+      reinterpret_cast<f4*>(ffl + FFP_BIAS + FFC * 4)[tid] = b2v;
+    }
+  }
   asm volatile("s_waitcnt vmcnt(0)" ::: "memory");
   __syncthreads();
+  constexpr int CPR = FFC / 8;
+  constexpr int XPT = FF_ROWS * CPR / FF_NT;
+  static_assert(XPT * FF_NT == FF_ROWS * CPR, "whole row-pass rounds");
+  h8 rr[XPT], xr[XPT];
+  if constexpr (PROJ) {
+    const __amdgpu_buffer_rsrc_t rwp = ff_rsrc(p.wp, FFP_BYTES);
+    ff_issue_proj(rwp, ffl, wave, lane16, 1);
+    ff_issue_proj(rwp, ffl, wave, lane16, 2);
+#pragma unroll
+    for (int i = 0; i < XPT; ++i) rr[i] = h8{};
+    if (p.res) {
+#pragma unroll
+      for (int i = 0; i < XPT; ++i) {
+        const int e = tid + i * FF_NT, r = e / CPR, c8 = e - r * CPR;
+        rr[i] = *reinterpret_cast<const h8*>(p.res + (size_t)(m0 + r) * p.res_ld + c8 * 8);
+      }
+    }
+  }
   half_t* os = reinterpret_cast<half_t*>(ffl);
   const int trow = pr * 32 + fr;
 #pragma unroll
@@ -171,14 +234,16 @@
 #pragma unroll
     for (int g = 0; g < 4; ++g) {
       const int ch = half * 160 + ob * 32 + 8 * g + 4 * hh;
-      const f4 bb = p.b2 ? *reinterpret_cast<const f4*>(p.b2 + ch) : f4{0.f, 0.f, 0.f, 0.f};
+      f4 bb;
+      if constexpr (PROJ) bb = *reinterpret_cast<const f4*>(ffl + FFP_BIAS + (FFC + ch) * 4);
+      else bb = p.b2 ? *reinterpret_cast<const f4*>(p.b2 + ch) : f4{0.f, 0.f, 0.f, 0.f};
       h4 v;
 #pragma unroll
       for (int q = 0; q < 4; ++q) v[q] = (half_t)(o[ob][4 * g + q] + bb[q]);
       *reinterpret_cast<h4*>(os + trow * FF_ORS + ch) = v;
     }
   __syncthreads();
-  constexpr int CPR = FFC / 8;
+  if constexpr (!PROJ)
   for (int e = tid; e < FF_ROWS * CPR; e += FF_NT) {
     const int r = e / CPR, c8 = e - r * CPR;
     const int m = m0 + r;
@@ -190,6 +255,96 @@
       for (int q = 0; q < 8; ++q) v[q] = (half_t)((float)v[q] + (float)rr[q]);
     }
     *reinterpret_cast<h8*>(p.out + (size_t)m * p.out_ld + c8 * 8) = v;
+  }
+  if constexpr (PROJ) {
+#pragma unroll
+    for (int i = 0; i < XPT; ++i) {
+      const int e = tid + i * FF_NT, r = e / CPR, c8 = e - r * CPR;
+      h8 v = *reinterpret_cast<const h8*>(os + r * FF_ORS + c8 * 8);
+      if (p.res) {
+#pragma unroll
+        for (int q = 0; q < 8; ++q) v[q] = (half_t)((float)v[q] + (float)rr[i][q]);
+      }
+      *reinterpret_cast<h8*>(os + r * FF_ORS + c8 * 8) = v;
+    }
+    const __amdgpu_buffer_rsrc_t rwp = ff_rsrc(p.wp, FFP_BYTES);
+    const int px = lane & 15, kq = lane >> 4;
+    f4 z[2][FFP_NBH];
+#pragma unroll
+    for (int tg = 0; tg < 2; ++tg)
+#pragma unroll
+      for (int nb = 0; nb < FFP_NBH; ++nb) z[tg][nb] = f4{0.f, 0.f, 0.f, 0.f};
+    const half_t* yb = os + (pr * 32 + px) * FF_ORS + 8 * kq;
+#pragma unroll
+    for (int i = 0; i < XPT; ++i) {
+      const int e = tid + i * FF_NT, r = e / CPR, c8 = e - r * CPR;
+      xr[i] = *reinterpret_cast<const h8*>(p.x + (size_t)(m0 + r) * p.x_ld + c8 * 8);
+    }
+#pragma unroll
+    for (int ks = 0; ks < FFP_KS; ++ks) {
+      if (ks == 0) {
+        asm volatile("s_waitcnt vmcnt(0)" ::: "memory");
+        __syncthreads();
+      } else {
+        if (ks == FFP_KS - 1) asm volatile("s_waitcnt vmcnt(0) lgkmcnt(0)" ::: "memory");
+        else if (ks >= 3) asm volatile("s_waitcnt vmcnt(%0) lgkmcnt(0)" ::"n"(FFP_GPW) : "memory");
+        else asm volatile("s_waitcnt lgkmcnt(0)" ::: "memory");
+        __builtin_amdgcn_s_barrier();
+        asm volatile("" ::: "memory");
+      }
+      if (ks >= 1 && ks + 2 < FFP_KS) ff_issue_proj(rwp, ffl, wave, lane16, ks + 2);
+      const char* st = ffl + ffp_stage(ks) + half * FFP_NBH * 1024 + lane * 16;
+      const h8 y0 = *reinterpret_cast<const h8*>(yb + 32 * ks);
+      const h8 y1 = *reinterpret_cast<const h8*>(yb + 16 * FF_ORS + 32 * ks);
+#pragma unroll
+      for (int nb = 0; nb < FFP_NBH; ++nb) {
+        const h8 wf = *reinterpret_cast<const h8*>(st + nb * 1024);
+        z[0][nb] = __builtin_amdgcn_mfma_f32_16x16x32_f16(wf, y0, z[0][nb], 0, 0, 0);
+        z[1][nb] = __builtin_amdgcn_mfma_f32_16x16x32_f16(wf, y1, z[1][nb], 0, 0, 0);
+      }
+    }
+    __syncthreads();
+#pragma unroll
+    for (int tg = 0; tg < 2; ++tg)
+#pragma unroll
+      for (int nb = 0; nb < FFP_NBH; ++nb) {
+        const int ch = half * 160 + 16 * nb + 4 * kq;
+        const f4 bb = *reinterpret_cast<const f4*>(ffl + FFP_BIAS + ch * 4);
+        h4 v;
+#pragma unroll
+        for (int q = 0; q < 4; ++q) v[q] = (half_t)(z[tg][nb][q] + bb[q]);
+        *reinterpret_cast<h4*>(os + (pr * 32 + 16 * tg + px) * FF_ORS + ch) = v;
+      }
+    __syncthreads();
+#pragma unroll
+    for (int i = 0; i < XPT; ++i) {
+      const int e = tid + i * FF_NT, r = e / CPR, c8 = e - r * CPR;
+      const int m = m0 + r;
+      h8 v = *reinterpret_cast<const h8*>(os + r * FF_ORS + c8 * 8);
+#pragma unroll
+      for (int q = 0; q < 8; ++q) v[q] = (half_t)((float)v[q] + (float)xr[i][q]);
+      *reinterpret_cast<h8*>(os + r * FF_ORS + c8 * 8) = v;
+      *reinterpret_cast<h8*>(p.out + (size_t)m * p.out_ld + c8 * 8) = v;
+    }
+    if (p.gnp) {
+      __syncthreads();
+      float2* park = reinterpret_cast<float2*>(ffl + FFP_RING);
+#pragma unroll
+      for (int b = 0; b < 5; ++b)
+        gn_block_stats<FFP_RB, 32, FF_ORS>(os + pr * FFP_RB * FF_ORS + half * 160 + 32 * b,
+                                           park + pr * FFC + half * 160 + 32 * b);
+      __syncthreads();
+      if (tid < FFC) {
+        const float2 a = park[tid], b = park[FFC + tid], c = park[2 * FFC + tid], d = park[3 * FFC + tid];
+        const float dab = b.x - a.x, dcd = d.x - c.x;
+        const float mab = 0.5f * (a.x + b.x), mcd = 0.5f * (c.x + d.x);
+        const float qab = a.y + b.y + dab * dab * (0.5f * FFP_RB), qcd = c.y + d.y + dcd * dcd * (0.5f * FFP_RB);
+        const float dd = mcd - mab;
+        const int img = m0 / p.hw, chunk = (m0 - img * p.hw) / FF_ROWS;
+        p.gnp[((size_t)img * (p.hw / FF_ROWS) + chunk) * FFC + tid] =
+            make_float2(0.5f * (mab + mcd), qab + qcd + dd * dd * (float)FFP_RB);
+      }
+    }
   }
 }
 
@@ -221,28 +376,43 @@
   }
 }
 
-template <int DBG>
+template <int DBG, bool PROJ>
 int ff_launch(const FfParams& p, unsigned blocks, hipStream_t s) {
   static std::atomic<unsigned long long> lds_done{0};
-  const int rc = ensure_dyn_lds((const void*)ff_geglu_kernel<DBG>, FF_LDS, lds_done, "feed_forward");
+  constexpr int lds = PROJ ? FFP_LDS : FF_LDS;
+  const int rc = ensure_dyn_lds((const void*)ff_geglu_kernel<DBG, PROJ>, lds, lds_done, "feed_forward");
   if (rc != SDK_OK) return rc;
-  hipLaunchKernelGGL(ff_geglu_kernel<DBG>, dim3(blocks), dim3(FF_NT), FF_LDS, s, p);
+  hipLaunchKernelGGL((ff_geglu_kernel<DBG, PROJ>), dim3(blocks), dim3(FF_NT), lds, s, p);
   return check_launch("feed_forward");
 }
 
 int ff_launch_dbg(const FfParams& p, unsigned blocks, int dbg, hipStream_t s) {
+  if (p.wp) return ff_launch<0, true>(p, blocks, s);
 #if defined(SDK_CONV_DIAGNOSTICS)
   switch (dbg) {
-    case 1: return ff_launch<1>(p, blocks, s);
-    case 2: return ff_launch<2>(p, blocks, s);
-    case 3: return ff_launch<3>(p, blocks, s);
-    case 4: return ff_launch<4>(p, blocks, s);
-    case 5: return ff_launch<5>(p, blocks, s);
+    case 1: return ff_launch<1, false>(p, blocks, s);
+    case 2: return ff_launch<2, false>(p, blocks, s);
+    case 3: return ff_launch<3, false>(p, blocks, s);
+    case 4: return ff_launch<4, false>(p, blocks, s);
+    case 5: return ff_launch<5, false>(p, blocks, s);
     default: break;
   }
 #endif
   (void)dbg;
-  return ff_launch<0>(p, blocks, s);
+  return ff_launch<0, false>(p, blocks, s);
+}
+
+__global__ void __launch_bounds__(256) ff_proj_pack_kernel(const half_t* __restrict__ w, int w_ld, char* __restrict__ out) {
+  const int e = blockIdx.x * 256 + threadIdx.x;
+  if (e >= FFP_BYTES / 16) return;
+  const int lane = e & 63, nb = (e >> 6) % FFP_NB, ks = (e >> 6) / FFP_NB;
+  *reinterpret_cast<h8*>(out + (size_t)e * 16) =
+      *reinterpret_cast<const h8*>(w + (size_t)(16 * nb + (lane & 15)) * w_ld + 32 * ks + 8 * (lane >> 4));
+}
+
+bool ff_overlap(const void* a, long long an, const void* b, long long bn) {
+  const uintptr_t x = (uintptr_t)a, y = (uintptr_t)b;
+  return x < y + (uintptr_t)bn && y < x + (uintptr_t)an;
 }
 
 bool ff_shape_ok(int channels, int features) { return channels == FFC && features > 0 && features % 32 == 0; }
@@ -282,7 +452,27 @@
     return fail(SDK_EINVAL, "feed_forward: pointers must be 16-B aligned");
   if ((long long)(a->features / 16) * FF_BLK >= 0x7fffffffLL) return fail(SDK_EINVAL, "feed_forward: too many features");
   FfParams p{(const half_t*)a->t, (const half_t*)a->res, (half_t*)a->out, (const char*)a->packed, a->b2,
-             a->t_ld, a->res_ld, a->out_ld, a->rows, a->features / 16};
+             a->t_ld, a->res_ld, a->out_ld, a->rows, a->features / 16,
+             nullptr, nullptr, nullptr, nullptr, 0, 0};
+  if (a->proj_packed) {
+    if (!a->x) return fail(SDK_EINVAL, "feed_forward: proj_packed needs x");
+    if (a->hw <= 0 || a->hw % FF_ROWS) return fail(SDK_EINVAL, "feed_forward: proj form needs hw % 128 == 0");
+    if (a->rows % a->hw) return fail(SDK_EINVAL, "feed_forward: proj form needs rows % hw == 0");
+    if (a->x_ld % 8 || a->x_ld < a->channels)
+      return fail(SDK_EINVAL, "feed_forward: x_ld must be a multiple of 8 and >= channels");
+    if (((uintptr_t)a->x | (uintptr_t)a->proj_packed | (uintptr_t)a->proj_bias | (uintptr_t)a->gn_partial) & 15)
+      return fail(SDK_EINVAL, "feed_forward: x / proj_packed / proj_bias / gn_partial must be 16-B aligned");
+    const auto span = [&](int ld) { return ((long long)(a->rows - 1) * ld + a->channels) * 2; };
+    if (ff_overlap(a->out, span(a->out_ld), a->t, span(a->t_ld)) ||
+        (a->res && ff_overlap(a->out, span(a->out_ld), a->res, span(a->res_ld))))
+      return fail(SDK_EINVAL, "feed_forward: in the proj form out must not alias t or res");
+    p.wp = (const char*)a->proj_packed;
+    p.bp = a->proj_bias;
+    p.x = (const half_t*)a->x;
+    p.gnp = reinterpret_cast<float2*>(a->gn_partial);
+    p.x_ld = a->x_ld;
+    p.hw = a->hw;
+  }
   const unsigned blocks = (unsigned)((a->rows + FF_ROWS - 1) / FF_ROWS);
 #if defined(SDK_CONV_DIAGNOSTICS)
   static const int dbg = getenv("SDK_FF_DBG") ? atoi(getenv("SDK_FF_DBG")) & 7 : 0;
@@ -291,3 +481,15 @@
 #endif
   return ff_launch_dbg(p, blocks, dbg, (hipStream_t)stream);
 }
+
+extern "C" int64_t sdk_ff_proj_packed_bytes(int32_t channels) { return channels == FFC ? (int64_t)FFP_BYTES : -1; }
+
+extern "C" int sdk_ff_proj_pack(const void* w, int32_t w_ld, void* packed, int32_t channels, sdk_stream_t stream) {
+  if (!w || !packed) return fail(SDK_EINVAL, "ff_proj_pack: null pointer");
+  if (channels != FFC) return fail(SDK_EINVAL, "ff_proj_pack: channels must be 320");
+  if (w_ld < channels || w_ld % 8 || (((uintptr_t)w | (uintptr_t)packed) & 15))
+    return fail(SDK_EINVAL, "ff_proj_pack: w_ld must be a multiple of 8 and >= channels, w / packed 16-B aligned");
+  hipLaunchKernelGGL(ff_proj_pack_kernel, dim3((FFP_BYTES / 16 + 255) / 256), dim3(256), 0, (hipStream_t)stream,
+                     (const half_t*)w, (int)w_ld, (char*)packed);
+  return check_launch("ff_proj_pack");
+}
diff --git a/stable-diffusion-from-scratch_amd/openai_model/attention.py b/stable-diffusion-from-scratch_amd/openai_model/attention.py
--- a/stable-diffusion-from-scratch_amd/openai_model/attention.py
+++ b/stable-diffusion-from-scratch_amd/openai_model/attention.py
@@ -42,6 +42,11 @@
 _CHAIN_ENV = os.environ.get("SD_AMD_PROJ_QKV_CHAIN", "1")
 PROJ_QKV_CHAIN = _CHAIN_ENV != "0"
 PROJ_QKV_CHAIN_GN = _CHAIN_ENV != "xn"
+FF_PROJ_CHAIN = os.environ.get("SD_AMD_FF_PROJ_CHAIN", "1") != "0"
+
+
+def ff_proj_chain_applies(fused_ff, hw, contiguous):
+    return bool(FF_PROJ_CHAIN and fused_ff and hw > 0 and hw % ops.FF_PROJ_ROWS == 0 and contiguous)
 
 
 class ReassocContext:
@@ -190,15 +195,22 @@
             raise NotImplementedError("sd_amd: only the gated (GEGLU) feed-forward is on the SD path")
         self.net = nn.Sequential(GELU(dim, inner_dim), nn.Dropout(dropout), nn.Linear(inner_dim, dim_out))
 
-    def _prepare(self, dev):
+    def _prepare(self, dev, proj=None):
         p = self.net[0].proj
         self._pc1 = ops.PackedConv([(p.weight, p.in_features)], p.bias, geglu=True, device=dev)
         self._pc2 = ops.PackedConv([(self.net[2].weight, self.net[2].in_features)], self.net[2].bias, device=dev)
         self._pff = None
         if FUSED_FF and ops.ff_supported(p.in_features, p.out_features // 2):
-            self._pff = ops.PackedFF(p.weight, p.bias, self.net[2].weight, self.net[2].bias, dev)
-
-    def _run(self, t, residual):
+            if proj is not None and tuple(proj[0].shape[:2]) != (p.in_features, p.in_features):
+                proj = None
+            self._pff = ops.PackedFF(p.weight, p.bias, self.net[2].weight, self.net[2].bias, dev, proj=proj)
+
+    def chains_proj(self):
+        return self._pff is not None and self._pff.proj_packed is not None
+
+    def _run(self, t, residual, proj_x=None, hw=None, out=None):
+        if proj_x is not None and t.is_contiguous() and residual.is_contiguous():
+            return ops.feed_forward(self._pff, t, residual=residual, proj_x=proj_x, hw=hw, out=out)
         if self._pff is not None and t.stride(-1) == 1:
             return ops.feed_forward(self._pff, t, residual=residual)
         g = ops.linear(self._pc1, t, out_mode=ops.OUT_GEGLU_F16)
@@ -218,13 +230,15 @@
         self.norm3 = nn.LayerNorm(dim)
         self.checkpoint = checkpoint
 
-    def _prepare(self, dev):
-        for m in (self.attn1, self.attn2, self.ff):
+    def _prepare(self, dev, proj=None):
+        for m in (self.attn1, self.attn2):
             m._prepare(dev)
+        self.ff._prepare(dev, proj=proj)
         for n in (self.norm1, self.norm2, self.norm3):
             prep_norm(n, dev)
 
-    def _run(self, tok, B, N, kv=None, Lc=None, t=None, qkv=None):
+    def _run(self, tok, B, N, kv=None, Lc=None, t=None, qkv=None, exit_x=None, exit_out=None):
+        ffx = dict(proj_x=exit_x, hw=N, out=exit_out) if exit_x is not None else {}
         if t is None and qkv is None:
             t = ops.layer_norm(tok, self.norm1._g, self.norm1._b, self.norm1.eps)
         tok = self.attn1._run(t, tok, B, N, qkv=qkv)
@@ -237,11 +251,11 @@
                 scale=a2.scale, residual=tok, norm_in=(self.norm2._g, self.norm2._b, self.norm2.eps),
                 norm_out=(self.norm3._g, self.norm3._b, self.norm3.eps))
             ops.PROFILER.region = None
-            return self.ff._run(t, tok)
+            return self.ff._run(t, tok, **ffx)
         t = ops.layer_norm(tok, self.norm2._g, self.norm2._b, self.norm2.eps)
         tok = self.attn2._run(t, tok, B, N, kv, Lc)
         t = ops.layer_norm(tok, self.norm3._g, self.norm3._b, self.norm3.eps)
-        return self.ff._run(t, tok)
+        return self.ff._run(t, tok, **ffx)
 
 
 class SpatialTransformer(nn.Module):
@@ -271,8 +285,9 @@
         self._ptl_in = (ops.PackedTokenLinear(self.proj_in.weight, self.proj_in.bias, dev)
                         if ops.token_linear_supported(self.in_channels, self.inner_dim) else None)
         self._pc_out = ops.PackedConv([(self.proj_out.weight, self.inner_dim)], self.proj_out.bias, device=dev)
-        for blk in self.transformer_blocks:
-            blk._prepare(dev)
+        nblk = len(self.transformer_blocks)
+        for i, blk in enumerate(self.transformer_blocks):
+            blk._prepare(dev, proj=(self.proj_out.weight, self.proj_out.bias) if i == nblk - 1 else None)
         self._ppq = None
         if len(self.transformer_blocks) and self._ptl_in is not None:
             a1 = self.transformer_blocks[0].attn1
@@ -282,6 +297,19 @@
 
     def context_kv(self, ctx2d, L=None):
         return [blk.attn2.context_kv(ctx2d, L) for blk in self.transformer_blocks]
+
+    def _exit_args(self, i, x):
+        B, H, W, Cc = x.shape
+        if i != len(self.transformer_blocks) - 1 or Cc != self.inner_dim or not ff_proj_chain_applies(
+                self.transformer_blocks[i].ff.chains_proj(), H * W, x.is_contiguous()):
+            return {}
+        return dict(exit_x=x.view(B * H * W, Cc), exit_out=torch.empty_like(x))
+
+    def _exit(self, tok, x):
+        if tok.dim() == 4:
+            return tok
+        B, H, W, _ = x.shape
+        return ops.conv2d(self._pc_out, tok.view(B, H, W, self.inner_dim), residual=x, gn_stats=True)
 
     def _run(self, x, kvs=None, Lc=None):
         B, H, W, Cc = x.shape
@@ -295,8 +323,9 @@
                 xn = gn_norm(self.norm, x, silu=False)
                 tok, qkv = ops.proj_norm_qkv(self._ppq, xn.view(B * H * W, Cc), (n1._g, n1._b, n1.eps))
             for i, blk in enumerate(self.transformer_blocks):
-                tok = blk._run(tok, B, H * W, None if kvs is None else kvs[i], Lc, qkv=qkv if i == 0 else None)
-            return ops.conv2d(self._pc_out, tok.view(B, H, W, self.inner_dim), residual=x, gn_stats=True)
+                tok = blk._run(tok, B, H * W, None if kvs is None else kvs[i], Lc, qkv=qkv if i == 0 else None,
+                               **self._exit_args(i, x))
+            return self._exit(tok, x)
         xn = gn_norm(self.norm, x, silu=False)
         t1 = None
         if TOKEN_LINEAR and self._ptl_in is not None and xn.is_contiguous():
@@ -308,8 +337,9 @@
         else:
             tok = ops.conv2d(self._pc_in, xn).view(B * H * W, self.inner_dim)
         for i, blk in enumerate(self.transformer_blocks):
-            tok = blk._run(tok, B, H * W, None if kvs is None else kvs[i], Lc, t=t1 if i == 0 else None)
-        return ops.conv2d(self._pc_out, tok.view(B, H, W, self.inner_dim), residual=x, gn_stats=True)
+            tok = blk._run(tok, B, H * W, None if kvs is None else kvs[i], Lc, t=t1 if i == 0 else None,
+                           **self._exit_args(i, x))
+        return self._exit(tok, x)
 
 
 class QKVAttentionLegacy(nn.Module):
diff --git a/stable-diffusion-from-scratch_amd/ops.py b/stable-diffusion-from-scratch_amd/ops.py
--- a/stable-diffusion-from-scratch_amd/ops.py
+++ b/stable-diffusion-from-scratch_amd/ops.py
@@ -1010,7 +1010,7 @@
 
 class PackedFF:
 
-    def __init__(self, w1, b1, w2, b2, device):
+    def __init__(self, w1, b1, w2, b2, device, proj=None):
         F2, Cc = w1.shape
         self.channels, self.features = Cc, F2 // 2
         if not ff_supported(Cc, self.features):
@@ -1023,9 +1023,26 @@
         self.packed = torch.empty(nbytes, dtype=torch.uint8, device=device)
         check(lib().sdk_ff_pack(_ptr(w1h), _ptr(b1f), _ptr(w2h), _ptr(self.packed), Cc, self.features, _stream()),
               "ff_pack")
-
-
-def feed_forward(pf: PackedFF, t, residual=None, out=None):
+        self.proj_packed = self.proj_bias = None
+        if proj is not None:
+            wp, bp = proj
+            wp = wp.detach().reshape(wp.shape[0], -1)
+            if tuple(wp.shape) != (Cc, Cc):
+                raise ValueError(f"sd_amd.PackedFF: proj weight must be [{Cc}, {Cc}], got {tuple(wp.shape)}")
+            wph = wp.to(device=device, dtype=torch.float16).contiguous()
+            self.proj_bias = bp.detach().to(device=device, dtype=torch.float32).contiguous() if bp is not None else None
+            self.proj_packed = torch.empty(lib().sdk_ff_proj_packed_bytes(Cc), dtype=torch.uint8, device=device)
+            check(lib().sdk_ff_proj_pack(_ptr(wph), Cc, _ptr(self.proj_packed), Cc, _stream()), "ff_proj_pack")
+
+
+FF_PROJ_ROWS = 128
+
+
+def ff_proj_chain_ok(hw, *tensors):
+    return hw > 0 and hw % FF_PROJ_ROWS == 0 and all(t.is_contiguous() for t in tensors)
+
+
+def feed_forward(pf: PackedFF, t, residual=None, out=None, proj_x=None, hw=None):
     _need_cuda(t, "feed_forward t")
     M, Cc = t.shape
     if Cc != pf.channels or t.stride(-1) != 1:
@@ -1033,20 +1050,38 @@
     if out is None:
         out = torch.empty(M, Cc, dtype=torch.float16, device=t.device)
     _claim(out)
+    o2 = out if out.dim() == 2 else out.view(M, Cc)
     a = FfArgs()
-    a.t, a.out, a.packed = t.data_ptr(), out.data_ptr(), pf.packed.data_ptr()
+    a.t, a.out, a.packed = t.data_ptr(), o2.data_ptr(), pf.packed.data_ptr()
     a.b2 = pf.b2.data_ptr() if pf.b2 is not None else None
     if residual is not None:
         _need_cuda(residual, "feed_forward residual")
         a.res, a.res_ld = residual.data_ptr(), residual.stride(0)
-    a.t_ld, a.out_ld = t.stride(0), out.stride(0)
+    a.t_ld, a.out_ld = t.stride(0), o2.stride(0)
     a.rows, a.channels, a.features = M, Cc, pf.features
+    flops = 2.0 * M * Cc * 3 * pf.features
+    part = None
+    if proj_x is not None:
+        _need_cuda(proj_x, "feed_forward proj_x")
+        if pf.proj_packed is None:
+            raise ValueError("sd_amd.feed_forward: proj_x needs a PackedFF built with proj=(weight, bias)")
+        if hw is None or proj_x.shape != t.shape or proj_x.stride(-1) != 1:
+            raise ValueError("sd_amd.feed_forward: proj_x must be [M, channels] with unit column stride, with hw given")
+        a.proj_packed = pf.proj_packed.data_ptr()
+        a.proj_bias = pf.proj_bias.data_ptr() if pf.proj_bias is not None else None
+        a.x, a.x_ld, a.hw = proj_x.data_ptr(), proj_x.stride(0), hw
+        if EMIT_GN_STATS and hw > 0 and hw % FF_PROJ_ROWS == 0 and M % hw == 0:
+            part = torch.empty(M // hw, hw // FF_PROJ_ROWS, Cc, 2, dtype=torch.float32, device=t.device)
+            a.gn_partial = part.data_ptr()
+        flops += 2.0 * M * Cc * Cc
     if PROFILER.active:
         PROFILER.begin("feed_forward", None, shape=(M, Cc, pf.features))
-        PROFILER._cur = PROFILER._cur[:2] + (2.0 * M * Cc * 3 * pf.features,) + PROFILER._cur[3:]
+        PROFILER._cur = PROFILER._cur[:2] + (flops,) + PROFILER._cur[3:]
     check(lib().sdk_feed_forward(C.byref(a), _stream()), "feed_forward")
     if PROFILER.active:
         PROFILER.end()
+    if part is not None:
+        setattr(out, GN_ATTR, (part, hw // FF_PROJ_ROWS, out._version))
     return out
 
 
```
